# ubisoft/ubisoft-laforge-msmd

Hardware: NVIDIA B200
Metric: generated_animation_seconds_per_second (higher is better)
Workload: dtype bf16 tcgen05 (t > 16) + one-pass fp16 tcgen05 (2 < t <= 16) + fp32-grade fp16x3 (t <= 2): every sampling step <= 1e-3 rel-L2 of the fp32 reference

## Files before the change

### ubisoft-laforge-msmd_b200/csrc/denoiser.cu

```cuda
#include "denoiser_kernels.cuh"
#include "gemm_tc.cuh"
#include "profile.cuh"
#include <cuda_fp16.h>
#include <cstdlib>
#include <cstring>
#include <map>
#include <string>
#include <tuple>
#include <vector>

using namespace msmd;

namespace {

constexpr int kRow0FusedMaxS = 1 << 30;

struct LayerW {
  bf16 *Wqkv = nullptr, *Wo = nullptr, *Wq0 = nullptr, *Wkv = nullptr, *Wco = nullptr, *W1 = nullptr, *W2 = nullptr;
  float *bqkv = nullptr, *bo = nullptr, *bq0 = nullptr, *bkv = nullptr, *bco = nullptr, *b1 = nullptr, *b2 = nullptr;
  float *g1 = nullptr, *be1 = nullptr, *g2 = nullptr, *be2 = nullptr, *g3 = nullptr, *be3 = nullptr;
  bf16 *kv = nullptr, *ca = nullptr;
  bf16 *kvh = nullptr, *cah = nullptr;
  __half *Wqkv_h = nullptr, *Wqkv_l = nullptr, *Wo_h = nullptr, *Wo_l = nullptr, *Wq0_h = nullptr, *Wq0_l = nullptr,
         *Wkv_h = nullptr, *Wkv_l = nullptr, *Wco_h = nullptr, *Wco_l = nullptr, *W1_h = nullptr, *W1_l = nullptr,
         *W2_h = nullptr, *W2_l = nullptr;
  float *kv32 = nullptr, *ca32 = nullptr;
};

uint16_t f2bf(float f) {
  uint32_t u;
  memcpy(&u, &f, 4);
  if ((u & 0x7fffffffu) > 0x7f800000u) return (uint16_t)((u >> 16) | 0x40);
  u += 0x7fffu + ((u >> 16) & 1u);
  return (uint16_t)(u >> 16);
}

}

struct msmd_model {
  msmd_config c{};
  int device = 0;
  bool loaded = false, window = false;
  int T = 0, dp = 0, ldd = 80;
  std::vector<LayerW> L;
  std::vector<void*> owned;
  std::vector<void*> wowned;
  bool packing = false;
  float *PE = nullptr, *temb = nullptr, *Wp = nullptr, *bp = nullptr, *Wf = nullptr, *WfT = nullptr, *bf_ = nullptr;
  __half* Wf16 = nullptr;
  std::vector<float*> Ws0, bs0, Ws2, bs2;
  bf16 *Wd1 = nullptr, *Wd2 = nullptr;
  float *bd1 = nullptr, *bd2 = nullptr;
  float *alphas = nullptr, *alpha_bars = nullptr, *sig_flex = nullptr, *sig_inflex = nullptr;
  bf16 *x = nullptr, *qkv = nullptr, *ctx = nullptr, *h = nullptr, *dec1 = nullptr, *mem = nullptr, *x0c = nullptr,
       *q0 = nullptr, *ctx0 = nullptr;
  bf16 *y = nullptr, *y0 = nullptr, *memh = nullptr;
  float *dec2 = nullptr, *pp = nullptr, *pmproj = nullptr, *stat = nullptr,
        *hid = nullptr, *xbuf = nullptr, *mixed = nullptr, *thr = nullptr;
  int* steps = nullptr;
  __half *Wd1_h = nullptr, *Wd1_l = nullptr, *Wd2_h = nullptr, *Wd2_l = nullptr;
  float *fx = nullptr, *fqkv = nullptr, *fctx = nullptr, *fh = nullptr, *fy = nullptr, *fdec1 = nullptr, *fmem = nullptr,
        *fx0c = nullptr, *fq0 = nullptr, *fctx0 = nullptr, *fy0 = nullptr;
  __half *ws_hi = nullptr, *ws_lo = nullptr;
  int* overflow = nullptr;
  int *h_overflow = nullptr;
  cudaEvent_t ovf_event = nullptr;
  bool ovf_pending = false;
  bool window16[2] = {false, false}, window32 = false;
  float *w_audio = nullptr, *w_prev_audio = nullptr, *w_ind = nullptr;
  int S = 0, NX = 0, E = 0;
  const float* indicator = nullptr;
  UpdateParams* d_up = nullptr;
  unsigned int* d_done = nullptr;
  cudaStream_t cap_stream = nullptr;
  typedef std::tuple<int, int, int, int, int, float, float, float> GraphKey;
  std::map<GraphKey, cudaGraphExec_t> graphs;
  void drop_graphs() {
    for (auto& g : graphs) cudaGraphExecDestroy(g.second);
    graphs.clear();
  }
};

namespace {

template <class Tp>
int dalloc(msmd_model* m, Tp** p, size_t n) {
  void* q = nullptr;
  MSMD_CHECK_CUDA(cudaMalloc(&q, n * sizeof(Tp)));
  (m->packing ? m->wowned : m->owned).push_back(q);
  *p = static_cast<Tp*>(q);
  return MSMD_OK;
}

int up_f32(msmd_model* m, float** dst, const std::vector<float>& h) {
  int rc = dalloc(m, dst, h.size());
  if (rc) return rc;
  MSMD_CHECK_CUDA(cudaMemcpy(*dst, h.data(), h.size() * 4, cudaMemcpyHostToDevice));
  return MSMD_OK;
}
int up_bf16(msmd_model* m, bf16** dst, const float* h, size_t n) {
  std::vector<uint16_t> t(n);
  for (size_t i = 0; i < n; ++i) t[i] = f2bf(h[i]);
  int rc = dalloc(m, dst, n);
  if (rc) return rc;
  MSMD_CHECK_CUDA(cudaMemcpy(*dst, t.data(), n * 2, cudaMemcpyHostToDevice));
  return MSMD_OK;
}

int gemm(int fmt, const bf16* A, int64_t lda, const void* W, int64_t ldw, const float* bias, const bf16* aux, int64_t ld_aux,
         void* out, int64_t ldo, int out_f32, int M, int N, int K, int act, cudaStream_t st) {
  GemmDesc d;
  d.mode = fmt ? 3 : 0; d.A = A; d.W = W; d.bias = bias; d.aux = aux; d.out = out;
  d.M = M; d.N = N; d.K = K; d.lda = lda; d.ldw = ldw; d.ldo = ldo; d.ld_aux = ld_aux;
  d.out_f32 = out_f32; d.aux_f32 = 0; d.act = act; d.gelu_heavy = act;
  return gemm_tc_launch(d, st);
}

int up_split(msmd_model* m, __half** hi, __half** lo, const float* h, size_t n, bool want_lo) {
  std::vector<__half> a(n), b(want_lo ? n : 0);
  for (size_t i = 0; i < n; ++i) {
    a[i] = __float2half_rn(h[i]);
    if (want_lo) b[i] = __float2half_rn((h[i] - __half2float(a[i])) * 2048.0f);
  }
  int rc;
  if ((rc = dalloc(m, hi, n))) return rc;
  MSMD_CHECK_CUDA(cudaMemcpy(*hi, a.data(), n * sizeof(__half), cudaMemcpyHostToDevice));
  if (want_lo) {
    if ((rc = dalloc(m, lo, n))) return rc;
    MSMD_CHECK_CUDA(cudaMemcpy(*lo, b.data(), n * sizeof(__half), cudaMemcpyHostToDevice));
  }
  return MSMD_OK;
}

int gemm32(msmd_model* m, const float* A, int64_t lda, const __half* Wh, const __half* Wl, int64_t ldw, const float* bias,
           float* out, int64_t ldo, int M, int N, int K, int act, cudaStream_t st) {
  int rc;
  if ((rc = split_f16(A, m->ws_hi, m->ws_lo, (int64_t)(M - 1) * lda + K, st, m->overflow))) return rc;
  GemmDesc d;
  d.mode = 2; d.A = m->ws_hi; d.A_lo = m->ws_lo; d.W = Wh; d.W_lo = Wl; d.bias = bias; d.out = out;
  d.M = M; d.N = N; d.K = K; d.lda = lda; d.ldw = ldw; d.ldo = ldo; d.out_f32 = 1; d.aux_f32 = 1; d.act = act;
  return gemm_tc_launch(d, st);
}

int window_begin_f32(msmd_model* m, cudaStream_t st);

int run_forward_f32(msmd_model* m, const float* xrows, cudaStream_t st) {
  const msmd_config& c = m->c;
  const int S = m->S, T = m->T, d = c.d_model, M = S * T;
  int rc;
  if (!m->window32 && (rc = window_begin_f32(m, st))) return rc;
  EmbedParams ep{};
  ep.pp = m->pp; ep.temb = m->temb; ep.pmproj = m->pmproj; ep.PE = m->PE; ep.steps = m->steps;
  ep.x = xrows; ep.indicator = c.use_indicator ? m->indicator : nullptr; ep.WfT = m->WfT; ep.bf = m->bf_;
  ep.out = nullptr; ep.S = S; ep.NX = m->NX; ep.E = m->E; ep.Lp = c.n_prev_motions; ep.L = c.n_motions; ep.d = d;
  ep.dm = c.motion_dim;
  if ((rc = embed_f32_launch(ep, m->fx, st))) return rc;
  for (int l = 0; l < c.n_layers; ++l) {
    LayerW& w = m->L[l];
    if ((rc = gemm32(m, m->fx, d, w.Wqkv_h, w.Wqkv_l, d, w.bqkv, m->fqkv, 3 * d, M, 3 * d, d, 0, st))) return rc;
    if ((rc = self_attn_f32_launch(m->fqkv, m->fctx, S, T, c.n_heads, st))) return rc;
    if ((rc = gemm32(m, m->fctx, d, w.Wo_h, w.Wo_l, d, w.bo, m->fy, d, M, d, d, 0, st))) return rc;
    if ((rc = ln_f32_launch(m->fy, m->fx, w.g1, w.be1, w.ca32, w.g2, w.be2, m->fx, m->fx0c, M, T, st))) return rc;
    if ((rc = gemm32(m, m->fx0c, d, w.Wq0_h, w.Wq0_l, d, w.bq0, m->fq0, d, S, d, d, 0, st))) return rc;
    if ((rc = cross_attn_row0_f32_launch(m->fq0, w.kv32, m->fctx0, S, T - 1, c.n_heads, st))) return rc;
    if ((rc = gemm32(m, m->fctx0, d, w.Wco_h, w.Wco_l, d, w.bco, m->fy0, d, S, d, d, 0, st))) return rc;
    if ((rc = ln_row0_f32_launch(m->fy0, m->fx0c, w.g2, w.be2, m->fx, S, T, st))) return rc;
    if ((rc = gemm32(m, m->fx, d, w.W1_h, w.W1_l, d, w.b1, m->fh, c.d_ff, M, c.d_ff, d, 1, st))) return rc;
    if ((rc = gemm32(m, m->fh, c.d_ff, w.W2_h, w.W2_l, c.d_ff, w.b2, m->fy, d, M, d, c.d_ff, 0, st))) return rc;
    if ((rc = ln_f32_launch(m->fy, m->fx, w.g3, w.be3, nullptr, nullptr, nullptr, m->fx, nullptr, M, T, st))) return rc;
  }
  if ((rc = gemm32(m, m->fx, d, m->Wd1_h, m->Wd1_l, d, m->bd1, m->fdec1, d / 2, M, d / 2, d, 1, st))) return rc;
  if ((rc = gemm32(m, m->fdec1, d / 2, m->Wd2_h, m->Wd2_l, d / 2, m->bd2, m->dec2, m->ldd, M, c.motion_dim + c.n_basis,
                   d / 2, 0, st)))
    return rc;
  return MSMD_OK;
}

int window_begin_f32(msmd_model* m, cudaStream_t st) {
  const msmd_config& c = m->c;
  const int S = m->S, d = c.d_model, Tk = m->T - 1;
  int rc;
  if ((rc = build_memory_f32(m->w_prev_audio, m->w_audio, m->fmem, S, c.n_prev_motions, c.n_motions, d, st))) return rc;
  for (auto& w : m->L) {
    if ((rc = gemm32(m, m->fmem, d, w.Wkv_h, w.Wkv_l, d, w.bkv, w.kv32, 2 * d, S * Tk, 2 * d, d, 0, st))) return rc;
    if ((rc = split_f16(w.kv32, m->ws_hi, m->ws_lo, (int64_t)S * Tk * 2 * d, st, m->overflow))) return rc;
    GemmDesc g;
    g.mode = 2; g.A = m->ws_hi + d; g.A_lo = m->ws_lo + d; g.W = w.Wco_h; g.W_lo = w.Wco_l; g.bias = w.bco; g.out = w.ca32;
    g.M = S * Tk; g.N = d; g.K = d; g.lda = 2 * d; g.ldw = d; g.ldo = d; g.out_f32 = 1; g.aux_f32 = 1;
    if ((rc = gemm_tc_launch(g, st))) return rc;
  }
  m->window32 = true;
  return MSMD_OK;
}

int run_forward(msmd_model* m, const float* xrows, cudaStream_t st, int fmt) {
  const msmd_config& c = m->c;
  const int S = m->S, T = m->T, d = c.d_model, M = S * T;
  int rc;
  EmbedParams ep{};
  ep.pp = m->pp; ep.temb = m->temb; ep.pmproj = m->pmproj; ep.PE = m->PE; ep.steps = m->steps;
  ep.x = xrows; ep.indicator = c.use_indicator ? m->indicator : nullptr; ep.WfT = m->WfT; ep.bf = m->bf_;
  ep.out = m->x; ep.S = S; ep.NX = m->NX; ep.E = m->E; ep.Lp = c.n_prev_motions; ep.L = c.n_motions; ep.d = d;
  ep.dm = c.motion_dim; ep.fp16 = fmt; ep.Wf16 = m->Wf16;
  if ((rc = embed_launch(ep, st))) return rc;
  for (int l = 0; l < c.n_layers; ++l) {
    LayerW& w = m->L[l];
    const void *Wqkv = fmt ? (const void*)w.Wqkv_h : w.Wqkv, *Wo = fmt ? (const void*)w.Wo_h : w.Wo,
               *Wq0 = fmt ? (const void*)w.Wq0_h : w.Wq0, *Wco = fmt ? (const void*)w.Wco_h : w.Wco,
               *W1 = fmt ? (const void*)w.W1_h : w.W1, *W2 = fmt ? (const void*)w.W2_h : w.W2;
    const bf16 *kv = fmt ? w.kvh : w.kv, *ca = fmt ? w.cah : w.ca;
    if ((rc = gemm(fmt, m->x, d, Wqkv, d, w.bqkv, nullptr, 0, m->qkv, 3 * d, 0, M, 3 * d, d, 0, st))) return rc;
    if ((rc = self_attn_tc_launch(m->qkv, m->ctx, S, T, c.n_heads, fmt, st))) return rc;
    if ((rc = gemm(fmt, m->ctx, d, Wo, d, w.bo, nullptr, 0, m->y, d, 0, M, d, d, 0, st))) return rc;
    LnParams lp{};
    lp.resid = m->x;
    lp.y = m->y; lp.g1 = w.g1; lp.b1 = w.be1; lp.add = ca; lp.g2 = w.g2; lp.b2 = w.be2; lp.out = m->x;
    lp.x0 = m->x0c; lp.skip_tok0 = 0; lp.M = M; lp.T = T; lp.d = d; lp.fp16 = fmt;
    if ((rc = ln_launch(lp, st))) return rc;
    static const int row0_max_s = [] { const char* e = getenv("MSMD_ROW0_FUSED_MAX_S"); return e ? atoi(e) : kRow0FusedMaxS; }();
    if (S <= row0_max_s) {
      if ((rc = row0_fused_launch(m->x0c, static_cast<const bf16*>(Wq0), w.bq0, kv, static_cast<const bf16*>(Wco), w.bco, w.g2,
                                  w.be2, m->x, S, T, T - 1, c.n_heads, d, fmt, st)))
        return rc;
    } else {
      if ((rc = gemm(fmt, m->x0c, d, Wq0, d, w.bq0, nullptr, 0, m->q0, d, 0, S, d, d, 0, st))) return rc;
      if ((rc = cross_attn_row0_launch(m->q0, kv, m->ctx0, S, T - 1, c.n_heads, fmt, st))) return rc;
      if ((rc = gemm(fmt, m->ctx0, d, Wco, d, w.bco, nullptr, 0, m->y0, d, 0, S, d, d, 0, st))) return rc;
      if ((rc = ln_row0_launch(m->y0, m->x0c, w.g2, w.be2, m->x, nullptr, S, T, d, fmt, st))) return rc;
    }
    if ((rc = gemm(fmt, m->x, d, W1, d, w.b1, nullptr, 0, m->h, c.d_ff, 0, M, c.d_ff, d, 1, st))) return rc;
    if ((rc = gemm(fmt, m->h, c.d_ff, W2, c.d_ff, w.b2, nullptr, 0, m->y, d, 0, M, d, c.d_ff, 0, st))) return rc;
    LnParams l3{};
    l3.resid = m->x;
    l3.y = m->y; l3.g1 = w.g3; l3.b1 = w.be3; l3.add = nullptr; l3.g2 = nullptr; l3.b2 = nullptr; l3.out = m->x;
    l3.x0 = nullptr; l3.skip_tok0 = 0; l3.M = M; l3.T = T; l3.d = d; l3.fp16 = fmt;
    if ((rc = ln_launch(l3, st))) return rc;
  }
  const void *Wd1 = fmt ? (const void*)m->Wd1_h : m->Wd1, *Wd2 = fmt ? (const void*)m->Wd2_h : m->Wd2;
  if ((rc = gemm(fmt, m->x, d, Wd1, d, m->bd1, nullptr, 0, m->dec1, d / 2, 0, M, d / 2, d, 1, st))) return rc;
  if ((rc = gemm(fmt, m->dec1, d / 2, Wd2, d / 2, m->bd2, nullptr, 0, m->dec2, m->ldd, 1, M, c.motion_dim + c.n_basis,
                 d / 2, 0, st)))
    return rc;
  return MSMD_OK;
}

int window_begin_16(msmd_model* m, int fmt, cudaStream_t st) {
  const msmd_config& c = m->c;
  const int S = m->S, d = c.d_model, Tk = m->T - 1;
  int rc;
  bf16* mem = fmt ? m->memh : m->mem;
  if ((rc = build_memory_h16(m->w_prev_audio, m->w_audio, mem, S, c.n_prev_motions, c.n_motions, d, fmt, st))) return rc;
  for (auto& w : m->L) {
    bf16 *kv = fmt ? w.kvh : w.kv, *ca = fmt ? w.cah : w.ca;
    const void *Wkv = fmt ? (const void*)w.Wkv_h : w.Wkv, *Wco = fmt ? (const void*)w.Wco_h : w.Wco;
    if ((rc = gemm(fmt, mem, d, Wkv, d, w.bkv, nullptr, 0, kv, 2 * d, 0, S * Tk, 2 * d, d, 0, st))) return rc;
    if ((rc = gemm(fmt, kv + d, 2 * d, Wco, d, w.bco, nullptr, 0, ca, d, 0, S * Tk, d, d, 0, st))) return rc;
  }
  m->window16[fmt] = true;
  return MSMD_OK;
}

bool has_bf16(const msmd_config& c) { return c.precision == 0 || c.precision == 2; }
bool has_fp16(const msmd_config& c) { return c.precision == 2 || c.precision == 3; }
bool has_f32(const msmd_config& c) { return c.precision == 1 || c.precision == 2; }

int poll_overflow(msmd_model* m, const char* who) {
  if (!m->ovf_pending || cudaEventQuery(m->ovf_event) != cudaSuccess) return MSMD_OK;
  m->ovf_pending = false;
  if (*m->h_overflow) {
    *m->h_overflow = 0;
    cudaMemset(m->overflow, 0, sizeof(int));
    set_error("%s: an earlier fp32-grade call left the fp16 range of its GEMM operand split (|activation| > 65504 or NaN); "
              "its output was poisoned with NaN", who);
    return MSMD_ERR_INVALID;
  }
  return MSMD_OK;
}
int post_overflow(msmd_model* m, cudaStream_t st) {
  MSMD_CHECK_CUDA(cudaMemcpyAsync(m->h_overflow, m->overflow, sizeof(int), cudaMemcpyDeviceToHost, st));
  MSMD_CHECK_CUDA(cudaEventRecord(m->ovf_event, st));
  m->ovf_pending = true;
  return MSMD_OK;
}

}

extern "C" int msmd_create(const msmd_config* cfg, int device, msmd_model** out) {
  MSMD_REQUIRE(cfg && out, "msmd_create: null argument");
  const msmd_config& c = *cfg;
  MSMD_REQUIRE(c.d_model == 512 && c.n_heads * 64 == c.d_model, "msmd_create: only d_model=512 / 8 heads x 64 is built (got %d / %d)",
               c.d_model, c.n_heads);
  MSMD_REQUIRE(c.n_motions > 0 && c.n_prev_motions >= 0 && 1 + c.n_prev_motions + c.n_motions <= 112,
               "msmd_create: sequence 1 + n_prev_motions + n_motions = %d exceeds the 112-token attention tile "
               "(the released configuration is 1 + 10 + 100)", 1 + c.n_prev_motions + c.n_motions);
  MSMD_REQUIRE(c.n_layers > 0 && c.d_ff > 0 && c.d_ff % 8 == 0 && c.max_seqs > 0 && c.n_diff_steps > 0, "msmd_create: bad sizes");
  MSMD_REQUIRE(c.motion_dim > 3 && c.n_basis >= 0 && c.motion_dim + c.n_basis <= 80, "msmd_create: motion_dim + n_basis > 80");
  if (c.align_mask_width != 1) {
    set_error("msmd_create: align_mask_width=%d: only width 1 (step-invariant cross attention) is implemented", c.align_mask_width);
    return MSMD_ERR_UNSUPPORTED;
  }
  MSMD_REQUIRE(c.precision >= 0 && c.precision <= 3,
               "msmd_create: precision %d (0 bf16, 1 fp32-grade, 2 hybrid: bf16 + fp16 + fp32-grade, 3 fp16)", c.precision);
  MSMD_CHECK_CUDA(cudaSetDevice(device));
  msmd_model* m = new msmd_model();
  m->c = c;
  m->device = device;
  m->T = 1 + c.n_prev_motions + c.n_motions;
  m->dp = c.d_shape + c.d_style;
  m->L.resize(c.n_layers);
  const size_t S = c.max_seqs, T = m->T, M = S * T, d = c.d_model;
  int rc = MSMD_OK;
  auto A = [&](auto** p, size_t n) { if (!rc) rc = dalloc(m, p, n); };
  A(&m->dec2, M * m->ldd); A(&m->pp, S * d);
  A(&m->pmproj, S * c.n_prev_motions * d); A(&m->stat, S * c.n_basis * c.motion_dim); A(&m->hid, S * d);
  A(&m->thr, S);
  A(&m->xbuf, S * c.n_motions * c.motion_dim); A(&m->mixed, S * (T - 1) * c.motion_dim); A(&m->steps, S);
  A(&m->w_audio, S * c.n_motions * d); A(&m->w_prev_audio, S * c.n_prev_motions * d); A(&m->w_ind, S * c.n_motions);
  A(&m->d_up, 1); A(&m->d_done, 1);
  if (has_bf16(c) || has_fp16(c)) {
    A(&m->x, M * d); A(&m->qkv, M * 3 * d); A(&m->ctx, M * d); A(&m->h, M * c.d_ff); A(&m->dec1, M * d / 2);
    A(&m->x0c, S * d); A(&m->q0, S * d); A(&m->ctx0, S * d); A(&m->y, M * d); A(&m->y0, S * d);
  }
  if (has_bf16(c)) {
    A(&m->mem, S * (T - 1) * d);
    for (auto& w : m->L) { A(&w.kv, S * (T - 1) * 2 * d); A(&w.ca, S * (T - 1) * d); }
  }
  if (has_fp16(c)) {
    A(&m->memh, S * (T - 1) * d);
    for (auto& w : m->L) { A(&w.kvh, S * (T - 1) * 2 * d); A(&w.cah, S * (T - 1) * d); }
  }
  if (has_f32(c)) {
    A(&m->fx, M * d); A(&m->fqkv, M * 3 * d); A(&m->fctx, M * d); A(&m->fh, M * c.d_ff); A(&m->fy, M * d);
    A(&m->fdec1, M * d / 2); A(&m->fmem, S * (T - 1) * d); A(&m->fx0c, S * d); A(&m->fq0, S * d); A(&m->fctx0, S * d);
    A(&m->fy0, S * d);
    const size_t ws = std::max(M * (size_t)c.d_ff, S * (T - 1) * 2 * d);
    A(&m->ws_hi, ws); A(&m->ws_lo, ws); A(&m->overflow, 1);
    for (auto& w : m->L) { A(&w.kv32, S * (T - 1) * 2 * d); A(&w.ca32, S * (T - 1) * d); }
  }
  if (!rc && cudaStreamCreateWithFlags(&m->cap_stream, cudaStreamNonBlocking) != cudaSuccess) rc = MSMD_ERR_CUDA;
  if (!rc && m->overflow) {
    if (cudaMallocHost(&m->h_overflow, sizeof(int)) != cudaSuccess ||
        cudaEventCreateWithFlags(&m->ovf_event, cudaEventDisableTiming) != cudaSuccess)
      rc = MSMD_ERR_CUDA;
    else
      *m->h_overflow = 0;
  }
  if (rc) { msmd_destroy(m); return rc; }
  cudaMemset(m->dec2, 0, M * m->ldd * sizeof(float));
  cudaMemset(m->d_done, 0, sizeof(unsigned int));
  if (m->overflow) cudaMemset(m->overflow, 0, sizeof(int));
  *out = m;
  return MSMD_OK;
}

extern "C" void msmd_destroy(msmd_model* m) {
  if (!m) return;
  cudaSetDevice(m->device);
  cudaDeviceSynchronize();
  m->drop_graphs();
  if (m->cap_stream) cudaStreamDestroy(m->cap_stream);
  if (m->ovf_event) cudaEventDestroy(m->ovf_event);
  if (m->h_overflow) cudaFreeHost(m->h_overflow);
  for (void* p : m->owned) cudaFree(p);
  for (void* p : m->wowned) cudaFree(p);
  delete m;
}

extern "C" int msmd_load_weights(msmd_model* m, const char* const* names, const void* const* data,
                                 const int64_t* numel, int n) {
  MSMD_REQUIRE(m && names && data && numel, "msmd_load_weights: null argument");
  const msmd_config& c = m->c;
  MSMD_CHECK_CUDA(cudaSetDevice(m->device));
  MSMD_CHECK_CUDA(cudaDeviceSynchronize());
  m->drop_graphs();
  for (void* p : m->wowned) cudaFree(p);
  m->wowned.clear();
  m->loaded = false;
  m->window = false;
  struct PackScope { msmd_model* m; PackScope(msmd_model* mm) : m(mm) { m->packing = true; } ~PackScope() { m->packing = false; } } scope(m);
  std::map<std::string, int> idx;
  for (int i = 0; i < n; ++i) idx[names[i]] = i;
  std::string missing;
  int rc = MSMD_OK;
  auto fetch = [&](const std::string& key, size_t expect, std::vector<float>& h) -> bool {
    auto it = idx.find(key);
    if (it == idx.end()) { missing += key + " "; return false; }
    if ((size_t)numel[it->second] != expect) {
      set_error("msmd_load_weights: %s has %lld elements, expected %zu", key.c_str(), (long long)numel[it->second], expect);
      rc = MSMD_ERR_INVALID;
      return false;
    }
    h.resize(expect);
    if (cudaMemcpy(h.data(), data[it->second], expect * 4, cudaMemcpyDefault) != cudaSuccess) {
      set_error("msmd_load_weights: copy of %s failed", key.c_str());
      rc = MSMD_ERR_CUDA;
      return false;
    }
    return true;
  };
  const size_t d = c.d_model, ff = c.d_ff, dm = c.motion_dim, fin = dm + (c.use_indicator ? 1 : 0);
  const std::string P = "denoising_net.";
  std::vector<float> h, h2;
  auto F32 = [&](const std::string& key, size_t n_, float** dst) { if (!rc && fetch(key, n_, h)) rc = up_f32(m, dst, h); };
  const bool want_bf = has_bf16(c), want_hi = has_fp16(c) || has_f32(c), want_lo = has_f32(c);
  auto put_w = [&](const float* src, size_t n_, bf16** dst, __half** hi, __half** lo) {
    if (!rc && want_bf) rc = up_bf16(m, dst, src, n_);
    if (!rc && want_hi) rc = up_split(m, hi, lo, src, n_, want_lo);
  };
  auto BF = [&](const std::string& key, size_t n_, bf16** dst, __half** hi, __half** lo) {
    if (!rc && fetch(key, n_, h)) put_w(h.data(), n_, dst, hi, lo);
  };

  for (int l = 0; l < c.n_layers && !rc; ++l) {
    LayerW& w = m->L[l];
    const std::string q = P + "transformer.layers." + std::to_string(l) + ".";
    BF(q + "self_attn.in_proj_weight", 3 * d * d, &w.Wqkv, &w.Wqkv_h, &w.Wqkv_l);
    F32(q + "self_attn.in_proj_bias", 3 * d, &w.bqkv);
    BF(q + "self_attn.out_proj.weight", d * d, &w.Wo, &w.Wo_h, &w.Wo_l);
    F32(q + "self_attn.out_proj.bias", d, &w.bo);
    if (!rc && fetch(q + "multihead_attn.in_proj_weight", 3 * d * d, h)) {
      put_w(h.data(), d * d, &w.Wq0, &w.Wq0_h, &w.Wq0_l);
      put_w(h.data() + d * d, 2 * d * d, &w.Wkv, &w.Wkv_h, &w.Wkv_l);
    }
    if (!rc && fetch(q + "multihead_attn.in_proj_bias", 3 * d, h)) {
      rc = up_f32(m, &w.bq0, std::vector<float>(h.begin(), h.begin() + d));
      if (!rc) rc = up_f32(m, &w.bkv, std::vector<float>(h.begin() + d, h.end()));
    }
    BF(q + "multihead_attn.out_proj.weight", d * d, &w.Wco, &w.Wco_h, &w.Wco_l);
    F32(q + "multihead_attn.out_proj.bias", d, &w.bco);
    BF(q + "linear1.weight", ff * d, &w.W1, &w.W1_h, &w.W1_l);
    F32(q + "linear1.bias", ff, &w.b1);
    BF(q + "linear2.weight", d * ff, &w.W2, &w.W2_h, &w.W2_l);
    F32(q + "linear2.bias", d, &w.b2);
    F32(q + "norm1.weight", d, &w.g1); F32(q + "norm1.bias", d, &w.be1);
    F32(q + "norm2.weight", d, &w.g2); F32(q + "norm2.bias", d, &w.be2);
    F32(q + "norm3.weight", d, &w.g3); F32(q + "norm3.bias", d, &w.be3);
  }
  F32(P + "PE", (size_t)m->T * d, &m->PE);
  F32(P + "person_proj.weight", d * m->dp, &m->Wp);
  F32(P + "person_proj.bias", d, &m->bp);
  if (!rc && fetch(P + "feature_proj.weight", d * fin, h)) {
    rc = up_f32(m, &m->Wf, h);
    std::vector<float> t((dm + 1) * d, 0.f);
    for (size_t cc = 0; cc < d; ++cc)
      for (size_t k = 0; k < fin; ++k) t[k * d + cc] = h[cc * fin + k];
    if (!rc) rc = up_f32(m, &m->WfT, t);
    if (!rc && dm <= 80) {
      std::vector<__half> w16(2 * d * 80, __float2half_rn(0.f));
      for (size_t cc = 0; cc < d; ++cc)
        for (size_t k = 0; k < dm; ++k) {
          const float v = h[cc * fin + k];
          const __half hi = __float2half_rn(v);
          w16[cc * 80 + k] = hi;
          w16[d * 80 + cc * 80 + k] = __float2half_rn(v - __half2float(hi));
        }
      rc = dalloc(m, &m->Wf16, w16.size());
      if (!rc) MSMD_CHECK_CUDA(cudaMemcpy(m->Wf16, w16.data(), w16.size() * sizeof(__half), cudaMemcpyHostToDevice));
    }
  }
  F32(P + "feature_proj.bias", d, &m->bf_);
  m->Ws0.assign(c.n_basis, nullptr); m->bs0 = m->Ws2 = m->bs2 = m->Ws0;
  for (int b = 0; b < c.n_basis && !rc; ++b) {
    const std::string q = P + "static_feature_mapping." + std::to_string(b) + ".";
    F32(q + "0.weight", d * c.d_style, &m->Ws0[b]); F32(q + "0.bias", d, &m->bs0[b]);
    F32(q + "2.weight", dm * d, &m->Ws2[b]); F32(q + "2.bias", dm, &m->bs2[b]);
  }
  BF(P + "motion_dec.0.weight", (d / 2) * d, &m->Wd1, &m->Wd1_h, &m->Wd1_l);
  F32(P + "motion_dec.0.bias", d / 2, &m->bd1);
  BF(P + "motion_dec.2.weight", (dm + c.n_basis) * (d / 2), &m->Wd2, &m->Wd2_h, &m->Wd2_l);
  if (!rc && fetch(P + "motion_dec.2.bias", dm + c.n_basis, h)) {
    h.resize(m->ldd, 0.f);
    rc = up_f32(m, &m->bd2, h);
  }
  const size_t nt = c.n_diff_steps + 1;
  float *te = nullptr, *w0 = nullptr, *b0 = nullptr, *w2 = nullptr, *b2 = nullptr, *hid = nullptr;
  F32(P + "TE.pe", nt * d, &te);
  F32(P + "diff_step_map.0.weight", d * d, &w0); F32(P + "diff_step_map.0.bias", d, &b0);
  F32(P + "diff_step_map.2.weight", d * d, &w2); F32(P + "diff_step_map.2.bias", d, &b2);
  F32("diffusion_sched.alphas", nt, &m->alphas);
  F32("diffusion_sched.alpha_bars", nt, &m->alpha_bars);
  F32("diffusion_sched.sigmas_flex", nt, &m->sig_flex);
  F32("diffusion_sched.sigmas_inflex", nt, &m->sig_inflex);
  if (rc) return rc;
  if (!missing.empty()) {
    set_error("msmd_load_weights: missing state_dict keys: %s", missing.c_str());
    return MSMD_ERR_INVALID;
  }
  if ((rc = dalloc(m, &hid, nt * d)) || (rc = dalloc(m, &m->temb, nt * d))) return rc;
  if ((rc = linear_simt(te, d, w0, d, b0, hid, d, (int)nt, (int)d, (int)d, 1, 0))) return rc;
  if ((rc = linear_simt(hid, d, w2, d, b2, m->temb, d, (int)nt, (int)d, (int)d, 0, 0))) return rc;
  MSMD_CHECK_CUDA(cudaDeviceSynchronize());
  m->loaded = true;
  return MSMD_OK;
}

extern "C" int msmd_window_begin(msmd_model* m, const float* audio, const float* person, const float* style,
                                 const float* prev_motion, const float* prev_audio, const float* indicator, int S,
                                 int NX, int E, void* stream) {
  MSMD_REQUIRE(m, "msmd_window_begin: null model");
  if (!m->loaded) { set_error("msmd_window_begin: weights not loaded"); return MSMD_ERR_STATE; }
  const msmd_config& c = m->c;
  MSMD_REQUIRE(S > 0 && NX > 0 && E > 0 && S == NX * E, "msmd_window_begin: S=%d must equal NX*E=%d*%d", S, NX, E);
  MSMD_REQUIRE(S <= c.max_seqs, "msmd_window_begin: %d sequences exceed the capacity %d given at create", S, c.max_seqs);
  MSMD_REQUIRE(E <= 3, "msmd_window_begin: at most 2 guidance conditions (3 entries)");
  MSMD_REQUIRE(audio && person && style && prev_motion && prev_audio, "msmd_window_begin: null conditioning tensor");
  MSMD_REQUIRE(!c.use_indicator || indicator, "Missing indicator: the model was built with use_indicator");
  int rc;
  if ((rc = poll_overflow(m, "msmd_window_begin"))) return rc;
  cudaStream_t st = static_cast<cudaStream_t>(stream);
  const int d = c.d_model, Lp = c.n_prev_motions, dm = c.motion_dim;
  m->S = S; m->NX = NX; m->E = E;
  MSMD_CHECK_CUDA(cudaMemcpyAsync(m->w_audio, audio, (size_t)S * c.n_motions * d * 4, cudaMemcpyDeviceToDevice, st));
  MSMD_CHECK_CUDA(cudaMemcpyAsync(m->w_prev_audio, prev_audio, (size_t)S * Lp * d * 4, cudaMemcpyDeviceToDevice, st));
  if (c.use_indicator)
    MSMD_CHECK_CUDA(cudaMemcpyAsync(m->w_ind, indicator, (size_t)S * c.n_motions * 4, cudaMemcpyDeviceToDevice, st));
  m->indicator = c.use_indicator ? m->w_ind : nullptr;
  m->window16[0] = m->window16[1] = m->window32 = false;
  if ((rc = linear_simt(person, m->dp, m->Wp, m->dp, m->bp, m->pp, d, S, d, m->dp, 0, st))) return rc;
  const int fin = dm + (c.use_indicator ? 1 : 0);
  if ((rc = linear_simt(prev_motion, dm, m->Wf, fin, m->bf_, m->pmproj, d, S * Lp, d, dm, 0, st))) return rc;
  for (int b = 0; b < c.n_basis; ++b) {
    if ((rc = linear_simt(style, c.d_style, m->Ws0[b], c.d_style, m->bs0[b], m->hid, d, S, d, c.d_style, 1, st))) return rc;
    if ((rc = linear_simt(m->hid, d, m->Ws2[b], d, m->bs2[b], m->stat + b * dm, (int64_t)c.n_basis * dm, S, dm, d, 0, st)))
      return rc;
  }
  if (c.precision == 1) { if ((rc = window_begin_f32(m, st))) return rc; }
  else if ((rc = window_begin_16(m, c.precision == 3 ? 1 : 0, st))) return rc;
  m->window = true;
  return MSMD_OK;
}

__global__ void steps_from_i64_kernel(const int64_t* in, int* out, int S, int t_max) {
  const int i = blockIdx.x * blockDim.x + threadIdx.x;
  if (i < S) out[i] = (int)min((int64_t)t_max, max((int64_t)0, in[i]));
}

namespace {
int check_path(const msmd_model* m, int path, const char* who) {
  const bool ok = path == 0 ? has_bf16(m->c) : (path == 1 ? has_f32(m->c) : (path == 2 ? has_fp16(m->c) : false));
  if (!ok) {
    set_error("%s: arithmetic %d (0 bf16, 1 fp32-grade, 2 fp16) is not resident in a model created with precision %d", who,
              path, m->c.precision);
    return MSMD_ERR_STATE;
  }
  return MSMD_OK;
}
int forward_path(msmd_model* m, const float* xrows, int path, cudaStream_t st) {
  int rc;
  if (path == 1) return run_forward_f32(m, xrows, st);
  const int fmt = path == 2 ? 1 : 0;
  if (!m->window16[fmt] && (rc = window_begin_16(m, fmt, st))) return rc;
  return run_forward(m, xrows, st, fmt);
}
}

extern "C" int msmd_denoise(msmd_model* m, const float* motion, const int64_t* steps, float* out, void* stream) {
  MSMD_REQUIRE(m, "msmd_denoise: null argument");
  return msmd_denoise_ex(m, motion, steps, out, m->c.precision == 1 ? 1 : (m->c.precision == 3 ? 2 : 0), stream);
}

extern "C" int msmd_denoise_ex(msmd_model* m, const float* motion, const int64_t* steps, float* out, int precise,
                               void* stream) {
  MSMD_REQUIRE(m && motion && steps && out, "msmd_denoise: null argument");
  if (!m->window) { set_error("msmd_denoise: call msmd_window_begin first"); return MSMD_ERR_STATE; }
  MSMD_REQUIRE(m->E == 1 && m->NX == m->S, "msmd_denoise: window must be opened with NX == S, E == 1");
  int rc = check_path(m, precise, "msmd_denoise");
  if (rc) return rc;
  cudaStream_t st = static_cast<cudaStream_t>(stream);
  steps_from_i64_kernel<<<cdiv(m->S, 256), 256, 0, st>>>(steps, m->steps, m->S, m->c.n_diff_steps);
  MSMD_CHECK_LAUNCH();
  if ((rc = forward_path(m, motion, precise, st))) return rc;
  if ((rc = mix_static_launch(m->dec2, m->stat, out, m->S, m->T, m->c.motion_dim, m->c.n_basis, m->ldd, st))) return rc;
  if (precise == 1) {
    int flag = 0;
    MSMD_CHECK_CUDA(cudaMemcpyAsync(&flag, m->overflow, sizeof(int), cudaMemcpyDeviceToHost, st));
    MSMD_CHECK_CUDA(cudaStreamSynchronize(st));
    if (flag) {
      cudaMemsetAsync(m->overflow, 0, sizeof(int), st);
      set_error("msmd_denoise: an activation left the fp16 range of the fp32-grade GEMM operand split (|x| > 65504 or NaN)");
      return MSMD_ERR_INVALID;
    }
  }
  return MSMD_OK;
}

extern "C" int msmd_denoise_parts(msmd_model* m, const float* motion, const int64_t* steps, float* dyn, float* stat,
                                  float* alphas, int precise, void* stream) {
  MSMD_REQUIRE(m && motion && steps && dyn && stat && alphas, "msmd_denoise_parts: null argument");
  if (!m->window) { set_error("msmd_denoise_parts: call msmd_window_begin first"); return MSMD_ERR_STATE; }
  MSMD_REQUIRE(m->E == 1 && m->NX == m->S, "msmd_denoise_parts: window must be opened with NX == S, E == 1");
  int rc = check_path(m, precise, "msmd_denoise_parts");
  if (rc) return rc;
  cudaStream_t st = static_cast<cudaStream_t>(stream);
  steps_from_i64_kernel<<<cdiv(m->S, 256), 256, 0, st>>>(steps, m->steps, m->S, m->c.n_diff_steps);
  MSMD_CHECK_LAUNCH();
  if ((rc = forward_path(m, motion, precise, st))) return rc;
  return split_parts_launch(m->dec2, m->stat, dyn, stat, alphas, m->S, m->T, m->c.motion_dim, m->c.n_basis, m->ldd, st);
}

extern "C" int msmd_sample_window(msmd_model* m, const float* x_T, const float* z, uint64_t seed, int cfg_independent,
                                  float scale0, float scale1, float flexibility, int t_start, int n_steps,
                                  float* x_out, float* traj, void* stream) {
  return msmd_sample_window_ex(m, x_T, z, seed, cfg_independent, scale0, scale1, flexibility, t_start, n_steps, x_out,
                               traj, nullptr, stream);
}

extern "C" int msmd_sample_window_ex(msmd_model* m, const float* x_T, const float* z, uint64_t seed, int cfg_independent,
                                     float scale0, float scale1, float flexibility, int t_start, int n_steps,
                                     float* x_out, float* traj, const msmd_sample_extras* ex, void* stream) {
  MSMD_REQUIRE(m && x_T && x_out, "msmd_sample_window: null argument");
  if (!m->window) { set_error("msmd_sample_window: call msmd_window_begin first"); return MSMD_ERR_STATE; }
  const msmd_config& c = m->c;
  MSMD_REQUIRE(t_start >= 1 && t_start <= c.n_diff_steps && n_steps >= 1 && n_steps <= t_start,
               "msmd_sample_window: steps %d..%d outside 1..%d", t_start, t_start - n_steps + 1, c.n_diff_steps);
  MSMD_REQUIRE(flexibility >= 0.f && flexibility <= 1.f, "msmd_sample_window: flexibility outside [0,1]");
  int rc;
  if ((rc = poll_overflow(m, "msmd_sample_window"))) return rc;
  cudaStream_t st = static_cast<cudaStream_t>(stream);
  const size_t n_el = (size_t)m->NX * c.n_motions * c.motion_dim;
  MSMD_CHECK_CUDA(cudaMemcpyAsync(m->xbuf, x_T, n_el * 4, cudaMemcpyDeviceToDevice, st));
  if ((rc = steps_set(m->steps, m->S, t_start, st))) return rc;

  int k32 = c.precision == 1 ? c.n_diff_steps : 0;
  int k16 = c.precision == 3 ? c.n_diff_steps : 0;
  if (ex && c.precision != 1) {
    k32 = ex->precise_last_steps < 0 ? c.n_diff_steps : ex->precise_last_steps;
    MSMD_REQUIRE(k32 == 0 || has_f32(c), "msmd_sample_window: precise_last_steps needs a model created with precision 2");
  }
  if (ex && c.precision != 3 && c.precision != 1) {
    k16 = ex->fp16_last_steps < 0 ? c.n_diff_steps : ex->fp16_last_steps;
    MSMD_REQUIRE(k16 == 0 || has_fp16(c), "msmd_sample_window: fp16_last_steps needs a model created with precision 2");
  }
  if (k16 < k32) k16 = k32;

  UpdateParams up{};
  up.dec = m->dec2; up.stat = m->stat; up.x = m->xbuf; up.z = z; up.traj = traj; up.steps = m->steps;
  up.alphas = m->alphas; up.alpha_bars = m->alpha_bars; up.sig_flex = m->sig_flex; up.sig_inflex = m->sig_inflex;
  up.scale0 = scale0; up.scale1 = scale1; up.flexibility = flexibility; up.seed = seed;
  up.NX = m->NX; up.E = m->E; up.T = m->T; up.L = c.n_motions; up.Lp = c.n_prev_motions; up.dm = c.motion_dim;
  up.nb = c.n_basis; up.ldd = m->ldd; up.cfg_independent = cfg_independent; up.target_noise = c.target_noise;
  up.thr = nullptr; up.tgt_dyn = nullptr; up.cum_static = nullptr; up.alpha_traj = nullptr; up.t_start = t_start;
  up.overflow = k32 > 0 ? m->overflow : nullptr;
  up.done = m->d_done; up.steps_rw = m->steps; up.S = m->S;
  bool use_dt = false;
  float dt_ratio = 0.f, dt_min = 0.f, dt_max = 0.f;
  if (ex) {
    use_dt = ex->use_dynamic_threshold != 0;
    dt_ratio = ex->dt_ratio; dt_min = ex->dt_min; dt_max = ex->dt_max;
    MSMD_REQUIRE(!use_dt || (dt_ratio >= 0.f && dt_ratio <= 1.f), "quantile() q values must be in the range [0, 1]");
    if (use_dt) up.thr = m->thr;
    up.tgt_dyn = ex->target_dynamic; up.cum_static = ex->cumulative_static; up.alpha_traj = ex->alpha_traj;
    up.noise_offset = (long long)ex->noise_clip_offset * c.n_motions * c.motion_dim;
    if (up.cum_static) MSMD_CHECK_CUDA(cudaMemsetAsync(up.cum_static, 0, n_el * 4, st));
  }
  if ((rc = update_params_set(m->d_up, up, st))) return rc;

  auto one_step = [&](cudaStream_t s, int path) -> int {
    int r;
    if ((r = forward_path(m, m->xbuf, path, s))) return r;
    if (use_dt && (r = threshold_launch(m->dec2, m->stat, m->thr, m->S, m->T, c.n_motions, c.n_prev_motions, c.motion_dim,
                                        c.n_basis, m->ldd, dt_ratio, dt_min, dt_max, s)))
      return r;
    return update_launch(m->d_up, m->NX, c.n_motions, c.motion_dim, s);
  };

  auto run_16 = [&](int path, int n) -> int {
    if (n <= 0) return MSMD_OK;
    int r;
    const int fmt = path == 2 ? 1 : 0;
    if ((r = check_path(m, path, "msmd_sample_window"))) return r;
    if (!m->window16[fmt] && (r = window_begin_16(m, fmt, st))) return r;
    if (profiling_on() || n < 3) {
      for (int i = 0; i < n; ++i)
        if ((r = one_step(st, path))) return r;
      return MSMD_OK;
    }
    const msmd_model::GraphKey key(fmt, m->S, m->NX, m->E, use_dt ? 1 : 0, dt_ratio, dt_min, dt_max);
    auto it = m->graphs.find(key);
    if (it == m->graphs.end()) {
      if ((r = one_step(st, path))) return r;
      n -= 1;
      cudaGraph_t graph = nullptr;
      cudaGraphExec_t exec = nullptr;
      MSMD_CHECK_CUDA(cudaStreamBeginCapture(m->cap_stream, cudaStreamCaptureModeThreadLocal));
      r = one_step(m->cap_stream, path);
      cudaError_t ce = cudaStreamEndCapture(m->cap_stream, &graph);
      if (r || ce != cudaSuccess) {
        if (graph) cudaGraphDestroy(graph);
        if (!r) { set_error("msmd_sample_window: graph capture failed: %s", cudaGetErrorString(ce)); r = MSMD_ERR_CUDA; }
        return r;
      }
      ce = cudaGraphInstantiate(&exec, graph, 0);
      cudaGraphDestroy(graph);
      if (ce != cudaSuccess) {
        set_error("msmd_sample_window: cudaGraphInstantiate failed: %s", cudaGetErrorString(ce));
        return MSMD_ERR_CUDA;
      }
      it = m->graphs.emplace(key, exec).first;
    }
    for (int i = 0; i < n; ++i) MSMD_CHECK_CUDA(cudaGraphLaunch(it->second, st));
    return MSMD_OK;
  };

  const int t_end = t_start - n_steps + 1;
  auto count = [&](int hi, int lo) { hi = std::min(hi, t_start); lo = std::max(lo, t_end); return hi >= lo ? hi - lo + 1 : 0; };
  const int n_main = count(c.n_diff_steps, k16 + 1), n_f16 = count(k16, k32 + 1), n_hi = count(k32, 1);
  if ((rc = run_16(has_bf16(c) ? 0 : 2, n_main))) return rc;
  if ((rc = run_16(2, n_f16))) return rc;
  if (n_hi > 0 && (rc = check_path(m, 1, "msmd_sample_window"))) return rc;
  for (int i = 0; i < n_hi; ++i)
    if ((rc = one_step(st, 1))) return rc;
  if (n_hi > 0 && (rc = post_overflow(m, st))) return rc;
  MSMD_CHECK_CUDA(cudaMemcpyAsync(x_out, m->xbuf, n_el * 4, cudaMemcpyDeviceToDevice, st));
  return MSMD_OK;
}

extern "C" int msmd_check(msmd_model* m, void* stream) {
  MSMD_REQUIRE(m, "msmd_check: null model");
  MSMD_CHECK_CUDA(cudaStreamSynchronize(static_cast<cudaStream_t>(stream)));
  return poll_overflow(m, "msmd_check");
}
```

### ubisoft-laforge-msmd_b200/csrc/denoiser_kernels.cu

```cuda
#include "denoiser_kernels.cuh"
#include "profile.cuh"
#include <cuda_fp16.h>
#include <cstdlib>

namespace msmd {

__device__ __forceinline__ float warp_sum(float v) {
#pragma unroll
  for (int o = 16; o > 0; o >>= 1) v += __shfl_xor_sync(0xffffffffu, v, o);
  return v;
}
__device__ __forceinline__ float warp_max(float v) {
#pragma unroll
  for (int o = 16; o > 0; o >>= 1) v = fmaxf(v, __shfl_xor_sync(0xffffffffu, v, o));
  return v;
}
__device__ __forceinline__ uint32_t pack_bf16(float lo, float hi) {
  __nv_bfloat162 h = __floats2bfloat162_rn(lo, hi);
  return *reinterpret_cast<uint32_t*>(&h);
}
template <bool F16>
__device__ __forceinline__ uint32_t pack_h(float lo, float hi) {
  if constexpr (F16) {
    __half2 h = __floats2half2_rn(lo, hi);
    return *reinterpret_cast<uint32_t*>(&h);
  } else {
    return pack_bf16(lo, hi);
  }
}
template <bool F16>
__device__ __forceinline__ float2 unpack_h(uint32_t w) {
  if constexpr (F16) return __half22float2(*reinterpret_cast<const __half2*>(&w));
  else return make_float2(__uint_as_float(w << 16), __uint_as_float(w & 0xffff0000u));
}
template <bool F16>
__device__ __forceinline__ void store_h1(bf16* dst, float v) {
  if constexpr (F16) *reinterpret_cast<__half*>(dst) = __float2half_rn(v);
  else *dst = __float2bfloat16_rn(v);
}
__device__ __forceinline__ float gelu_exact(float x) { return 0.5f * x * (1.0f + erff(x * 0.70710678118654752f)); }

__global__ void __launch_bounds__(256) linear_simt_kernel(const float* __restrict__ x, int64_t ldx,
                                                          const float* __restrict__ W, int64_t ldw,
                                                          const float* __restrict__ b, float* __restrict__ out,
                                                          int64_t ldo, int R, int C, int K, int act) {
  const int lane = threadIdx.x & 31;
  const int64_t w = ((int64_t)blockIdx.x * blockDim.x + threadIdx.x) >> 5;
  if (w >= (int64_t)R * C) return;
  const int r = (int)(w / C), c = (int)(w % C);
  const float* xr = x + r * ldx;
  const float* wr = W + (int64_t)c * ldw;
  float s = 0.f;
  for (int k = lane; k < K; k += 32) s = fmaf(xr[k], wr[k], s);
  s = warp_sum(s);
  if (lane == 0) {
    s += b ? b[c] : 0.f;
    if (act == 1) s = gelu_exact(s);
    out[r * ldo + c] = s;
  }
}
int linear_simt(const float* x, int64_t ldx, const float* W, int64_t ldw, const float* b, float* out, int64_t ldo, int R,
                int C, int K, int act, cudaStream_t st) {
  if (R <= 0 || C <= 0) return MSMD_OK;
  const int64_t warps = (int64_t)R * C;
  linear_simt_kernel<<<cdiv(warps * 32, 256), 256, 0, st>>>(x, ldx, W, ldw, b, out, ldo, R, C, K, act);
  MSMD_CHECK_LAUNCH();
  return MSMD_OK;
}

__global__ void cast_rows_bf16_kernel(const float* __restrict__ src, int64_t lds, bf16* __restrict__ dst, int64_t ldd,
                                      int64_t rows, int cols) {
  const int64_t n = rows * cols;
  for (int64_t i = (int64_t)blockIdx.x * blockDim.x + threadIdx.x; i < n; i += (int64_t)gridDim.x * blockDim.x) {
    const int64_t r = i / cols;
    const int c = (int)(i % cols);
    dst[r * ldd + c] = __float2bfloat16_rn(src[r * lds + c]);
  }
}
int cast_rows_bf16(const float* src, int64_t lds, bf16* dst, int64_t ldd, int64_t rows, int cols, cudaStream_t st) {
  if (rows * cols == 0) return MSMD_OK;
  cast_rows_bf16_kernel<<<(int)std::min<int64_t>(cdiv(rows * cols, 256), kNumSMs * 16), 256, 0, st>>>(src, lds, dst, ldd,
                                                                                                   rows, cols);
  MSMD_CHECK_LAUNCH();
  return MSMD_OK;
}

template <bool F16>
__global__ void build_memory_kernel(const float* __restrict__ prev_audio, const float* __restrict__ audio,
                                    bf16* __restrict__ mem, int S, int Lp, int L, int d) {
  const int64_t n = (int64_t)S * (Lp + L) * d;
  for (int64_t i = (int64_t)blockIdx.x * blockDim.x + threadIdx.x; i < n; i += (int64_t)gridDim.x * blockDim.x) {
    const int c = (int)(i % d);
    const int64_t row = i / d;
    const int tok = (int)(row % (Lp + L));
    const int64_t s = row / (Lp + L);
    const float v = tok < Lp ? prev_audio[(s * Lp + tok) * d + c] : audio[(s * L + tok - Lp) * d + c];
    store_h1<F16>(mem + i, v);
  }
}
int build_memory_h16(const float* prev_audio, const float* audio, bf16* mem, int S, int Lp, int L, int d, int fp16,
                     cudaStream_t st) {
  const int64_t n = (int64_t)S * (Lp + L) * d;
  const int grid = (int)std::min<int64_t>(cdiv(n, 256), kNumSMs * 16);
  if (fp16) build_memory_kernel<true><<<grid, 256, 0, st>>>(prev_audio, audio, mem, S, Lp, L, d);
  else build_memory_kernel<false><<<grid, 256, 0, st>>>(prev_audio, audio, mem, S, Lp, L, d);
  MSMD_CHECK_LAUNCH();
  return MSMD_OK;
}

template <bool F16>
__device__ __forceinline__ void embed_ctx_rows(const EmbedParams& p, int row) {
  const int T = 1 + p.Lp + p.L;
  const int s = row / (p.Lp + 1), i = row % (p.Lp + 1);
  const int t = p.steps[s];
  for (int c = threadIdx.x; c < p.d; c += blockDim.x) {
    float v = p.PE[i * p.d + c];
    v += (i == 0) ? (p.pp[(int64_t)s * p.d + c] + p.temb[(int64_t)t * p.d + c])
                  : p.pmproj[((int64_t)s * p.Lp + (i - 1)) * p.d + c];
    store_h1<F16>(p.out + ((int64_t)s * T + i) * p.d + c, v);
  }
}
constexpr int kEmbedRows = 25, kEmbedPitch = 28;
template <bool F16>
__global__ void __launch_bounds__(256, 2) embed_x_kernel(EmbedParams p) {
  griddep_launch();
  griddep_wait();
  extern __shared__ __align__(16) float xs[];
  const int T = 1 + p.Lp + p.L;
  const int blocks_per_x = (p.L + kEmbedRows - 1) / kEmbedRows;
  if ((int)blockIdx.x >= p.NX * blocks_per_x) {
    embed_ctx_rows<F16>(p, (int)blockIdx.x - p.NX * blocks_per_x);
    return;
  }
  const int n = blockIdx.x / blocks_per_x;
  const int l0 = (blockIdx.x % blocks_per_x) * kEmbedRows;
  const int nr = min(kEmbedRows, p.L - l0);
  float* inds = xs + p.dm * kEmbedPitch;
  for (int i = threadIdx.x; i < kEmbedPitch * p.dm; i += blockDim.x) {
    const int r = i / p.dm, k = i % p.dm;
    xs[k * kEmbedPitch + r] = r < nr ? p.x[((int64_t)n * p.L + l0 + r) * p.dm + k] : 0.f;
  }
  for (int i = threadIdx.x; i < p.E * kEmbedPitch; i += blockDim.x) {
    const int e = i / kEmbedPitch, r = i % kEmbedPitch;
    inds[i] = (p.indicator && r < nr) ? p.indicator[(int64_t)(e * p.NX + n) * p.L + l0 + r] : 0.f;
  }
  __syncthreads();
  for (int c = 2 * threadIdx.x; c < p.d; c += 2 * blockDim.x) {
    float a0[kEmbedPitch], a1[kEmbedPitch];
    const float2 bc = *reinterpret_cast<const float2*>(p.bf + c);
#pragma unroll
    for (int r = 0; r < kEmbedPitch; ++r) {
      float2 pe = make_float2(0.f, 0.f);
      if (r < nr) pe = __ldg(reinterpret_cast<const float2*>(p.PE + (int64_t)(1 + p.Lp + l0 + r) * p.d + c));
      a0[r] = bc.x + pe.x;
      a1[r] = bc.y + pe.y;
    }
    const float* wcol = p.WfT + c;
    for (int k0 = 0; k0 < p.dm; k0 += 4) {
      float2 w[4];
#pragma unroll
      for (int u = 0; u < 4; ++u)
        w[u] = k0 + u < p.dm ? __ldg(reinterpret_cast<const float2*>(wcol + (int64_t)(k0 + u) * p.d)) : make_float2(0.f, 0.f);
#pragma unroll
      for (int u = 0; u < 4; ++u) {
        if (k0 + u < p.dm) {
          const float4* xr = reinterpret_cast<const float4*>(xs + (k0 + u) * kEmbedPitch);
#pragma unroll
          for (int q = 0; q < kEmbedPitch / 4; ++q) {
            const float4 xv = xr[q];
            a0[4 * q + 0] = fmaf(xv.x, w[u].x, a0[4 * q + 0]); a1[4 * q + 0] = fmaf(xv.x, w[u].y, a1[4 * q + 0]);
            a0[4 * q + 1] = fmaf(xv.y, w[u].x, a0[4 * q + 1]); a1[4 * q + 1] = fmaf(xv.y, w[u].y, a1[4 * q + 1]);
            a0[4 * q + 2] = fmaf(xv.z, w[u].x, a0[4 * q + 2]); a1[4 * q + 2] = fmaf(xv.z, w[u].y, a1[4 * q + 2]);
            a0[4 * q + 3] = fmaf(xv.w, w[u].x, a0[4 * q + 3]); a1[4 * q + 3] = fmaf(xv.w, w[u].y, a1[4 * q + 3]);
          }
        }
      }
    }
    const float2 wi = *reinterpret_cast<const float2*>(p.WfT + (int64_t)p.dm * p.d + c);
#pragma unroll
    for (int r = 0; r < kEmbedRows; ++r) {
      if (r < nr) {
        const int l = l0 + r;
        for (int e = 0; e < p.E; ++e) {
          const float ind = inds[e * kEmbedPitch + r];
          const int s = e * p.NX + n;
          *reinterpret_cast<uint32_t*>(p.out + ((int64_t)s * T + 1 + p.Lp + l) * p.d + c) =
              pack_h<F16>(fmaf(ind, wi.x, a0[r]), fmaf(ind, wi.y, a1[r]));
        }
      }
    }
  }
}

constexpr int kEmRows = 32, kEmK = 80, kEmAPitch = 88, kEmSPitch = 72;
constexpr int kEmSmem = 2 * kEmRows * kEmAPitch * 2 + 3 * kEmRows * 4 + 8 * kEmRows * kEmSPitch * 4;
__device__ __forceinline__ void em_ldmatrix_x4(uint32_t (&r)[4], const void* smem_row) {
  asm volatile("ldmatrix.sync.aligned.m8n8.x4.shared.b16 {%0, %1, %2, %3}, [%4];"
               : "=r"(r[0]), "=r"(r[1]), "=r"(r[2]), "=r"(r[3])
               : "r"((uint32_t)__cvta_generic_to_shared(smem_row)));
}
__device__ __forceinline__ void em_mma(float (&d)[4], const uint32_t (&a)[4], uint32_t b0, uint32_t b1) {
  asm("mma.sync.aligned.m16n8k16.row.col.f32.f16.f16.f32 {%0, %1, %2, %3}, {%4, %5, %6, %7}, {%8, %9}, {%0, %1, %2, %3};"
               : "+f"(d[0]), "+f"(d[1]), "+f"(d[2]), "+f"(d[3]) : "r"(a[0]), "r"(a[1]), "r"(a[2]), "r"(a[3]), "r"(b0), "r"(b1));
}
template <bool F16>
__global__ void __launch_bounds__(256, 2) embed_x_mma_kernel(EmbedParams p) {
  griddep_launch();
  griddep_wait();
  extern __shared__ __align__(16) uint8_t esm[];
  const int T = 1 + p.Lp + p.L;
  const int rows_total = p.NX * p.L;
  const int n_tiles = (rows_total + kEmRows - 1) / kEmRows;
  if ((int)blockIdx.x >= n_tiles) {
    embed_ctx_rows<F16>(p, (int)blockIdx.x - n_tiles);
    return;
  }
  __half* a_hi = reinterpret_cast<__half*>(esm);
  __half* a_lo = a_hi + kEmRows * kEmAPitch;
  float* inds = reinterpret_cast<float*>(a_lo + kEmRows * kEmAPitch);
  float* stage = inds + 3 * kEmRows;
  const int tid = threadIdx.x, warp = tid >> 5, lane = tid & 31, gid = lane >> 2, tig = lane & 3;
  const int g0 = blockIdx.x * kEmRows;
  for (int i = tid; i < kEmRows * kEmK; i += 256) {
    const int r = i / kEmK, k = i - r * kEmK;
    float v = 0.f;
    if (k < p.dm && g0 + r < rows_total) v = p.x[(int64_t)(g0 + r) * p.dm + k];
    const __half hi = __float2half_rn(v);
    a_hi[r * kEmAPitch + k] = hi;
    a_lo[r * kEmAPitch + k] = __float2half_rn(v - __half2float(hi));
  }
  for (int i = tid; i < 3 * kEmRows; i += 256) {
    const int e = i / kEmRows, r = i - e * kEmRows, g = g0 + r;
    float v = 0.f;
    if (p.indicator != nullptr && e < p.E && g < rows_total) {
      const int n = g / p.L, l = g - n * p.L;
      v = p.indicator[(int64_t)(e * p.NX + n) * p.L + l];
    }
    inds[i] = v;
  }
  __syncthreads();

  const int n0 = warp * 64;
  float acc[2][8][4];
#pragma unroll
  for (int mt = 0; mt < 2; ++mt)
#pragma unroll
    for (int nt = 0; nt < 8; ++nt)
#pragma unroll
      for (int j = 0; j < 4; ++j) acc[mt][nt][j] = 0.f;
  const __half* Wh = static_cast<const __half*>(p.Wf16);
  const __half* Wl = Wh + (int64_t)p.d * kEmK;
  const int a_off = ((lane & 7) + ((lane >> 3) & 1) * 8) * kEmAPitch + (lane >> 4) * 8;
#pragma unroll
  for (int ks = 0; ks < kEmK / 16; ++ks) {
    uint32_t ah[2][4], al[2][4];
#pragma unroll
    for (int mt = 0; mt < 2; ++mt) {
      em_ldmatrix_x4(ah[mt], a_hi + 16 * mt * kEmAPitch + a_off + 16 * ks);
      em_ldmatrix_x4(al[mt], a_lo + 16 * mt * kEmAPitch + a_off + 16 * ks);
    }
#pragma unroll
    for (int nt = 0; nt < 8; ++nt) {
      const int64_t wo = (int64_t)(n0 + 8 * nt + gid) * kEmK + 16 * ks + 2 * tig;
      const uint32_t bh0 = __ldg(reinterpret_cast<const uint32_t*>(Wh + wo)), bh1 = __ldg(reinterpret_cast<const uint32_t*>(Wh + wo + 8));
      const uint32_t bl0 = __ldg(reinterpret_cast<const uint32_t*>(Wl + wo)), bl1 = __ldg(reinterpret_cast<const uint32_t*>(Wl + wo + 8));
#pragma unroll
      for (int mt = 0; mt < 2; ++mt) {
        em_mma(acc[mt][nt], al[mt], bh0, bh1);
        em_mma(acc[mt][nt], ah[mt], bl0, bl1);
        em_mma(acc[mt][nt], ah[mt], bh0, bh1);
      }
    }
  }
  float* sw = stage + warp * (kEmRows * kEmSPitch);
#pragma unroll
  for (int mt = 0; mt < 2; ++mt)
#pragma unroll
    for (int nt = 0; nt < 8; ++nt) {
      *reinterpret_cast<float2*>(sw + (16 * mt + gid) * kEmSPitch + 8 * nt + 2 * tig) = make_float2(acc[mt][nt][0], acc[mt][nt][1]);
      *reinterpret_cast<float2*>(sw + (16 * mt + gid + 8) * kEmSPitch + 8 * nt + 2 * tig) = make_float2(acc[mt][nt][2], acc[mt][nt][3]);
    }
  __syncwarp();
  const int c8 = (lane & 7) * 8, col = n0 + c8;
  float bias[8], wi[8];
  {
    const float4 b0 = __ldg(reinterpret_cast<const float4*>(p.bf + col)), b1 = __ldg(reinterpret_cast<const float4*>(p.bf + col + 4));
    const float4 w0 = __ldg(reinterpret_cast<const float4*>(p.WfT + (int64_t)p.dm * p.d + col));
    const float4 w1 = __ldg(reinterpret_cast<const float4*>(p.WfT + (int64_t)p.dm * p.d + col + 4));
    bias[0] = b0.x; bias[1] = b0.y; bias[2] = b0.z; bias[3] = b0.w; bias[4] = b1.x; bias[5] = b1.y; bias[6] = b1.z; bias[7] = b1.w;
    wi[0] = w0.x; wi[1] = w0.y; wi[2] = w0.z; wi[3] = w0.w; wi[4] = w1.x; wi[5] = w1.y; wi[6] = w1.z; wi[7] = w1.w;
  }
  float4 pe0[kEmRows / 4], pe1[kEmRows / 4];
#pragma unroll
  for (int it = 0; it < kEmRows / 4; ++it) {
    const int g = g0 + it * 4 + (lane >> 3);
    pe0[it] = pe1[it] = make_float4(0.f, 0.f, 0.f, 0.f);
    if (g < rows_total) {
      const int l = g - (g / p.L) * p.L;
      const float* pe = p.PE + (int64_t)(1 + p.Lp + l) * p.d + col;
      pe0[it] = __ldg(reinterpret_cast<const float4*>(pe));
      pe1[it] = __ldg(reinterpret_cast<const float4*>(pe + 4));
    }
  }
#pragma unroll
  for (int it = 0; it < kEmRows / 4; ++it) {
    const int r = it * 4 + (lane >> 3), g = g0 + r;
    if (g < rows_total) {
      const int n = g / p.L, l = g - n * p.L;
      const float4 s0 = *reinterpret_cast<const float4*>(sw + r * kEmSPitch + c8), s1 = *reinterpret_cast<const float4*>(sw + r * kEmSPitch + c8 + 4);
      const float4 p0 = pe0[it], p1 = pe1[it];
      float v[8] = {s0.x + (bias[0] + p0.x), s0.y + (bias[1] + p0.y), s0.z + (bias[2] + p0.z), s0.w + (bias[3] + p0.w),
                    s1.x + (bias[4] + p1.x), s1.y + (bias[5] + p1.y), s1.z + (bias[6] + p1.z), s1.w + (bias[7] + p1.w)};
      for (int e = 0; e < p.E; ++e) {
        const float ind = inds[e * kEmRows + r];
        uint4 o;
        o.x = pack_h<F16>(fmaf(ind, wi[0], v[0]), fmaf(ind, wi[1], v[1]));
        o.y = pack_h<F16>(fmaf(ind, wi[2], v[2]), fmaf(ind, wi[3], v[3]));
        o.z = pack_h<F16>(fmaf(ind, wi[4], v[4]), fmaf(ind, wi[5], v[5]));
        o.w = pack_h<F16>(fmaf(ind, wi[6], v[6]), fmaf(ind, wi[7], v[7]));
        *reinterpret_cast<uint4*>(p.out + ((int64_t)(e * p.NX + n) * T + 1 + p.Lp + l) * p.d + col) = o;
      }
    }
  }
}
int embed_launch(const EmbedParams& p, cudaStream_t st) {
  ProfileScope prof("embed", st);
  static const bool use_mma = [] { const char* e = getenv("MSMD_EMBED_MMA"); return e ? atoi(e) != 0 : true; }();
  if (use_mma && p.Wf16 != nullptr && p.d == 512 && p.dm <= kEmK && p.E <= 3) {
    static bool attr = false;
    if (!attr) {
      MSMD_CHECK_CUDA(cudaFuncSetAttribute(embed_x_mma_kernel<true>, cudaFuncAttributeMaxDynamicSharedMemorySize, kEmSmem));
      MSMD_CHECK_CUDA(cudaFuncSetAttribute(embed_x_mma_kernel<false>, cudaFuncAttributeMaxDynamicSharedMemorySize, kEmSmem));
      attr = true;
    }
    const int blocks = cdiv(p.NX * p.L, kEmRows) + p.S * (p.Lp + 1);
    MSMD_CHECK_CUDA(launch_pdl(p.fp16 ? embed_x_mma_kernel<true> : embed_x_mma_kernel<false>, dim3(blocks), dim3(256), kEmSmem, st, p));
    MSMD_CHECK_LAUNCH();
    return MSMD_OK;
  }
  const int blocks = p.NX * ((p.L + kEmbedRows - 1) / kEmbedRows) + p.S * (p.Lp + 1);
  MSMD_CHECK_CUDA(launch_pdl(p.fp16 ? embed_x_kernel<true> : embed_x_kernel<false>, dim3(blocks), dim3(256),
                             (p.dm + 3) * kEmbedPitch * sizeof(float), st, p));
  MSMD_CHECK_LAUNCH();
  return MSMD_OK;
}

template <int D>
__device__ __forceinline__ void ln_row(float (&v)[D / 32], const float* __restrict__ g, const float* __restrict__ b,
                                       int lane) {
  constexpr int NV = D / 32;
  float s = 0.f;
#pragma unroll
  for (int i = 0; i < NV; ++i) s += v[i];
  const float mean = warp_sum(s) * (1.0f / D);
  float q = 0.f;
#pragma unroll
  for (int i = 0; i < NV; ++i) { const float dlt = v[i] - mean; q = fmaf(dlt, dlt, q); }
  const float rstd = rsqrtf(warp_sum(q) * (1.0f / D) + 1e-5f);
#pragma unroll
  for (int i = 0; i < NV / 4; ++i) {
    const float4 gg = *reinterpret_cast<const float4*>(g + i * 128 + lane * 4);
    const float4 bb = *reinterpret_cast<const float4*>(b + i * 128 + lane * 4);
    v[4 * i + 0] = (v[4 * i + 0] - mean) * rstd * gg.x + bb.x;
    v[4 * i + 1] = (v[4 * i + 1] - mean) * rstd * gg.y + bb.y;
    v[4 * i + 2] = (v[4 * i + 2] - mean) * rstd * gg.z + bb.z;
    v[4 * i + 3] = (v[4 * i + 3] - mean) * rstd * gg.w + bb.w;
  }
}
template <bool F16>
__device__ __forceinline__ void store_h4(bf16* dst, float a, float b, float c, float d) {
  uint2 u;
  u.x = pack_h<F16>(a, b);
  u.y = pack_h<F16>(c, d);
  *reinterpret_cast<uint2*>(dst) = u;
}
template <bool F16, bool ADD>
__device__ __forceinline__ void load_h4(const bf16* src, float* v) {
  const uint2 u = *reinterpret_cast<const uint2*>(src);
  const float2 a = unpack_h<F16>(u.x), b = unpack_h<F16>(u.y);
  if (ADD) { v[0] += a.x; v[1] += a.y; v[2] += b.x; v[3] += b.y; }
  else { v[0] = a.x; v[1] = a.y; v[2] = b.x; v[3] = b.y; }
}

template <bool F16>
__device__ __forceinline__ void ln_unpack8(const uint4& u, float* v, bool add) {
  const float2 a = unpack_h<F16>(u.x), b = unpack_h<F16>(u.y), c = unpack_h<F16>(u.z), d = unpack_h<F16>(u.w);
  if (add) { v[0] += a.x; v[1] += a.y; v[2] += b.x; v[3] += b.y; v[4] += c.x; v[5] += c.y; v[6] += d.x; v[7] += d.y; }
  else { v[0] = a.x; v[1] = a.y; v[2] = b.x; v[3] = b.y; v[4] = c.x; v[5] = c.y; v[6] = d.x; v[7] = d.y; }
}
template <bool F16>
__device__ __forceinline__ uint4 ln_pack8(const float* v) {
  return make_uint4(pack_h<F16>(v[0], v[1]), pack_h<F16>(v[2], v[3]), pack_h<F16>(v[4], v[5]), pack_h<F16>(v[6], v[7]));
}
__device__ __forceinline__ void ln16(float (&v)[16], const float* __restrict__ sg, const float* __restrict__ sb, int lane) {
  float s = 0.f;
#pragma unroll
  for (int i = 0; i < 16; ++i) s += v[i];
  const float mean = warp_sum(s) * (1.0f / 512.0f);
  float q = 0.f;
#pragma unroll
  for (int i = 0; i < 16; ++i) { v[i] -= mean; q = fmaf(v[i], v[i], q); }
  const float rstd = rsqrtf(warp_sum(q) * (1.0f / 512.0f) + 1e-5f);
#pragma unroll
  for (int h = 0; h < 2; ++h) {
    const float4 g0 = *reinterpret_cast<const float4*>(sg + h * 256 + lane * 8), g1 = *reinterpret_cast<const float4*>(sg + h * 256 + lane * 8 + 4);
    const float4 b0 = *reinterpret_cast<const float4*>(sb + h * 256 + lane * 8), b1 = *reinterpret_cast<const float4*>(sb + h * 256 + lane * 8 + 4);
    float* w = v + 8 * h;
    w[0] = fmaf(w[0] * rstd, g0.x, b0.x); w[1] = fmaf(w[1] * rstd, g0.y, b0.y); w[2] = fmaf(w[2] * rstd, g0.z, b0.z); w[3] = fmaf(w[3] * rstd, g0.w, b0.w);
    w[4] = fmaf(w[4] * rstd, g1.x, b1.x); w[5] = fmaf(w[5] * rstd, g1.y, b1.y); w[6] = fmaf(w[6] * rstd, g1.z, b1.z); w[7] = fmaf(w[7] * rstd, g1.w, b1.w);
  }
}

template <int D, bool F16, int kLnRows>
__global__ void __launch_bounds__(256) ln_kernel(LnParams p) {
  static_assert(D == 512, "lane layout: two 8-element chunks per lane");
  griddep_launch();
  __shared__ __align__(16) float sgb[4][D];
  for (int i = threadIdx.x; i < D; i += blockDim.x) {
    sgb[0][i] = p.g1[i]; sgb[1][i] = p.b1[i];
    sgb[2][i] = p.g2 ? p.g2[i] : 0.f; sgb[3][i] = p.b2 ? p.b2[i] : 0.f;
  }
  griddep_wait();
  __syncthreads();
  const int lane = threadIdx.x & 31;
  const int row0 = (blockIdx.x * (blockDim.x >> 5) + (threadIdx.x >> 5)) * kLnRows;
  const int c0 = lane * 8, c1 = 256 + lane * 8;
  struct Raw { uint4 y0, y1, r0, r1, a0, a1; };
  auto load = [&](int row, Raw& w) {
    if (row >= p.M) return;
    const bf16* y = p.y + (int64_t)row * D;
    w.y0 = *reinterpret_cast<const uint4*>(y + c0); w.y1 = *reinterpret_cast<const uint4*>(y + c1);
    if (p.resid != nullptr) {
      const bf16* r = p.resid + (int64_t)row * D;
      w.r0 = *reinterpret_cast<const uint4*>(r + c0); w.r1 = *reinterpret_cast<const uint4*>(r + c1);
    }
    const int s = row / p.T, tok = row - s * p.T;
    if (p.add != nullptr && tok > 0) {
      const bf16* a = p.add + ((int64_t)s * (p.T - 1) + (tok - 1)) * D;
      w.a0 = __ldg(reinterpret_cast<const uint4*>(a + c0)); w.a1 = __ldg(reinterpret_cast<const uint4*>(a + c1));
    }
  };
  Raw cur, nxt;
  load(row0, cur);
#pragma unroll
  for (int i = 0; i < kLnRows; ++i) {
    const int row = row0 + i;
    if (i + 1 < kLnRows) load(row + 1, nxt);
    if (row < p.M) {
      const int s = row / p.T, tok = row - s * p.T;
      float v[16];
      ln_unpack8<F16>(cur.y0, v, false); ln_unpack8<F16>(cur.y1, v + 8, false);
      if (p.resid != nullptr) {
        ln_unpack8<F16>(cur.r0, v, true); ln_unpack8<F16>(cur.r1, v + 8, true);
      }
      if (!(tok == 0 && p.skip_tok0)) {
        ln16(v, sgb[0], sgb[1], lane);
        if (tok == 0 && p.x0 != nullptr) {
          bf16* o = p.x0 + (int64_t)s * D;
          *reinterpret_cast<uint4*>(o + c0) = ln_pack8<F16>(v); *reinterpret_cast<uint4*>(o + c1) = ln_pack8<F16>(v + 8);
        } else {
          if (p.add != nullptr && tok > 0) {
            ln_unpack8<F16>(cur.a0, v, true); ln_unpack8<F16>(cur.a1, v + 8, true);
            ln16(v, sgb[2], sgb[3], lane);
          }
          bf16* o = p.out + (int64_t)row * D;
          *reinterpret_cast<uint4*>(o + c0) = ln_pack8<F16>(v); *reinterpret_cast<uint4*>(o + c1) = ln_pack8<F16>(v + 8);
        }
      }
    }
    cur = nxt;
  }
}
template <int D, bool F16>
__global__ void __launch_bounds__(256) ln_kernel_v1(LnParams p) {
  griddep_launch();
  griddep_wait();
  constexpr int NV = D / 32;
  const int lane = threadIdx.x & 31;
  const int row = blockIdx.x * (blockDim.x >> 5) + (threadIdx.x >> 5);
  if (row >= p.M) return;
  const int s = row / p.T, tok = row % p.T;
  float v[NV];
  const bf16* y = p.y + (int64_t)row * D;
#pragma unroll
  for (int i = 0; i < NV / 4; ++i) load_h4<F16, false>(y + i * 128 + lane * 4, v + 4 * i);
  if (p.resid != nullptr) {
    const bf16* r = p.resid + (int64_t)row * D;
#pragma unroll
    for (int i = 0; i < NV / 4; ++i) load_h4<F16, true>(r + i * 128 + lane * 4, v + 4 * i);
  }
  if (tok == 0 && p.skip_tok0) return;
  ln_row<D>(v, p.g1, p.b1, lane);
  if (tok == 0 && p.x0 != nullptr) {
#pragma unroll
    for (int i = 0; i < NV / 4; ++i)
      store_h4<F16>(p.x0 + (int64_t)s * D + i * 128 + lane * 4, v[4 * i], v[4 * i + 1], v[4 * i + 2], v[4 * i + 3]);
    return;
  }
  if (p.add != nullptr && tok > 0) {
    const bf16* a = p.add + ((int64_t)s * (p.T - 1) + (tok - 1)) * D;
#pragma unroll
    for (int i = 0; i < NV / 4; ++i) load_h4<F16, true>(a + i * 128 + lane * 4, v + 4 * i);
    ln_row<D>(v, p.g2, p.b2, lane);
  }
  bf16* o = p.out + (int64_t)row * D;
#pragma unroll
  for (int i = 0; i < NV / 4; ++i) store_h4<F16>(o + i * 128 + lane * 4, v[4 * i], v[4 * i + 1], v[4 * i + 2], v[4 * i + 3]);
}
int ln_launch(const LnParams& p, cudaStream_t st) {
  MSMD_REQUIRE(p.d == 512, "ln: only d_model = 512 is instantiated (got %d)", p.d);
  ProfileScope prof(p.add ? "ln1_ln2" : "ln3", st);
  static const int rows = [] { const char* e = getenv("MSMD_LN_ROWS"); return e ? atoi(e) : 0; }();
  if (rows == 0) {
    MSMD_CHECK_CUDA(launch_pdl(p.fp16 ? ln_kernel_v1<512, true> : ln_kernel_v1<512, false>, dim3(cdiv(p.M, 8)), dim3(256), 0, st, p));
  } else if (rows == 1 || p.M <= 148 * 3 * 8) {
    MSMD_CHECK_CUDA(launch_pdl(p.fp16 ? ln_kernel<512, true, 1> : ln_kernel<512, false, 1>, dim3(cdiv(p.M, 8)), dim3(256), 0, st, p));
  } else if (rows == 4 || p.M < 148 * 3 * 8 * 4) {
    MSMD_CHECK_CUDA(launch_pdl(p.fp16 ? ln_kernel<512, true, 4> : ln_kernel<512, false, 4>, dim3(cdiv(p.M, 8 * 4)), dim3(256), 0, st, p));
  } else {
    MSMD_CHECK_CUDA(launch_pdl(p.fp16 ? ln_kernel<512, true, 6> : ln_kernel<512, false, 6>, dim3(cdiv(p.M, 8 * 6)), dim3(256), 0, st, p));
  }
  MSMD_CHECK_LAUNCH();
  return MSMD_OK;
}

template <int D, bool F16>
__global__ void __launch_bounds__(256) ln_row0_kernel(const bf16* __restrict__ y0, const bf16* __restrict__ resid0,
                                                      const float* __restrict__ g, const float* __restrict__ b,
                                                      bf16* __restrict__ out, bf16* __restrict__ out_c, int S, int T) {
  griddep_launch();
  griddep_wait();
  constexpr int NV = D / 32;
  const int lane = threadIdx.x & 31;
  const int s = blockIdx.x * (blockDim.x >> 5) + (threadIdx.x >> 5);
  if (s >= S) return;
  float v[NV];
#pragma unroll
  for (int i = 0; i < NV / 4; ++i) {
    load_h4<F16, false>(y0 + (int64_t)s * D + i * 128 + lane * 4, v + 4 * i);
    if (resid0 != nullptr) load_h4<F16, true>(resid0 + (int64_t)s * D + i * 128 + lane * 4, v + 4 * i);
  }
  ln_row<D>(v, g, b, lane);
#pragma unroll
  for (int i = 0; i < NV / 4; ++i) {
    if (out) store_h4<F16>(out + (int64_t)s * T * D + i * 128 + lane * 4, v[4 * i], v[4 * i + 1], v[4 * i + 2], v[4 * i + 3]);
    if (out_c) store_h4<F16>(out_c + (int64_t)s * D + i * 128 + lane * 4, v[4 * i], v[4 * i + 1], v[4 * i + 2], v[4 * i + 3]);
  }
}
int ln_row0_launch(const bf16* y0, const bf16* resid0, const float* g, const float* b, bf16* out, bf16* out_c, int S,
                   int T, int d, int fp16, cudaStream_t st) {
  MSMD_REQUIRE(d == 512, "ln_row0: only d_model = 512 is instantiated");
  ProfileScope prof("ln_row0", st);
  MSMD_CHECK_CUDA(launch_pdl(fp16 ? ln_row0_kernel<512, true> : ln_row0_kernel<512, false>, dim3(cdiv(S, 8)), dim3(256), 0, st,
                             y0, resid0, g, b, out, out_c, S, T));
  MSMD_CHECK_LAUNCH();
  return MSMD_OK;
}

constexpr int kCaBatch = 28;
template <bool F16>
__global__ void __launch_bounds__(128, 3) cross_attn_row0_kernel(const bf16* __restrict__ q0, const bf16* __restrict__ kv,
                                                                 bf16* __restrict__ ctx0, int Tk, int H) {
  griddep_launch();
  griddep_wait();
  constexpr int d = 512;
  const int w = blockIdx.x * 4 + (threadIdx.x >> 5), lane = threadIdx.x & 31;
  const int s = w / H, h = w % H;
  const bf16* kbase = kv + (int64_t)s * Tk * 2 * d + h * 64;
  const uint32_t* vbase = reinterpret_cast<const uint32_t*>(kbase + d) + lane;
  const int64_t vstride = d;

  uint32_t vb[2][kCaBatch];
  auto load_v = [&](int b, uint32_t (&dst)[kCaBatch]) {
#pragma unroll
    for (int u = 0; u < kCaBatch; ++u) {
      const int j = b * kCaBatch + u;
      dst[u] = j < Tk ? __ldg(vbase + (int64_t)j * vstride) : 0u;
    }
  };
  load_v(0, vb[0]);

  float q[64];
  {
    const uint4* qp = reinterpret_cast<const uint4*>(q0 + (int64_t)s * d + h * 64);
#pragma unroll
    for (int i = 0; i < 8; ++i) {
      const uint4 u = __ldg(qp + i);
      const uint32_t ww[4] = {u.x, u.y, u.z, u.w};
#pragma unroll
      for (int k = 0; k < 4; ++k) {
        const float2 f = unpack_h<F16>(ww[k]);
        q[i * 8 + 2 * k] = f.x;
        q[i * 8 + 2 * k + 1] = f.y;
      }
    }
  }
  float sc[4];
#pragma unroll
  for (int grp = 0; grp < 4; ++grp) {
    const int j = grp * 32 + lane;
    float dot = -INFINITY;
    if (j < Tk) {
      const uint4* kp = reinterpret_cast<const uint4*>(kbase + (int64_t)j * 2 * d);
      uint4 kr[8];
#pragma unroll
      for (int i = 0; i < 8; ++i) kr[i] = __ldg(kp + i);
      float acc = 0.f;
#pragma unroll
      for (int i = 0; i < 8; ++i) {
        const uint32_t ww[4] = {kr[i].x, kr[i].y, kr[i].z, kr[i].w};
#pragma unroll
        for (int k = 0; k < 4; ++k) {
          const float2 f = unpack_h<F16>(ww[k]);
          acc = fmaf(q[i * 8 + 2 * k], f.x, acc);
          acc = fmaf(q[i * 8 + 2 * k + 1], f.y, acc);
        }
      }
      dot = acc * 0.125f;
    }
    sc[grp] = dot;
  }
  const float m = warp_max(fmaxf(fmaxf(sc[0], sc[1]), fmaxf(sc[2], sc[3])));
  float l = 0.f;
#pragma unroll
  for (int i = 0; i < 4; ++i) { sc[i] = (sc[i] == -INFINITY) ? 0.f : __expf(sc[i] - m); l += sc[i]; }
  l = warp_sum(l);
  float oa = 0.f, ob = 0.f;
  auto consume = [&](int b, const uint32_t (&src)[kCaBatch]) {
#pragma unroll
    for (int u = 0; u < kCaBatch; ++u) {
      const int j = b * kCaBatch + u;
      const float p = __shfl_sync(0xffffffffu, sc[j >> 5], j & 31);
      const float2 f = unpack_h<F16>(src[u]);
      oa = fmaf(p, f.x, oa);
      ob = fmaf(p, f.y, ob);
    }
  };
  load_v(1, vb[1]); consume(0, vb[0]);
  load_v(2, vb[0]); consume(1, vb[1]);
  load_v(3, vb[1]); consume(2, vb[0]);
  consume(3, vb[1]);
  const float inv = 1.0f / l;
  *reinterpret_cast<uint32_t*>(ctx0 + (int64_t)s * d + h * 64 + 2 * lane) = pack_h<F16>(oa * inv, ob * inv);
}
int cross_attn_row0_launch(const bf16* q0, const bf16* kv, bf16* ctx0, int S, int Tk, int H, int fp16, cudaStream_t st) {
  MSMD_REQUIRE(Tk <= 4 * kCaBatch && H == 8, "cross_attn_row0: built for 8 heads x 64 and <= %d memory tokens (got %d, %d)",
               4 * kCaBatch, H, Tk);
  ProfileScope prof("cross_attn_row0", st);
  MSMD_CHECK_CUDA(launch_pdl(fp16 ? cross_attn_row0_kernel<true> : cross_attn_row0_kernel<false>, dim3(S * H / 4), dim3(128), 0, st,
                             q0, kv, ctx0, Tk, H));
  MSMD_CHECK_LAUNCH();
  return MSMD_OK;
}

__device__ __forceinline__ float philox_normal(unsigned long long seed, uint32_t t, uint32_t idx) {
  uint32_t c0 = idx, c1 = t, c2 = 0x9E3779B9u, c3 = 0xBB67AE85u;
  uint32_t k0 = (uint32_t)seed, k1 = (uint32_t)(seed >> 32);
#pragma unroll
  for (int r = 0; r < 10; ++r) {
    const uint32_t hi0 = __umulhi(0xD2511F53u, c0), lo0 = 0xD2511F53u * c0;
    const uint32_t hi1 = __umulhi(0xCD9E8D57u, c2), lo1 = 0xCD9E8D57u * c2;
    c0 = hi1 ^ c1 ^ k0; c1 = lo1; c2 = hi0 ^ c3 ^ k1; c3 = lo0;
    k0 += 0x9E3779B9u; k1 += 0xBB67AE85u;
  }
  const float u1 = ((c0 >> 8) + 1) * (1.0f / 16777216.0f);
  const float u2 = (c1 >> 8) * (1.0f / 16777216.0f);
  return sqrtf(-2.0f * __logf(u1)) * __cosf(6.283185307179586f * u2);
}

__device__ __forceinline__ void split_target(const float* dec, const float* stat, int T, int Lp, int dm, int nb, int ldd,
                                             int s, int l, int c, float& dyn, float& sta) {
  const float* row = dec + ((int64_t)s * T + 1 + Lp + l) * ldd;
  const float* st = stat + (int64_t)s * nb * dm;
  dyn = row[c];
  const bool face = c < dm - 3;
  float v = 0.f;
  for (int b = 0; b < nb; ++b) v += (face ? row[dm + b] : 1.0f) * st[b * dm + c];
  sta = v;
}

__global__ void __launch_bounds__(256) update_kernel(const UpdateParams* __restrict__ pp) {
  griddep_launch();
  griddep_wait();
  __shared__ __align__(16) unsigned char p_raw[sizeof(UpdateParams)];
  static_assert(sizeof(UpdateParams) % 4 == 0, "UpdateParams is copied in 32-bit words");
  for (int i = threadIdx.x; i < (int)(sizeof(UpdateParams) / 4); i += blockDim.x)
    reinterpret_cast<uint32_t*>(p_raw)[i] = reinterpret_cast<const uint32_t*>(pp)[i];
  __syncthreads();
  const UpdateParams& p = *reinterpret_cast<const UpdateParams*>(p_raw);
  const int64_t n_el = (int64_t)p.NX * p.L * p.dm;
  const int t = p.steps[0];
  const float alpha = p.alphas[t], ab = p.alpha_bars[t], abp = p.alpha_bars[t - 1];
  const float sigma = p.sig_flex[t] * p.flexibility + p.sig_inflex[t] * (1.0f - p.flexibility);
  float c0, c1;
  if (p.target_noise) {
    c0 = 1.0f / sqrtf(alpha);
    c1 = (1.0f - alpha) / sqrtf(1.0f - ab);
  } else {
    c0 = (1.0f - abp) * sqrtf(alpha) / (1.0f - ab);
    c1 = (1.0f - alpha) * sqrtf(abp) / (1.0f - ab);
  }
  struct Loc {
    const float *dec, *stat, *z, *thr; float *x, *traj, *tgt_dyn, *cum_static, *alpha_traj; const int* overflow;
    float scale0, scale1; unsigned long long seed; long long noise_offset;
    int NX, E, T, L, Lp, dm, nb, ldd, cfg_independent, target_noise, t_start;
  };
  const Loc q = {p.dec, p.stat, p.z, p.thr, p.x, p.traj, p.tgt_dyn, p.cum_static, p.alpha_traj, p.overflow,
                 p.scale0, p.scale1, p.seed, p.noise_offset,
                 p.NX, p.E, p.T, p.L, p.Lp, p.dm, p.nb, p.ldd, p.cfg_independent, p.target_noise, p.t_start};
  const bool sep = q.tgt_dyn != nullptr || q.cum_static != nullptr;
  const int lane = threadIdx.x & 31;
  const int rows = q.NX * q.L;
  for (int row = blockIdx.x * (blockDim.x >> 5) + (threadIdx.x >> 5); row < rows; row += gridDim.x * (blockDim.x >> 5)) {
    const int n = row / q.L, l = row - n * q.L;
    const float* rowp[3];
    const float* stp[3];
    float thv[3], al[3][4];
#pragma unroll
    for (int e = 0; e < 3; ++e) {
      const int sq = (e < q.E ? e : 0) * q.NX + n;
      rowp[e] = q.dec + ((int64_t)sq * q.T + 1 + q.Lp + l) * q.ldd;
      stp[e] = q.stat + (int64_t)sq * q.nb * q.dm;
      thv[e] = q.thr ? q.thr[sq] : 0.f;
#pragma unroll
      for (int b = 0; b < 4; ++b) al[e][b] = b < q.nb ? rowp[e][q.dm + b] : 0.f;
    }
   for (int c = lane; c < q.dm; c += 32) {
    const int64_t i = (int64_t)row * q.dm + c;
    const bool face = c < q.dm - 3;
    float tgt = 0.f, prev = 0.f, td = 0.f, pd = 0.f, ts = 0.f, psv = 0.f;
#pragma unroll
    for (int e = 0; e < 3; ++e) {
      if (e >= q.E) break;
      const float dyn = rowp[e][c];
      float sta = 0.f;
      if (q.nb <= 4) {
#pragma unroll
        for (int b = 0; b < 4; ++b)
          if (b < q.nb) sta += (face ? al[e][b] : 1.0f) * stp[e][b * q.dm + c];
      } else {
        for (int b = 0; b < q.nb; ++b) sta += (face ? rowp[e][q.dm + b] : 1.0f) * stp[e][b * q.dm + c];
      }
      float r = dyn + sta;
      if (q.thr) { const float th = thv[e]; r = fminf(fmaxf(r, -th), th); }
      if (e == 0) {
        tgt = r; td = dyn; ts = sta;
      } else {
        const float sc = (e == 1) ? q.scale0 : q.scale1;
        const bool run = q.cfg_independent || e == 1;
        tgt = tgt + sc * (r - (run ? tgt : prev));
        if (sep) { td = td + sc * (dyn - (run ? td : pd)); ts = ts + sc * (sta - (run ? ts : psv)); }
      }
      prev = r; pd = dyn; psv = sta;
    }
    float zt = 0.f;
    if (t > 1) zt = q.z ? q.z[(int64_t)t * n_el + i] : philox_normal(q.seed, (uint32_t)t, (uint32_t)(i + q.noise_offset));
    const float xo = q.x[i];
    float xn = q.target_noise ? (c0 * (xo - c1 * tgt) + sigma * zt) : (c0 * xo + c1 * tgt + sigma * zt);
    if (q.overflow != nullptr && *q.overflow != 0) xn = __int_as_float(0x7fc00000);
    q.x[i] = xn;
    if (q.traj) q.traj[(int64_t)(t - 1) * n_el + i] = xn;
    if (q.tgt_dyn) q.tgt_dyn[i] = td;
    if (q.cum_static) q.cum_static[i] += c1 * ts;
    if (q.alpha_traj && c < q.nb) {
      float ta = 0.f, pa = 0.f;
      for (int e = 0; e < q.E; ++e) {
        const float a = q.dec[((int64_t)(e * q.NX + n) * q.T + 1 + q.Lp + l) * q.ldd + q.dm + c];
        if (e == 0) ta = a;
        else ta = ta + ((e == 1) ? q.scale0 : q.scale1) * (a - ((q.cfg_independent || e == 1) ? ta : pa));
        pa = a;
      }
      q.alpha_traj[(((int64_t)(q.t_start - t) * q.NX + n) * q.L + l) * q.nb + c] = ta;
    }
   }
  }
  if (p.done != nullptr) {
    __shared__ bool last;
    __syncthreads();
    if (threadIdx.x == 0) {
      __threadfence();
      last = atomicAdd(p.done, 1u) == gridDim.x - 1;
    }
    __syncthreads();
    if (last) {
      for (int i = threadIdx.x; i < p.S; i += blockDim.x) p.steps_rw[i] = t - 1;
      if (threadIdx.x == 0) *p.done = 0u;
    }
  }
}

__global__ void __launch_bounds__(1024) threshold_kernel(const float* __restrict__ dec, const float* __restrict__ stat,
                                                         float* __restrict__ thr, int T, int L, int Lp, int dm, int nb,
                                                         int ldd, float ratio, float lo, float hi) {
  extern __shared__ uint32_t keys[];
  const int n = L * dm;
  uint32_t* hist = keys + n;
  uint32_t* sel = hist + 256;
  const int s = blockIdx.x, tid = threadIdx.x;
  for (int i = tid; i < n; i += blockDim.x) {
    float dyn, sta;
    split_target(dec, stat, T, Lp, dm, nb, ldd, s, i / dm, i % dm, dyn, sta);
    keys[i] = __float_as_uint(fabsf(dyn + sta));
  }
  const float pos = ratio * (float)(n - 1);
  const int k_lo = (int)floorf(pos), k_hi = (int)ceilf(pos);
  float v[2];
  for (int which = 0; which < 2; ++which) {
    int k = which == 0 ? k_lo : k_hi;
    uint32_t prefix = 0, mask = 0;
    for (int pass = 3; pass >= 0; --pass) {
      for (int i = tid; i < 256; i += blockDim.x) hist[i] = 0;
      __syncthreads();
      for (int i = tid; i < n; i += blockDim.x) {
        const uint32_t key = keys[i];
        if ((key & mask) == prefix) atomicAdd(&hist[(key >> (8 * pass)) & 255u], 1u);
      }
      __syncthreads();
      if (tid == 0) {
        uint32_t cum = 0, b = 0;
        for (; b < 256; ++b) {
          if (cum + hist[b] > (uint32_t)k) break;
          cum += hist[b];
        }
        sel[0] = b; sel[1] = cum;
      }
      __syncthreads();
      prefix |= sel[0] << (8 * pass);
      mask |= 255u << (8 * pass);
      k -= (int)sel[1];
      __syncthreads();
    }
    v[which] = __uint_as_float(prefix);
  }
  if (tid == 0) {
    const float w = pos - (float)k_lo;
    const float q = v[0] + w * (v[1] - v[0]);
    thr[s] = fminf(fmaxf(q, lo), hi);
  }
}
int threshold_launch(const float* dec, const float* stat, float* thr, int S, int T, int L, int Lp, int dm, int nb, int ldd,
                     float ratio, float lo, float hi, cudaStream_t st) {
  MSMD_REQUIRE(ratio >= 0.f && ratio <= 1.f, "quantile() q values must be in the range [0, 1] (got %f)", ratio);
  const size_t smem = ((size_t)L * dm + 256 + 4) * sizeof(uint32_t);
  MSMD_REQUIRE(smem <= 48 * 1024, "threshold: %d values per sequence exceed the shared-memory tile", L * dm);
  threshold_kernel<<<S, 1024, smem, st>>>(dec, stat, thr, T, L, Lp, dm, nb, ldd, ratio, lo, hi);
  MSMD_CHECK_LAUNCH();
  return MSMD_OK;
}

__global__ void update_params_set_kernel(UpdateParams* dst, const UpdateParams src) { *dst = src; }
int update_params_set(UpdateParams* d_dst, const UpdateParams& p, cudaStream_t st) {
  update_params_set_kernel<<<1, 1, 0, st>>>(d_dst, p);
  MSMD_CHECK_LAUNCH();
  return MSMD_OK;
}
int update_launch(const UpdateParams* d_p, int NX, int L, int dm, cudaStream_t st) {
  (void)dm;
  ProfileScope prof("update", st);
  MSMD_CHECK_CUDA(launch_pdl(update_kernel, dim3(std::min(cdiv(NX * L, 8), kNumSMs * 2)), dim3(256), 0, st, d_p));
  MSMD_CHECK_LAUNCH();
  return MSMD_OK;
}

__global__ void steps_set_kernel(int* steps, int S, int v) {
  const int i = blockIdx.x * blockDim.x + threadIdx.x;
  if (i < S) steps[i] = v;
}
int steps_set(int* steps, int S, int value, cudaStream_t st) {
  steps_set_kernel<<<cdiv(S, 256), 256, 0, st>>>(steps, S, value);
  MSMD_CHECK_LAUNCH();
  return MSMD_OK;
}
__global__ void mix_static_kernel(const float* __restrict__ dec, const float* __restrict__ stat, float* __restrict__ out,
                                  int S, int T, int dm, int nb, int ldd) {
  const int64_t n_el = (int64_t)S * (T - 1) * dm;
  for (int64_t i = (int64_t)blockIdx.x * blockDim.x + threadIdx.x; i < n_el; i += (int64_t)gridDim.x * blockDim.x) {
    const int c = (int)(i % dm);
    const int tok = (int)((i / dm) % (T - 1));
    const int s = (int)(i / ((int64_t)dm * (T - 1)));
    const float* row = dec + ((int64_t)s * T + 1 + tok) * ldd;
    float v = row[c];
    const bool face = c < dm - 3;
    for (int b = 0; b < nb; ++b) v += (face ? row[dm + b] : 1.0f) * stat[((int64_t)s * nb + b) * dm + c];
    out[i] = v;
  }
}
int mix_static_launch(const float* dec, const float* stat, float* out, int S, int T, int dm, int nb, int ldd,
                      cudaStream_t st) {
  const int64_t n = (int64_t)S * (T - 1) * dm;
  mix_static_kernel<<<(int)std::min<int64_t>(cdiv(n, 256), kNumSMs * 8), 256, 0, st>>>(dec, stat, out, S, T, dm, nb, ldd);
  MSMD_CHECK_LAUNCH();
  return MSMD_OK;
}


__global__ void split_parts_kernel(const float* __restrict__ dec, const float* __restrict__ stat, float* __restrict__ dyn,
                                   float* __restrict__ sta, float* __restrict__ alphas, int S, int T, int dm, int nb, int ldd) {
  const int64_t rows = (int64_t)S * (T - 1);
  const int per_row = dm + nb * dm + nb;
  const int64_t n = rows * per_row;
  for (int64_t i = (int64_t)blockIdx.x * blockDim.x + threadIdx.x; i < n; i += (int64_t)gridDim.x * blockDim.x) {
    const int64_t r = i / per_row;
    const int k = (int)(i % per_row);
    const int s = (int)(r / (T - 1)), tok = (int)(r % (T - 1));
    const float* row = dec + ((int64_t)s * T + 1 + tok) * ldd;
    if (k < dm) dyn[r * dm + k] = row[k];
    else if (k < dm + nb * dm) sta[r * nb * dm + (k - dm)] = stat[(int64_t)s * nb * dm + (k - dm)];
    else alphas[r * nb + (k - dm - nb * dm)] = row[dm + (k - dm - nb * dm)];
  }
}
int split_parts_launch(const float* dec, const float* stat, float* dyn, float* sta, float* alphas, int S, int T, int dm,
                       int nb, int ldd, cudaStream_t st) {
  const int64_t n = (int64_t)S * (T - 1) * (dm + nb * dm + nb);
  split_parts_kernel<<<(int)std::min<int64_t>(cdiv(n, 256), kNumSMs * 8), 256, 0, st>>>(dec, stat, dyn, sta, alphas, S, T, dm,
                                                                                        nb, ldd);
  MSMD_CHECK_LAUNCH();
  return MSMD_OK;
}

}
```

### ubisoft-laforge-msmd_b200/csrc/gemm_tc.cu

```cuda
#include "gemm_tc.cuh"
#include "profile.cuh"
#include <cuda_fp16.h>
#include <algorithm>
#include <cudaTypedefs.h>
#include <mutex>
#include <cstdlib>
#include <cstring>
#include <vector>

namespace msmd {

static PFN_cuTensorMapEncodeTiled_v12000 get_encode() {
  static PFN_cuTensorMapEncodeTiled_v12000 fn = nullptr;
  static std::once_flag once;
  std::call_once(once, [] {
    void* p = nullptr;
    cudaDriverEntryPointQueryResult q;
    if (cudaGetDriverEntryPoint("cuTensorMapEncodeTiled", &p, cudaEnableDefault, &q) == cudaSuccess &&
        q == cudaDriverEntryPointSuccess)
      fn = reinterpret_cast<PFN_cuTensorMapEncodeTiled_v12000>(p);
  });
  return fn;
}

int make_tmap(CUtensorMap* out, const void* base, CUtensorMapDataType dt, int rank, const uint64_t* dims,
              const uint64_t* strides_bytes, const uint32_t* box, CUtensorMapSwizzle swz) {
  auto enc = get_encode();
  if (!enc) {
    set_error("cuTensorMapEncodeTiled entry point unavailable (driver too old?)");
    return MSMD_ERR_CUDA;
  }
  cuuint64_t gdim[5], gstr[4];
  cuuint32_t bx[5], es[5];
  for (int i = 0; i < rank; ++i) { gdim[i] = dims[i]; bx[i] = box[i]; es[i] = 1; }
  for (int i = 0; i + 1 < rank; ++i) gstr[i] = strides_bytes[i];
  if ((reinterpret_cast<uintptr_t>(base) & 15) != 0) {
    set_error("tensor map: base address %p is not 16-byte aligned", base);
    return MSMD_ERR_INVALID;
  }
  for (int i = 0; i + 1 < rank; ++i)
    if (gstr[i] % 16 != 0) {
      set_error("tensor map: stride %llu bytes is not a multiple of 16", (unsigned long long)gstr[i]);
      return MSMD_ERR_INVALID;
    }
  CUresult r = enc(out, dt, rank, const_cast<void*>(base), gdim, gstr, bx, es, CU_TENSOR_MAP_INTERLEAVE_NONE, swz,
                   CU_TENSOR_MAP_L2_PROMOTION_L2_256B, CU_TENSOR_MAP_FLOAT_OOB_FILL_NONE);
  if (r != CUDA_SUCCESS) {
    set_error("cuTensorMapEncodeTiled failed with CUresult %d (rank %d dims %llu,%llu box %u,%u)", (int)r, rank,
              (unsigned long long)gdim[0], (unsigned long long)(rank > 1 ? gdim[1] : 0), bx[0], rank > 1 ? bx[1] : 0);
    return MSMD_ERR_CUDA;
  }
  return MSMD_OK;
}

int make_tmap_2d(CUtensorMap* out, const void* base, CUtensorMapDataType dt, uint64_t inner, uint64_t outer,
                 uint64_t row_stride_bytes, uint32_t box_inner, uint32_t box_outer, CUtensorMapSwizzle swz) {
  uint64_t dims[2] = {inner, outer};
  uint64_t str[1] = {row_stride_bytes};
  uint32_t box[2] = {box_inner, box_outer};
  return make_tmap(out, base, dt, 2, dims, str, box, swz);
}

static int make_tmap_23(CUtensorMap* out, const void* base, CUtensorMapDataType dt, int esz, uint64_t inner,
                        uint64_t outer, int64_t row_stride, int batch, int64_t batch_stride, uint32_t box_inner,
                        uint32_t box_outer) {
  if (batch <= 1)
    return make_tmap_2d(out, base, dt, inner, outer, (uint64_t)row_stride * esz, box_inner, box_outer,
                        CU_TENSOR_MAP_SWIZZLE_128B);
  uint64_t dims[3] = {inner, outer, (uint64_t)batch};
  uint64_t str[2] = {(uint64_t)row_stride * esz, (uint64_t)batch_stride * esz};
  uint32_t box[3] = {box_inner, box_outer, 1};
  return make_tmap(out, base, dt, 3, dims, str, box, CU_TENSOR_MAP_SWIZZLE_128B);
}

template <class Cfg, int MODE, bool GELU>
static int launch_cfg2(const GemmDesc& d, cudaStream_t st) {
  GemmParams p;
  memset(&p, 0, sizeof(p));
  const auto in_dt = MODE == 0 ? CU_TENSOR_MAP_DATA_TYPE_BFLOAT16
                               : (MODE == 1 ? CU_TENSOR_MAP_DATA_TYPE_FLOAT32 : CU_TENSOR_MAP_DATA_TYPE_FLOAT16);
  const int esz = Cfg::ELT;
  int rc;
  if ((rc = make_tmap_23(&p.a_map, d.A, in_dt, esz, d.K, d.M, d.lda, d.batch, d.sA, Cfg::BK, Cfg::BM))) return rc;
  {
    const int wb = (d.batch > 1 && d.wz_mod != 0) ? (d.wz_mod > 0 ? d.wz_mod : d.batch) : 1;
    if ((rc = make_tmap_23(&p.b_map, d.W, in_dt, esz, d.K, d.N, d.ldw, wb, d.sW, Cfg::BK, Cfg::B_ROWS))) return rc;
  }
  if (Cfg::NSPLIT == 2) {
    MSMD_REQUIRE(d.A_lo && d.W_lo, "gemm: the three-pass modes need the lo operands");
    MSMD_REQUIRE(d.batch <= 1, "gemm: batched three-pass GEMMs are not implemented");
    if ((rc = make_tmap_23(&p.a_lo_map, d.A_lo, in_dt, esz, d.K, d.M, d.lda, 1, 0, Cfg::BK, Cfg::BM))) return rc;
    if ((rc = make_tmap_23(&p.b_lo_map, d.W_lo, in_dt, esz, d.K, d.N, d.ldw, 1, 0, Cfg::BK, Cfg::B_ROWS))) return rc;
  }
  using OutT = typename Cfg::OutT;
  using AuxT = typename Cfg::AuxT;
  const auto dt16 = MODE == 3 ? CU_TENSOR_MAP_DATA_TYPE_FLOAT16 : CU_TENSOR_MAP_DATA_TYPE_BFLOAT16;
  const auto out_dt = sizeof(OutT) == 2 ? dt16 : CU_TENSOR_MAP_DATA_TYPE_FLOAT32;
  if ((rc = make_tmap_23(&p.out_map, d.out, out_dt, sizeof(OutT), d.N, d.M, d.ldo, d.batch, d.sO, Cfg::OUT_COLS, 32)))
    return rc;
  if (Cfg::HAS_AUX) {
    const auto aux_dt = sizeof(AuxT) == 2 ? dt16 : CU_TENSOR_MAP_DATA_TYPE_FLOAT32;
    if ((rc = make_tmap_23(&p.aux_map, d.aux, aux_dt, sizeof(AuxT), d.N, d.M, d.ld_aux, d.batch, d.sAux,
                           Cfg::AUX_COLS, 32)))
      return rc;
  }
  p.bias = d.bias;
  p.M = d.M; p.N = d.N; p.K = d.K;
  p.act = d.act;
  p.batch = d.batch < 1 ? 1 : d.batch;
  p.wz_mod = d.wz_mod;
  p.bias_zstride = d.bias_zstride;
#ifdef MSMD_GEMM_TRACE
  static const bool env_trace = getenv("MSMD_GEMM_TRACE") != nullptr;
#else
  constexpr bool env_trace = false;
#endif
  static unsigned long long* trace_buf = nullptr;
  constexpr size_t kTraceN = (size_t)kNumSMs * 3 * 16 * 4;
  if (env_trace) {
    if (!trace_buf) MSMD_CHECK_CUDA(cudaMalloc(&trace_buf, kTraceN * 8));
    MSMD_CHECK_CUDA(cudaMemsetAsync(trace_buf, 0, kTraceN * 8, st));
    p.trace = trace_buf;
  }
  p.tiles_m = cdiv(d.M, Cfg::CTA2 ? 2 * Cfg::BM : Cfg::BM);
  p.tiles_n = cdiv(d.N, Cfg::BN);
  const int tiles = p.tiles_m * p.tiles_n * p.batch;
  auto kern = gemm_tc_kernel<Cfg, MODE, GELU>;
  static bool attr_set = false;
  if (!attr_set) {
    MSMD_CHECK_CUDA(cudaFuncSetAttribute(kern, cudaFuncAttributeMaxDynamicSharedMemorySize, Cfg::SMEM_BYTES));
    attr_set = true;
  }
  ProfileScope prof(MODE == 0 ? "gemm_bf16" : (MODE == 1 ? "gemm_tf32x3" : (MODE == 2 ? "gemm_fp16x3" : "gemm_fp16")), st);
  char shape_name[64];
  snprintf(shape_name, sizeof(shape_name), "gemm_%dx%dx%d%s", d.M, d.N, d.K, Cfg::CTA2 ? "_pair" : "");
  ProfileScope prof2(profiling_on() ? strdup(shape_name) : "", st);
  if constexpr (Cfg::CTA2) {
    const int sms = (d.max_ctas > 0 && d.max_ctas < kNumSMs) ? d.max_ctas : kNumSMs;
    int pairs = tiles < sms / 2 ? tiles : sms / 2;
    cudaLaunchConfig_t cfg = {};
    cfg.blockDim = dim3(Cfg::THREADS);
    cfg.dynamicSmemBytes = Cfg::SMEM_BYTES;
    cfg.stream = st;
    cudaLaunchAttribute attr[2];
    attr[0].id = cudaLaunchAttributeClusterDimension;
    attr[0].val.clusterDim.x = 2; attr[0].val.clusterDim.y = 1; attr[0].val.clusterDim.z = 1;
    static const int cl4_env = [] { const char* e = getenv("MSMD_GEMM_CL4"); return e ? atoi(e) : 1; }();
    if (cl4_env && Cfg::NSPLIT == 1 && p.tiles_n % 2 == 0 && d.max_ctas <= 0 && tiles >= 4) {
      static int max_cl4 = -1;
      if (max_cl4 < 0) {
        cfg.gridDim = dim3(kNumSMs / 4 * 4);
        attr[0].val.clusterDim.x = 4;
        cfg.attrs = attr;
        cfg.numAttrs = 1;
        int nc = 0;
        if (cudaOccupancyMaxActiveClusters(&nc, kern, &cfg) != cudaSuccess) { (void)cudaGetLastError(); nc = 0; }
        max_cl4 = nc < kNumSMs / 4 ? nc : kNumSMs / 4;
        attr[0].val.clusterDim.x = 2;
      }
      const int want = pairs / 2;
      const int cl = want < max_cl4 ? want : max_cl4;
      if (cl >= 1 && cdiv(tiles, 2 * cl) <= cdiv(tiles, pairs)) {
        if (make_tmap_23(&p.a_half_map, d.A, in_dt, esz, d.K, d.M, d.lda, 1, 0, Cfg::BK, Cfg::BM / 2)) return MSMD_ERR_CUDA;
        p.cl4 = 1;
        pairs = 2 * cl;
        attr[0].val.clusterDim.x = 4;
      }
    }
    cfg.gridDim = dim3(2 * pairs);
    attr[1].id = cudaLaunchAttributeProgrammaticStreamSerialization;
    attr[1].val.programmaticStreamSerializationAllowed = 1;
    cfg.attrs = attr;
    cfg.numAttrs = pdl_enabled() ? 2 : 1;
    MSMD_CHECK_CUDA(cudaLaunchKernelEx(&cfg, kern, p));
  } else {
    const int sms = (d.max_ctas > 0 && d.max_ctas < kNumSMs) ? d.max_ctas : kNumSMs;
    const int grid = tiles < sms ? tiles : sms;
    MSMD_CHECK_CUDA(launch_pdl(kern, dim3(grid), dim3(Cfg::THREADS), Cfg::SMEM_BYTES, st, p));
  }
  MSMD_CHECK_LAUNCH();
  if (env_trace) {
    static int dumps = 0;
    std::vector<unsigned long long> h(kTraceN);
    MSMD_CHECK_CUDA(cudaStreamSynchronize(st));
    MSMD_CHECK_CUDA(cudaMemcpy(h.data(), trace_buf, kTraceN * 8, cudaMemcpyDeviceToHost));
    if (dumps++ % 23 == 22) {
      for (int cta : {0, 1, 77}) {
        const unsigned long long t0 = h[((size_t)cta * 3 + 0) * 64 + 0];
        fprintf(stderr, "[trace] %s cta %d (cycles since the producer's first stamp)\n", shape_name, cta);
        const char* names[3] = {"tma  [start, slot0 free, last kb issued, -]", "mma  [start, acc free, first full, last issued]",
                                "epi0 [start, acc full, tmem drained, done]"};
        for (int role = 0; role < 3; ++role) {
          fprintf(stderr, "  %s\n", names[role]);
          for (int it = 0; it < 12; ++it) {
            const unsigned long long* e = &h[(((size_t)cta * 3 + role) * 16 + it) * 4];
            if (!e[0] && !e[1]) break;
            fprintf(stderr, "    tile %2d: %7lld %7lld %7lld %7lld\n", it, (long long)(e[0] - t0), (long long)(e[1] - t0),
                    (long long)(e[2] ? e[2] - t0 : 0), (long long)(e[3] ? e[3] - t0 : 0));
          }
        }
      }
    }
  }
  return MSMD_OK;
}

template <class Cfg, int MODE>
static int launch_cfg(const GemmDesc& d, cudaStream_t st) {
  return d.act ? launch_cfg2<Cfg, MODE, true>(d, st) : launch_cfg2<Cfg, MODE, false>(d, st);
}

template <int MODE, class H>
static int dispatch16(const GemmDesc& d, cudaStream_t st) {
  const bool aux = d.aux != nullptr;
  const bool narrow = d.N <= 128;
  static const int cta2_mode = [] { const char* e = getenv("MSMD_GEMM_CTA2"); return e ? atoi(e) : 1; }();
  const bool cta2_env = cta2_mode != 0;
  const bool pair = d.cta2 == 1 || (d.cta2 < 0 && cta2_env && !aux && !d.out_f32 && d.batch <= 1 && d.N >= 256 &&
                                    d.M >= 2048);
  const bool epi8 = d.gelu_heavy != 0;
  if (pair) {
    if (epi8) return launch_cfg<GemmCfg<MODE, 256, 8, false, H, H, true>, MODE>(d, st);
    return launch_cfg<GemmCfg<MODE, 256, 4, false, H, H, true>, MODE>(d, st);
  }
  if (!aux && !d.out_f32 && d.batch <= 1 && d.M <= 512 && d.N >= 256)
    return launch_cfg<GemmCfg<MODE, 64, 4, false, H, H>, MODE>(d, st);
  if (!aux) {
    if (d.out_f32) {
      return narrow ? launch_cfg<GemmCfg<MODE, 128, 4, false, float, float>, MODE>(d, st)
                    : launch_cfg<GemmCfg<MODE, 256, 4, false, float, float>, MODE>(d, st);
    }
    if (epi8 && !narrow) return launch_cfg<GemmCfg<MODE, 256, 8, false, H, H>, MODE>(d, st);
    return narrow ? launch_cfg<GemmCfg<MODE, 128, 4, false, H, H>, MODE>(d, st)
                  : launch_cfg<GemmCfg<MODE, 256, 4, false, H, H>, MODE>(d, st);
  }
  if constexpr (MODE == 0) {
    if (d.out_f32 && !d.aux_f32) return launch_cfg<GemmCfg<0, 256, 4, true, float, H>, 0>(d, st);
    if (d.out_f32 && d.aux_f32) return launch_cfg<GemmCfg<0, 256, 4, true, float, float>, 0>(d, st);
    if (!d.out_f32 && !d.aux_f32) return launch_cfg<GemmCfg<0, 256, 4, true, H, H>, 0>(d, st);
    set_error("gemm: bf16 output with fp32 aux is not instantiated");
    return MSMD_ERR_UNSUPPORTED;
  } else {
    set_error("gemm: the one-pass fp16 mode has no residual (aux) epilogue");
    return MSMD_ERR_UNSUPPORTED;
  }
}

int gemm_tc_launch(const GemmDesc& d, cudaStream_t st) {
  MSMD_REQUIRE(d.M > 0 && d.N > 0 && d.K > 0, "gemm: empty problem %dx%dx%d", d.M, d.N, d.K);
  MSMD_REQUIRE(d.A && d.W && d.out, "gemm: null operand");
  const bool aux = d.aux != nullptr;
  if (d.mode == 0) return dispatch16<0, __nv_bfloat16>(d, st);
  if (d.mode == 3) return dispatch16<3, __half>(d, st);
  MSMD_REQUIRE(d.mode == 1 || d.mode == 2, "gemm: unknown mode %d", d.mode);
  MSMD_REQUIRE(d.out_f32 && (!aux || d.aux_f32), "gemm: the three-pass modes are fp32 out");
  if (d.mode == 2) {
    static const bool cta2_env2 = [] { const char* e = getenv("MSMD_GEMM_CTA2"); return !e || atoi(e) != 0; }();
    if (aux) return launch_cfg<GemmCfg<2, 128, 4, true, float, float>, 2>(d, st);
    if (d.cta2 != 0 && cta2_env2 && d.batch <= 1 && d.N >= 256 && d.M >= 2048)
      return launch_cfg<GemmCfg<2, 128, 4, false, float, float, true>, 2>(d, st);
    return launch_cfg<GemmCfg<2, 128, 4, false, float, float>, 2>(d, st);
  }
  if (aux) return launch_cfg<GemmCfg<1, 128, 4, true, float, float>, 1>(d, st);
  return launch_cfg<GemmCfg<1, 128, 4, false, float, float>, 1>(d, st);
}

__global__ void split_tf32_kernel(const float* __restrict__ x, float* __restrict__ hi, float* __restrict__ lo, int64_t n) {
  for (int64_t i = (int64_t)blockIdx.x * blockDim.x + threadIdx.x; i < n; i += (int64_t)gridDim.x * blockDim.x) {
    const float v = x[i];
    const float h = __uint_as_float(__float_as_uint(v) & 0xffffe000u);
    hi[i] = h;
    lo[i] = v - h;
  }
}

__global__ void split_f16_kernel(const float* __restrict__ x, __half* __restrict__ hi, __half* __restrict__ lo, int64_t n,
                                 int* __restrict__ overflow) {
  bool bad = false;
  for (int64_t i = (int64_t)blockIdx.x * blockDim.x + threadIdx.x; i < n; i += (int64_t)gridDim.x * blockDim.x) {
    const float v = x[i];
    const __half h = __float2half_rn(v);
    hi[i] = h;
    lo[i] = __float2half_rn((v - __half2float(h)) * 2048.0f);
    bad |= !(fabsf(v) <= 65504.0f);
  }
  if (bad && overflow) *overflow = 1;
}
int split_f16(const float* x, __half* hi, __half* lo, int64_t n, cudaStream_t st, int* overflow) {
  if (n == 0) return MSMD_OK;
  ProfileScope prof("split_f16", st);
  const int blocks = (int)std::min<int64_t>(cdiv(n, 256), kNumSMs * 16);
  split_f16_kernel<<<blocks, 256, 0, st>>>(x, hi, lo, n, overflow);
  MSMD_CHECK_LAUNCH();
  return MSMD_OK;
}

int split_tf32(const float* x, float* hi, float* lo, int64_t n, cudaStream_t st) {
  if (n == 0) return MSMD_OK;
  const int blocks = (int)std::min<int64_t>((n + 255) / 256, (int64_t)kNumSMs * 8);
  split_tf32_kernel<<<blocks, 256, 0, st>>>(x, hi, lo, n);
  MSMD_CHECK_LAUNCH();
  return MSMD_OK;
}

}

using namespace msmd;

extern "C" int msmd_linear(int mode, const void* x, const void* x_lo, const void* w, const void* w_lo,
                           const float* bias, const void* aux, void* out, int M, int N, int K, int64_t ldx,
                           int64_t ldw, int64_t ldo, int64_t ld_aux, int out_f32, int aux_f32, int act, void* stream) {
  GemmDesc d;
  d.mode = mode; d.A = x; d.A_lo = x_lo; d.W = w; d.W_lo = w_lo; d.bias = bias; d.aux = aux; d.out = out;
  d.M = M; d.N = N; d.K = K; d.lda = ldx; d.ldw = ldw; d.ldo = ldo; d.ld_aux = ld_aux;
  d.out_f32 = out_f32; d.aux_f32 = aux_f32; d.act = act & 1; d.gelu_heavy = (act & 1);
  return gemm_tc_launch(d, static_cast<cudaStream_t>(stream));
}

extern "C" int msmd_split_f16(const float* x, void* hi, void* lo, int64_t n, void* stream) {
  MSMD_REQUIRE(n >= 0, "msmd_split_f16: negative count");
  MSMD_REQUIRE(n == 0 || (x && hi && lo), "msmd_split_f16: null pointer");
  return split_f16(x, static_cast<__half*>(hi), static_cast<__half*>(lo), n, static_cast<cudaStream_t>(stream), nullptr);
}

extern "C" int msmd_split_tf32(const float* x, float* hi, float* lo, int64_t n, void* stream) {
  MSMD_REQUIRE(n >= 0, "msmd_split_tf32: negative count");
  MSMD_REQUIRE(n == 0 || (x && hi && lo), "msmd_split_tf32: null pointer");
  return split_tf32(x, hi, lo, n, static_cast<cudaStream_t>(stream));
}
```

### ubisoft-laforge-msmd_b200/csrc/gemm_tc.cuh

```cuda
#pragma once
#include "common.cuh"
#include "tc_common.cuh"
#include <cuda_bf16.h>
#include <cuda_fp16.h>

namespace msmd {

struct GemmParams {
  CUtensorMap a_map, b_map;
  CUtensorMap a_lo_map, b_lo_map;
  CUtensorMap out_map;
  CUtensorMap aux_map;
  CUtensorMap a_half_map;
  int cl4;
  const float* bias;
  int M, N, K;
  int act;
  int batch;
  int wz_mod;
  int bias_zstride;
  int tiles_m, tiles_n;
  unsigned long long* trace;
};

template <int MODE, int BN_, int EPI_WARPS_, bool HAS_AUX_, typename OutT_, typename AuxT_, bool CTA2_ = false, int OUT_BUFS_ = 2>
struct GemmCfg {
  static constexpr int OUT_BUFS = OUT_BUFS_;
  static constexpr bool CTA2 = CTA2_;
  using OutT = OutT_;
  using AuxT = AuxT_;
  static constexpr int BN = BN_, EPI_WARPS = EPI_WARPS_;
  static constexpr bool HAS_AUX = HAS_AUX_;
  static constexpr int BM = 128;
  static constexpr int ELT = MODE == 1 ? 4 : 2;
  static constexpr int BK = 128 / ELT;
  static constexpr int UK = 32 / ELT;
  static constexpr int B_ROWS = CTA2 ? BN / 2 : BN;
  static constexpr int A_BYTES = BM * 128, B_BYTES = B_ROWS * 128;
  static constexpr int UMMA_M = CTA2 ? 256 : 128;
  static constexpr int NSPLIT = (MODE == 0 || MODE == 3) ? 1 : 2;
  static constexpr int STAGE_BYTES = NSPLIT * (A_BYTES + B_BYTES);
  static constexpr int OUT_COLS = 128 / (int)sizeof(OutT);
  static constexpr int AUX_COLS = 128 / (int)sizeof(AuxT);
  static constexpr int EPI_WARP_BYTES = OUT_BUFS * 4096 + (HAS_AUX ? 8192 : 0);
  static constexpr int EPI_BYTES = EPI_WARPS * EPI_WARP_BYTES;
  static constexpr int BAR_BYTES = 256 + 2 * 256 * 4;
  static constexpr int ALIGN_SLACK = 512;
  static constexpr int BUDGET = 227 * 1024 - ALIGN_SLACK - BAR_BYTES;
  static constexpr int STAGES_RAW = (BUDGET - EPI_BYTES) / STAGE_BYTES;
  static constexpr int STAGES = STAGES_RAW > 6 ? 6 : STAGES_RAW;
  static constexpr int SMEM_BYTES = ALIGN_SLACK + STAGES * STAGE_BYTES + EPI_BYTES + BAR_BYTES;
  static constexpr int THREADS = 64 + 32 * EPI_WARPS;
  static constexpr int ACC_COLS = NSPLIT * BN;
  static constexpr int TMEM_NEED = 2 * ACC_COLS;
  static constexpr int TMEM_COLS = (TMEM_NEED <= 32) ? 32 : (TMEM_NEED <= 64) ? 64 : (TMEM_NEED <= 128) ? 128 : (TMEM_NEED <= 256) ? 256 : 512;
  static constexpr int COL_SPLIT = EPI_WARPS / 4;
  static constexpr int COLS_PER_WARP = BN / COL_SPLIT;
  static_assert(EPI_WARPS == 4 || EPI_WARPS == 8, "epilogue warps must cover the 4 TMEM lane quarters");
  static_assert(BN % 32 == 0 && BN <= 256 && TMEM_NEED <= 512, "BN");
  static_assert(COLS_PER_WARP % 64 == 0, "the epilogue processes 32-column chunks in pairs");
  static_assert(SMEM_BYTES <= 227 * 1024, "shared memory budget");
  static_assert(STAGES >= 2, "not enough shared memory for a pipeline");
  static_assert(!CTA2 || (MODE != 1 && !HAS_AUX && BN % 32 == 0), "CTA-pair variant: 16-bit operands, no aux");
};

__device__ __forceinline__ float erf_fast(float x) {
  const float ax = fabsf(x);
  const float t = __fdividef(1.0f, fmaf(0.3275911f, ax, 1.0f));
  float p = fmaf(1.061405429f, t, -1.453152027f);
  p = fmaf(p, t, 1.421413741f);
  p = fmaf(p, t, -0.284496736f);
  p = fmaf(p, t, 0.254829592f);
  const float r = 1.0f - p * t * __expf(-ax * ax);
  return copysignf(r, x);
}
__device__ __forceinline__ float gelu_tanh3(float x) {
  const float x2 = fminf(x * x, 64.0f);
  const float u = x * fmaf(x2, fmaf(x2, -0.000351516788570472f, 0.037005646019657945f), 0.7975078842869763f);
  float th;
  asm("tanh.approx.f32 %0, %1;" : "=f"(th) : "f"(u));
  const float hx = 0.5f * x;
  return fmaf(hx, th, hx);
}
template <int MODE>
__device__ __forceinline__ float gelu_erf(float x) {
  if constexpr (MODE == 0) return gelu_tanh3(x);
  else if constexpr (MODE == 3) return 0.5f * x * (1.0f + erf_fast(x * 0.70710678118654752f));
  else return 0.5f * x * (1.0f + erff(x * 0.70710678118654752f));
}
template <class T> struct is_half_t { static constexpr bool value = false; };
template <> struct is_half_t<__half> { static constexpr bool value = true; };
template <class T>
__device__ __forceinline__ uint32_t pack16x2(float a, float b) {
  if constexpr (is_half_t<T>::value) {
    __half2 h = __floats2half2_rn(a, b);
    return *reinterpret_cast<uint32_t*>(&h);
  } else {
    __nv_bfloat162 h = __floats2bfloat162_rn(a, b);
    return *reinterpret_cast<uint32_t*>(&h);
  }
}
template <class T>
__device__ __forceinline__ float2 unpack16x2(uint32_t w) {
  if constexpr (is_half_t<T>::value) return __half22float2(*reinterpret_cast<const __half2*>(&w));
  else return make_float2(__uint_as_float(w << 16), __uint_as_float(w & 0xffff0000u));
}

__device__ __forceinline__ void trace_stamp(unsigned long long* tr, int role, int it, int ev) {
#ifdef MSMD_GEMM_TRACE
  if (tr != nullptr && it < 16) tr[((blockIdx.x * 3 + role) * 16 + it) * 4 + ev] = clock64();
#endif
}

template <class Cfg, int MODE, bool GELU>
__global__ void __launch_bounds__(Cfg::THREADS, 1) gemm_tc_kernel(const __grid_constant__ GemmParams p) {
  using namespace tc;
  using OutT = typename Cfg::OutT;
  using AuxT = typename Cfg::AuxT;
  constexpr int BM = Cfg::BM, BN = Cfg::BN, BK = Cfg::BK, STAGES = Cfg::STAGES;
  extern __shared__ uint8_t smem_raw[];
  uint8_t* smem = reinterpret_cast<uint8_t*>((reinterpret_cast<uintptr_t>(smem_raw) + 1023) & ~uintptr_t(1023));
  uint8_t* stage_base = smem;
  uint8_t* epi_base = smem + STAGES * Cfg::STAGE_BYTES;
  uint64_t* bars = reinterpret_cast<uint64_t*>(epi_base + Cfg::EPI_BYTES);
  uint64_t* full_bar = bars;
  uint64_t* empty_bar = bars + STAGES;
  uint64_t* tfull_bar = bars + 2 * STAGES;
  uint64_t* tempty_bar = bars + 2 * STAGES + 2;
  uint64_t* aux_bar = bars + 2 * STAGES + 4;
  uint32_t* tmem_slot = reinterpret_cast<uint32_t*>(bars + 2 * STAGES + 4 + 2 * Cfg::EPI_WARPS);
  float* bias_tile = reinterpret_cast<float*>(reinterpret_cast<uint8_t*>(bars) + 256);
  static_assert((2 * Cfg::STAGES + 4 + 2 * Cfg::EPI_WARPS) * 8 + 4 <= 256, "barrier block overflows its 256 bytes");
  if (threadIdx.x == 0 && reinterpret_cast<uint8_t*>(bias_tile) + 2 * 256 * 4 > smem_raw + Cfg::SMEM_BYTES) __trap();

  griddep_launch();
  const int warp = threadIdx.x >> 5, lane = threadIdx.x & 31;
  const int crank = Cfg::CTA2 ? (int)cluster_ctarank() : 0;
  const int cta_rank = crank & 1;
  const bool cl4 = Cfg::CTA2 && p.cl4 != 0;
  const uint16_t pair_mask = (uint16_t)(3u << (crank & ~1));
  const int tile0 = Cfg::CTA2 ? (int)blockIdx.x / 2 : (int)blockIdx.x;
  const int tstride = Cfg::CTA2 ? (int)gridDim.x / 2 : (int)gridDim.x;
  const int num_tiles = p.tiles_m * p.tiles_n * p.batch;
  const int num_kb = (p.K + BK - 1) / BK;

  if (warp == 0 && lane == 0) {
    prefetch_tmap(&p.a_map);
    prefetch_tmap(&p.b_map);
    prefetch_tmap(&p.out_map);
    if (Cfg::NSPLIT == 2) { prefetch_tmap(&p.a_lo_map); prefetch_tmap(&p.b_lo_map); }
    if (cl4) prefetch_tmap(&p.a_half_map);
    if (Cfg::HAS_AUX) prefetch_tmap(&p.aux_map);
    for (int s = 0; s < STAGES; ++s) { mbar_init(&full_bar[s], 1); mbar_init(&empty_bar[s], cl4 ? 2 : 1); }
    for (int a = 0; a < 2; ++a) { mbar_init(&tfull_bar[a], 1); mbar_init(&tempty_bar[a], Cfg::EPI_WARPS * (Cfg::CTA2 ? 2 : 1)); }
    for (int i = 0; i < 2 * Cfg::EPI_WARPS; ++i) mbar_init(&aux_bar[i], 1);
    fence_barrier_init();
  }
  if (warp == 1) {
    if constexpr (Cfg::CTA2) tmem_alloc_2sm(tmem_slot, Cfg::TMEM_COLS);
    else tmem_alloc(tmem_slot, Cfg::TMEM_COLS);
  }
  tc_fence_before();
  if constexpr (Cfg::CTA2) cluster_sync();
  else __syncthreads();
  tc_fence_after();
  const uint32_t tmem_base = *tmem_slot;
  griddep_wait();

  auto tile_coords = [&](int t, int& m0, int& n0, int& z) {
    const int per_z = p.tiles_m * p.tiles_n;
    z = t / per_z;
    const int r = t - z * per_z;
    m0 = (r / p.tiles_n) * (Cfg::CTA2 ? 2 * BM : BM) + cta_rank * BM;
    n0 = (r % p.tiles_n) * BN;
  };

  if (warp == 0) {
    int s = 0;
    uint32_t ph = 0;
    int pit = 0;
    for (int t = tile0; t < num_tiles; t += tstride, ++pit) {
      int m0, n0, z;
      tile_coords(t, m0, n0, z);
      for (int kb = 0; kb < num_kb; ++kb) {
        if (lane == 0) {
          if (kb == 0) trace_stamp(p.trace, 0, pit, 0);
          mbar_wait(&empty_bar[s], ph ^ 1);
          if (kb == 0) trace_stamp(p.trace, 0, pit, 1);
          if (kb == num_kb - 1) trace_stamp(p.trace, 0, pit, 2);
          uint8_t* sa = stage_base + s * Cfg::STAGE_BYTES;
          uint8_t* sb = sa + Cfg::NSPLIT * Cfg::A_BYTES;
          if constexpr (Cfg::CTA2) {
            if (cta_rank == 0) mbar_expect_tx(&full_bar[s], 2 * Cfg::STAGE_BYTES);
            if (cl4) {
              const int j = crank >> 1;
              tma_load_2d_2sm_mc(sa + j * (Cfg::A_BYTES / 2), &p.a_half_map, &full_bar[s], kb * BK, m0 + j * (BM / 2),
                                 (uint16_t)(5u << cta_rank));
            } else {
              tma_load_2d_2sm(sa, &p.a_map, &full_bar[s], kb * BK, m0);
            }
            tma_load_2d_2sm(sb, &p.b_map, &full_bar[s], kb * BK, n0 + cta_rank * Cfg::B_ROWS);
            if (Cfg::NSPLIT == 2) {
              tma_load_2d_2sm(sa + Cfg::A_BYTES, &p.a_lo_map, &full_bar[s], kb * BK, m0);
              tma_load_2d_2sm(sb + Cfg::B_BYTES, &p.b_lo_map, &full_bar[s], kb * BK, n0 + cta_rank * Cfg::B_ROWS);
            }
          } else if (p.batch > 1) {
            mbar_expect_tx(&full_bar[s], Cfg::STAGE_BYTES);
            tma_load_3d(sa, &p.a_map, &full_bar[s], kb * BK, m0, z);
            if (p.wz_mod == 0) tma_load_2d(sb, &p.b_map, &full_bar[s], kb * BK, n0);
            else tma_load_3d(sb, &p.b_map, &full_bar[s], kb * BK, n0, p.wz_mod > 0 ? z % p.wz_mod : z);
          } else {
            mbar_expect_tx(&full_bar[s], Cfg::STAGE_BYTES);
            tma_load_2d(sa, &p.a_map, &full_bar[s], kb * BK, m0);
            tma_load_2d(sb, &p.b_map, &full_bar[s], kb * BK, n0);
            if (Cfg::NSPLIT == 2) {
              tma_load_2d(sa + Cfg::A_BYTES, &p.a_lo_map, &full_bar[s], kb * BK, m0);
              tma_load_2d(sb + Cfg::B_BYTES, &p.b_lo_map, &full_bar[s], kb * BK, n0);
            }
          }
        }
        __syncwarp();
        if (++s == STAGES) { s = 0; ph ^= 1; }
      }
    }
  } else if (warp == 1) {
    constexpr uint32_t idesc = make_idesc(MODE == 0 ? 1 : (MODE == 1 ? 2 : 0), Cfg::UMMA_M, BN);
    int s = 0;
    uint32_t ph = 0;
    int it = 0;
    for (int t = (Cfg::CTA2 && cta_rank != 0) ? num_tiles : tile0; t < num_tiles; t += tstride, ++it) {
      const int a = it & 1;
      const uint32_t aph = (it >> 1) & 1;
      const uint32_t d_tmem = tmem_base + a * Cfg::ACC_COLS;
      if (lane == 0) {
        trace_stamp(p.trace, 1, it, 0);
        mbar_wait(&tempty_bar[a], aph ^ 1);
        tc_fence_after();
        trace_stamp(p.trace, 1, it, 1);
      }
      __syncwarp();
      for (int kb = 0; kb < num_kb; ++kb) {
        if (lane == 0) {
          mbar_wait(&full_bar[s], ph);
          tc_fence_after();
          if (kb == 0) trace_stamp(p.trace, 1, it, 2);
          const uint32_t sa = smem_u32(stage_base + s * Cfg::STAGE_BYTES);
          const uint32_t sb = sa + Cfg::NSPLIT * Cfg::A_BYTES;
          const uint64_t da = make_smem_desc_sw128(sa), db = make_smem_desc_sw128(sb);
#pragma unroll
          for (int k = 0; k < BK / Cfg::UK; ++k) {
            const uint32_t acc = (kb | k) != 0;
            if constexpr (Cfg::NSPLIT == 1) {
              if constexpr (Cfg::CTA2) umma_2sm(d_tmem, desc_advance(da, k * 32), desc_advance(db, k * 32), idesc, acc);
              else umma<0>(d_tmem, desc_advance(da, k * 32), desc_advance(db, k * 32), idesc, acc);
            } else {
              const uint64_t dal = make_smem_desc_sw128(sa + Cfg::A_BYTES), dbl = make_smem_desc_sw128(sb + Cfg::B_BYTES);
              constexpr int KIND = MODE == 1 ? 1 : 0;
              if constexpr (Cfg::CTA2) {
                umma_2sm(d_tmem + BN, desc_advance(dal, k * 32), desc_advance(db, k * 32), idesc, acc);
                umma_2sm(d_tmem + BN, desc_advance(da, k * 32), desc_advance(dbl, k * 32), idesc, 1u);
                umma_2sm(d_tmem, desc_advance(da, k * 32), desc_advance(db, k * 32), idesc, acc);
              } else {
                umma<KIND>(d_tmem + BN, desc_advance(dal, k * 32), desc_advance(db, k * 32), idesc, acc);
                umma<KIND>(d_tmem + BN, desc_advance(da, k * 32), desc_advance(dbl, k * 32), idesc, 1u);
                umma<KIND>(d_tmem, desc_advance(da, k * 32), desc_advance(db, k * 32), idesc, acc);
              }
            }
          }
          if constexpr (Cfg::CTA2) umma_commit_2sm(&empty_bar[s], cl4 ? (uint16_t)0xF : pair_mask);
          else umma_commit(&empty_bar[s]);
        }
        __syncwarp();
        if (++s == STAGES) { s = 0; ph ^= 1; }
      }
      if (lane == 0) trace_stamp(p.trace, 1, it, 3);
      if (lane == 0) {
        if constexpr (Cfg::CTA2) umma_commit_2sm(&tfull_bar[a], pair_mask);
        else umma_commit(&tfull_bar[a]);
      }
      __syncwarp();
    }
  } else {
    const int e = warp - 2;
    const int q = warp & 3;
    const int csplit = e / 4;
    uint8_t* my = epi_base + e * Cfg::EPI_WARP_BYTES;
    uint8_t* out_stage = my;
    uint8_t* aux_stage = my + Cfg::OUT_BUFS * 4096;
    uint64_t* my_aux_bar = aux_bar + 2 * e;
    constexpr int CPW = Cfg::COLS_PER_WARP;
    constexpr int AUX_PER_TILE = Cfg::HAS_AUX ? CPW / Cfg::AUX_COLS : 1;
    constexpr int EPI_THREADS = 32 * Cfg::EPI_WARPS;
    const int swz = lane & 7;
    const int etid = threadIdx.x - 64;

    auto issue_aux = [&](int f) {
      if constexpr (Cfg::HAS_AUX) {
        const int lt = f / AUX_PER_TILE, ck = f % AUX_PER_TILE;
        const int t = tile0 + lt * tstride;
        if (t < num_tiles && lane == 0) {
          int m0, n0, z;
          tile_coords(t, m0, n0, z);
          const int b = f & 1;
          mbar_expect_tx(&my_aux_bar[b], 4096);
          const int c0 = n0 + csplit * CPW + ck * Cfg::AUX_COLS;
          if (p.batch > 1) tma_load_3d(aux_stage + b * 4096, &p.aux_map, &my_aux_bar[b], c0, m0 + q * 32, z);
          else tma_load_2d(aux_stage + b * 4096, &p.aux_map, &my_aux_bar[b], c0, m0 + q * 32);
        }
      }
    };
    int af = 0;
    int so = 0;
    issue_aux(0);

    constexpr int BPT = (BN + EPI_THREADS - 1) / EPI_THREADS;
    float bnext[BPT];
    auto fetch_bias = [&](int t) {
      if (t < num_tiles) {
        int m0, n0, z;
        tile_coords(t, m0, n0, z);
        const float* bias_z = p.bias + (p.wz_mod > 0 ? (z % p.wz_mod) * p.bias_zstride : 0);
#pragma unroll
        for (int i = 0; i < BPT; ++i) {
          const int col = etid + i * EPI_THREADS;
          bnext[i] = (p.bias != nullptr && col < BN && n0 + col < p.N) ? __ldg(bias_z + n0 + col) : 0.f;
        }
      }
    };
    fetch_bias(tile0);

    int it = 0;
    for (int t = tile0; t < num_tiles; t += tstride, ++it) {
      int m0, n0, z;
      tile_coords(t, m0, n0, z);
      const int a = it & 1;
      const uint32_t aph = (it >> 1) & 1;
      float* sb = bias_tile + a * BN;
#pragma unroll
      for (int i = 0; i < BPT; ++i) {
        const int col = etid + i * EPI_THREADS;
        if (col < BN) sb[col] = bnext[i];
      }
      asm volatile("bar.sync 1, %0;" ::"n"(EPI_THREADS) : "memory");
      fetch_bias(t + tstride);
      if (e == 0 && lane == 0) trace_stamp(p.trace, 2, it, 0);
      mbar_wait(&tfull_bar[a], aph);
      tc_fence_after();
      if (e == 0 && lane == 0) trace_stamp(p.trace, 2, it, 1);
      const uint32_t t_addr = tmem_base + ((uint32_t)(q * 32) << 16) + a * Cfg::ACC_COLS + csplit * CPW;
      const float* sbw = sb + csplit * CPW;

      auto process = [&](uint32_t (&raw)[32], uint32_t (&raw2)[Cfg::NSPLIT == 2 ? 32 : 1], int c) {
        const uint8_t* aux_buf = nullptr;
        int aux_off = 0;
        if constexpr (Cfg::HAS_AUX) {
          if (c % Cfg::AUX_COLS == 0) {
            __syncwarp();
            issue_aux(af + 1);
            mbar_wait(&my_aux_bar[af & 1], (af >> 1) & 1);
          }
          aux_buf = aux_stage + (af & 1) * 4096 + lane * 128;
          aux_off = (c % Cfg::AUX_COLS) * (int)sizeof(AuxT) / 16;
        }
        float v[32];
#pragma unroll
        for (int j = 0; j < 8; ++j) {
          const float4 b4 = *reinterpret_cast<const float4*>(sbw + c + 4 * j);
          v[4 * j + 0] = __uint_as_float(raw[4 * j + 0]) + b4.x;
          v[4 * j + 1] = __uint_as_float(raw[4 * j + 1]) + b4.y;
          v[4 * j + 2] = __uint_as_float(raw[4 * j + 2]) + b4.z;
          v[4 * j + 3] = __uint_as_float(raw[4 * j + 3]) + b4.w;
        }
        if constexpr (MODE == 1) {
#pragma unroll
          for (int j = 0; j < 32; ++j) v[j] += __uint_as_float(raw2[j]);
        }
        if constexpr (MODE == 2) {
#pragma unroll
          for (int j = 0; j < 32; ++j) v[j] = fmaf(__uint_as_float(raw2[j]), 1.0f / 2048.0f, v[j]);
        }
        if constexpr (GELU) {
#pragma unroll
          for (int j = 0; j < 32; ++j) v[j] = gelu_erf<MODE>(v[j]);
        }
        if constexpr (Cfg::HAS_AUX) {
          if constexpr (sizeof(AuxT) == 4) {
#pragma unroll
            for (int j = 0; j < 8; ++j) {
              const float4 r4 = *reinterpret_cast<const float4*>(aux_buf + (((aux_off + j) ^ swz) << 4));
              v[4 * j + 0] += r4.x; v[4 * j + 1] += r4.y; v[4 * j + 2] += r4.z; v[4 * j + 3] += r4.w;
            }
          } else {
#pragma unroll
            for (int j = 0; j < 4; ++j) {
              const uint4 r4 = *reinterpret_cast<const uint4*>(aux_buf + (((aux_off + j) ^ swz) << 4));
              const uint32_t w[4] = {r4.x, r4.y, r4.z, r4.w};
#pragma unroll
              for (int u = 0; u < 4; ++u) {
                const float2 f2 = unpack16x2<AuxT>(w[u]);
                v[8 * j + 2 * u + 0] += f2.x;
                v[8 * j + 2 * u + 1] += f2.y;
              }
            }
          }
          if ((c + 32) % Cfg::AUX_COLS == 0) ++af;
        }
        const int o_off = (c % Cfg::OUT_COLS) * (int)sizeof(OutT) / 16;
        if (c % Cfg::OUT_COLS == 0) {
          if (lane == 0) tma_store_wait_read<Cfg::OUT_BUFS - 1>();
          __syncwarp();
        }
        uint8_t* obuf = out_stage + (so % Cfg::OUT_BUFS) * 4096;
        uint8_t* orow = obuf + lane * 128;
        if constexpr (sizeof(OutT) == 4) {
#pragma unroll
          for (int j = 0; j < 8; ++j)
            *reinterpret_cast<float4*>(orow + (((o_off + j) ^ swz) << 4)) =
                make_float4(v[4 * j], v[4 * j + 1], v[4 * j + 2], v[4 * j + 3]);
        } else {
#pragma unroll
          for (int j = 0; j < 4; ++j) {
            uint32_t w[4];
#pragma unroll
            for (int u = 0; u < 4; ++u) w[u] = pack16x2<OutT>(v[8 * j + 2 * u], v[8 * j + 2 * u + 1]);
            *reinterpret_cast<uint4*>(orow + (((o_off + j) ^ swz) << 4)) = make_uint4(w[0], w[1], w[2], w[3]);
          }
        }
        if ((c + 32) % Cfg::OUT_COLS == 0) {
          fence_proxy_async_smem();
          __syncwarp();
          if (lane == 0) {
            const int c0 = n0 + csplit * CPW + (c / Cfg::OUT_COLS) * Cfg::OUT_COLS;
            if (p.batch > 1) tma_store_3d(&p.out_map, obuf, c0, m0 + q * 32, z);
            else tma_store_2d(&p.out_map, obuf, c0, m0 + q * 32);
            tma_store_commit();
          }
          ++so;
        }
      };

      auto release_acc = [&]() {
        if (e == 0 && lane == 0) trace_stamp(p.trace, 2, it, 2);
        tc_fence_before();
        __syncwarp();
        if (lane == 0) {
          if (Cfg::CTA2 && cta_rank != 0) mbar_arrive_cluster(&tempty_bar[a], crank & ~1);
          else mbar_arrive(&tempty_bar[a]);
        }
      };
      if constexpr (Cfg::NSPLIT == 2) {
        uint32_t rA[32], rB[32], rA2[32], rB2[32];
        tmem_ld32(t_addr, rA);
        tmem_ld32(t_addr + BN, rA2);
#pragma unroll 1
        for (int c = 0; c < CPW; c += 64) {
          tmem_ld_wait();
          tmem_ld32(t_addr + c + 32, rB);
          tmem_ld32(t_addr + BN + c + 32, rB2);
          process(rA, rA2, c);
          tmem_ld_wait();
          if (c + 64 < CPW) {
            tmem_ld32(t_addr + c + 64, rA);
            tmem_ld32(t_addr + BN + c + 64, rA2);
          } else {
            release_acc();
          }
          process(rB, rB2, c + 32);
        }
      } else {
        uint32_t r0[32], r1[32], r2[32], r3[32];
        uint32_t none[1];
        tmem_ld32(t_addr, r0);
        tmem_ld32(t_addr + 32, r1);
#pragma unroll 1
        for (int c = 0; c < CPW; c += 128) {
          tmem_ld_wait();
          const bool more = c + 64 < CPW;
          if (more) {
            tmem_ld32(t_addr + c + 64, r2);
            tmem_ld32(t_addr + c + 96, r3);
          } else {
            release_acc();
          }
          process(r0, none, c);
          process(r1, none, c + 32);
          if (more) {
            tmem_ld_wait();
            if (c + 128 < CPW) {
              tmem_ld32(t_addr + c + 128, r0);
              tmem_ld32(t_addr + c + 160, r1);
            } else {
              release_acc();
            }
            process(r2, none, c + 64);
            process(r3, none, c + 96);
          }
        }
      }
      if (e == 0 && lane == 0) trace_stamp(p.trace, 2, it, 3);
    }
    if (lane == 0) tma_store_wait<0>();
  }

  tc_fence_before();
  if constexpr (Cfg::CTA2) cluster_sync();
  else __syncthreads();
  if (warp == 1) {
    tc_fence_after();
    if constexpr (Cfg::CTA2) tmem_dealloc_2sm(tmem_base, Cfg::TMEM_COLS);
    else tmem_dealloc(tmem_base, Cfg::TMEM_COLS);
  }
}

struct GemmDesc {
  int mode = 0;
  const void* A = nullptr;
  const void* A_lo = nullptr;
  const void* W = nullptr;
  const void* W_lo = nullptr;
  const float* bias = nullptr;
  const void* aux = nullptr;
  void* out = nullptr;
  int M = 0, N = 0, K = 0;
  int64_t lda = 0, ldw = 0, ldo = 0, ld_aux = 0;
  int out_f32 = 0, aux_f32 = 0;
  int act = 0;
  int batch = 1;
  int64_t sA = 0, sW = 0, sO = 0, sAux = 0;
  int wz_mod = -1;
  int bias_zstride = 0;
  int gelu_heavy = 0;
  int cta2 = -1;
  int max_ctas = 0;
};

int gemm_tc_launch(const GemmDesc& d, cudaStream_t st);
int split_f16(const float* x, __half* hi, __half* lo, int64_t n, cudaStream_t st, int* overflow = nullptr);

}
```

### ubisoft-laforge-msmd_b200/csrc/tc_common.cuh

```cuda
#pragma once
#include <cuda.h>
#include <cuda_runtime.h>
#include <cstdint>

namespace msmd {
namespace tc {

__device__ __forceinline__ uint32_t smem_u32(const void* p) { return (uint32_t)__cvta_generic_to_shared(p); }

__device__ __forceinline__ bool elect_one() {
  uint32_t pred;
  asm volatile(
      "{\n\t.reg .pred p;\n\telect.sync _|p, 0xffffffff;\n\tselp.u32 %0, 1, 0, p;\n\t}"
      : "=r"(pred));
  return pred != 0;
}

__device__ __forceinline__ void mbar_init(uint64_t* bar, uint32_t count) {
  asm volatile("mbarrier.init.shared::cta.b64 [%0], %1;" ::"r"(smem_u32(bar)), "r"(count) : "memory");
}
__device__ __forceinline__ void fence_barrier_init() {
  asm volatile("fence.mbarrier_init.release.cluster;" ::: "memory");
}
__device__ __forceinline__ void mbar_expect_tx(uint64_t* bar, uint32_t bytes) {
  asm volatile("mbarrier.arrive.expect_tx.shared::cta.b64 _, [%0], %1;" ::"r"(smem_u32(bar)), "r"(bytes) : "memory");
}
__device__ __forceinline__ void mbar_arrive(uint64_t* bar) {
  asm volatile("mbarrier.arrive.shared::cta.b64 _, [%0];" ::"r"(smem_u32(bar)) : "memory");
}
__device__ __forceinline__ bool mbar_try_wait(uint64_t* bar, uint32_t parity) {
  uint32_t ok;
  asm volatile(
      "{\n\t.reg .pred p;\n\t"
      "mbarrier.try_wait.parity.shared::cta.b64 p, [%1], %2;\n\t"
      "selp.u32 %0, 1, 0, p;\n\t}"
      : "=r"(ok)
      : "r"(smem_u32(bar)), "r"(parity)
      : "memory");
  return ok != 0;
}
__device__ __forceinline__ void mbar_wait(uint64_t* bar, uint32_t parity) {
  while (!mbar_try_wait(bar, parity)) {
  }
}

__device__ __forceinline__ void prefetch_tmap(const CUtensorMap* m) {
  asm volatile("prefetch.tensormap [%0];" ::"l"(reinterpret_cast<uint64_t>(m)) : "memory");
}
__device__ __forceinline__ void tma_load_2d(void* smem_dst, const CUtensorMap* map, uint64_t* bar, int c0, int c1) {
  asm volatile(
      "cp.async.bulk.tensor.2d.shared::cluster.global.mbarrier::complete_tx::bytes [%0], [%1, {%3, %4}], [%2];"
      ::"r"(smem_u32(smem_dst)), "l"(reinterpret_cast<uint64_t>(map)), "r"(smem_u32(bar)), "r"(c0), "r"(c1)
      : "memory");
}
__device__ __forceinline__ void tma_load_3d(void* smem_dst, const CUtensorMap* map, uint64_t* bar, int c0, int c1,
                                            int c2) {
  asm volatile(
      "cp.async.bulk.tensor.3d.shared::cluster.global.mbarrier::complete_tx::bytes [%0], [%1, {%3, %4, %5}], [%2];"
      ::"r"(smem_u32(smem_dst)), "l"(reinterpret_cast<uint64_t>(map)), "r"(smem_u32(bar)), "r"(c0), "r"(c1), "r"(c2)
      : "memory");
}
__device__ __forceinline__ void tma_store_2d(const CUtensorMap* map, const void* smem_src, int c0, int c1) {
  asm volatile("cp.async.bulk.tensor.2d.global.shared::cta.bulk_group [%0, {%2, %3}], [%1];"
               ::"l"(reinterpret_cast<uint64_t>(map)), "r"(smem_u32(smem_src)), "r"(c0), "r"(c1)
               : "memory");
}
__device__ __forceinline__ void tma_store_3d(const CUtensorMap* map, const void* smem_src, int c0, int c1, int c2) {
  asm volatile("cp.async.bulk.tensor.3d.global.shared::cta.bulk_group [%0, {%2, %3, %4}], [%1];"
               ::"l"(reinterpret_cast<uint64_t>(map)), "r"(smem_u32(smem_src)), "r"(c0), "r"(c1), "r"(c2)
               : "memory");
}
__device__ __forceinline__ void tma_store_commit() { asm volatile("cp.async.bulk.commit_group;" ::: "memory"); }
template <int N>
__device__ __forceinline__ void tma_store_wait_read() {
  asm volatile("cp.async.bulk.wait_group.read %0;" ::"n"(N) : "memory");
}
template <int N>
__device__ __forceinline__ void tma_store_wait() {
  asm volatile("cp.async.bulk.wait_group %0;" ::"n"(N) : "memory");
}
__device__ __forceinline__ void fence_proxy_async_smem() { asm volatile("fence.proxy.async.shared::cta;" ::: "memory"); }

__device__ __forceinline__ void tmem_alloc(uint32_t* smem_dst, uint32_t ncols) {
  asm volatile("tcgen05.alloc.cta_group::1.sync.aligned.shared::cta.b32 [%0], %1;" ::"r"(smem_u32(smem_dst)), "r"(ncols)
               : "memory");
  asm volatile("tcgen05.relinquish_alloc_permit.cta_group::1.sync.aligned;" ::: "memory");
}
__device__ __forceinline__ void tmem_dealloc(uint32_t taddr, uint32_t ncols) {
  asm volatile("tcgen05.dealloc.cta_group::1.sync.aligned.b32 %0, %1;" ::"r"(taddr), "r"(ncols) : "memory");
}
__device__ __forceinline__ void tc_fence_before() { asm volatile("tcgen05.fence::before_thread_sync;" ::: "memory"); }
__device__ __forceinline__ void tc_fence_after() { asm volatile("tcgen05.fence::after_thread_sync;" ::: "memory"); }

template <int KIND>
__device__ __forceinline__ void umma(uint32_t tmem_d, uint64_t desc_a, uint64_t desc_b, uint32_t idesc, uint32_t accum) {
  if constexpr (KIND == 0) {
    asm volatile(
        "{\n\t.reg .pred p;\n\tsetp.ne.b32 p, %4, 0;\n\t"
        "tcgen05.mma.cta_group::1.kind::f16 [%0], %1, %2, %3, p;\n\t}"
        ::"r"(tmem_d), "l"(desc_a), "l"(desc_b), "r"(idesc), "r"(accum)
        : "memory");
  } else {
    asm volatile(
        "{\n\t.reg .pred p;\n\tsetp.ne.b32 p, %4, 0;\n\t"
        "tcgen05.mma.cta_group::1.kind::tf32 [%0], %1, %2, %3, p;\n\t}"
        ::"r"(tmem_d), "l"(desc_a), "l"(desc_b), "r"(idesc), "r"(accum)
        : "memory");
  }
}
__device__ __forceinline__ void umma_commit(uint64_t* bar) {
  asm volatile("tcgen05.commit.cta_group::1.mbarrier::arrive::one.shared::cluster.b64 [%0];" ::"r"(smem_u32(bar))
               : "memory");
}

__device__ __forceinline__ void tmem_ld32(uint32_t taddr, uint32_t* v) {
  asm volatile(
      "tcgen05.ld.sync.aligned.32x32b.x32.b32 "
      "{%0, %1, %2, %3, %4, %5, %6, %7, %8, %9, %10, %11, %12, %13, %14, %15, "
      "%16, %17, %18, %19, %20, %21, %22, %23, %24, %25, %26, %27, %28, %29, %30, %31}, [%32];"
      : "=r"(v[0]), "=r"(v[1]), "=r"(v[2]), "=r"(v[3]), "=r"(v[4]), "=r"(v[5]), "=r"(v[6]), "=r"(v[7]), "=r"(v[8]),
        "=r"(v[9]), "=r"(v[10]), "=r"(v[11]), "=r"(v[12]), "=r"(v[13]), "=r"(v[14]), "=r"(v[15]), "=r"(v[16]),
        "=r"(v[17]), "=r"(v[18]), "=r"(v[19]), "=r"(v[20]), "=r"(v[21]), "=r"(v[22]), "=r"(v[23]), "=r"(v[24]),
        "=r"(v[25]), "=r"(v[26]), "=r"(v[27]), "=r"(v[28]), "=r"(v[29]), "=r"(v[30]), "=r"(v[31])
      : "r"(taddr)
      : "memory");
}
__device__ __forceinline__ void tmem_ld_wait() { asm volatile("tcgen05.wait::ld.sync.aligned;" ::: "memory"); }

__device__ __forceinline__ uint32_t cluster_ctarank() {
  uint32_t r;
  asm volatile("mov.u32 %0, %%cluster_ctarank;" : "=r"(r));
  return r;
}
__device__ __forceinline__ void cluster_sync() {
  asm volatile("barrier.cluster.arrive.release.aligned;" ::: "memory");
  asm volatile("barrier.cluster.wait.acquire.aligned;" ::: "memory");
}
__device__ __forceinline__ void tma_load_2d_2sm(void* smem_dst, const CUtensorMap* map, uint64_t* bar, int c0, int c1) {
  asm volatile(
      "cp.async.bulk.tensor.2d.cta_group::2.shared::cluster.global.mbarrier::complete_tx::bytes [%0], [%1, {%3, %4}], [%2];"
      ::"r"(smem_u32(smem_dst)), "l"(reinterpret_cast<uint64_t>(map)), "r"(smem_u32(bar) & 0xFEFFFFFFu), "r"(c0), "r"(c1)
      : "memory");
}
__device__ __forceinline__ void tma_load_2d_2sm_mc(void* smem_dst, const CUtensorMap* map, uint64_t* bar, int c0, int c1,
                                                   uint16_t cta_mask) {
  asm volatile(
      "cp.async.bulk.tensor.2d.cta_group::2.shared::cluster.global.mbarrier::complete_tx::bytes.multicast::cluster"
      " [%0], [%1, {%3, %4}], [%2], %5;"
      ::"r"(smem_u32(smem_dst)), "l"(reinterpret_cast<uint64_t>(map)), "r"(smem_u32(bar) & 0xFEFFFFFFu), "r"(c0), "r"(c1),
        "h"(cta_mask)
      : "memory");
}
__device__ __forceinline__ void tmem_alloc_2sm(uint32_t* smem_dst, uint32_t ncols) {
  asm volatile("tcgen05.alloc.cta_group::2.sync.aligned.shared::cta.b32 [%0], %1;" ::"r"(smem_u32(smem_dst)), "r"(ncols)
               : "memory");
  asm volatile("tcgen05.relinquish_alloc_permit.cta_group::2.sync.aligned;" ::: "memory");
}
__device__ __forceinline__ void tmem_dealloc_2sm(uint32_t taddr, uint32_t ncols) {
  asm volatile("tcgen05.dealloc.cta_group::2.sync.aligned.b32 %0, %1;" ::"r"(taddr), "r"(ncols) : "memory");
}
__device__ __forceinline__ void umma_2sm(uint32_t tmem_d, uint64_t desc_a, uint64_t desc_b, uint32_t idesc, uint32_t accum) {
  asm volatile(
      "{\n\t.reg .pred p;\n\tsetp.ne.b32 p, %4, 0;\n\t"
      "tcgen05.mma.cta_group::2.kind::f16 [%0], %1, %2, %3, p;\n\t}"
      ::"r"(tmem_d), "l"(desc_a), "l"(desc_b), "r"(idesc), "r"(accum)
      : "memory");
}
__device__ __forceinline__ void umma_2sm_tf32(uint32_t tmem_d, uint64_t desc_a, uint64_t desc_b, uint32_t idesc, uint32_t accum) {
  asm volatile(
      "{\n\t.reg .pred p;\n\tsetp.ne.b32 p, %4, 0;\n\t"
      "tcgen05.mma.cta_group::2.kind::tf32 [%0], %1, %2, %3, p;\n\t}"
      ::"r"(tmem_d), "l"(desc_a), "l"(desc_b), "r"(idesc), "r"(accum)
      : "memory");
}
__device__ __forceinline__ void umma_commit_2sm(uint64_t* bar, uint16_t cta_mask = 3) {
  asm volatile("tcgen05.commit.cta_group::2.mbarrier::arrive::one.shared::cluster.multicast::cluster.b64 [%0], %1;"
               ::"r"(smem_u32(bar)), "h"(cta_mask)
               : "memory");
}
__device__ __forceinline__ void mbar_arrive_cluster(uint64_t* bar, uint32_t rank) {
  asm volatile(
      "{\n\t.reg .b32 ra;\n\tmapa.shared::cluster.u32 ra, %0, %1;\n\t"
      "mbarrier.arrive.shared::cluster.b64 _, [ra];\n\t}"
      ::"r"(smem_u32(bar)), "r"(rank)
      : "memory");
}

__device__ __forceinline__ uint64_t make_smem_desc_sw128(uint32_t smem_addr) {
  uint64_t d = 0;
  d |= (uint64_t)((smem_addr & 0x3FFFF) >> 4);
  d |= (uint64_t)1 << 16;
  d |= (uint64_t)(1024 >> 4) << 32;
  d |= (uint64_t)1 << 46;
  d |= (uint64_t)2 << 61;
  return d;
}
__device__ __forceinline__ uint64_t make_smem_desc_sw64(uint32_t smem_addr) {
  uint64_t d = 0;
  d |= (uint64_t)((smem_addr & 0x3FFFF) >> 4);
  d |= (uint64_t)1 << 16;
  d |= (uint64_t)(512 >> 4) << 32;
  d |= (uint64_t)1 << 46;
  d |= (uint64_t)4 << 61;
  return d;
}
__device__ __forceinline__ uint64_t desc_advance(uint64_t d, uint32_t bytes) { return d + (uint64_t)(bytes >> 4); }

__host__ __device__ constexpr uint32_t make_idesc(int fmt, int M, int N) {
  return (1u << 4) | ((uint32_t)fmt << 7) | ((uint32_t)fmt << 10) | ((uint32_t)(N >> 3) << 17) |
         ((uint32_t)(M >> 4) << 24);
}

}

int make_tmap(CUtensorMap* out, const void* base, CUtensorMapDataType dt, int rank, const uint64_t* dims,
              const uint64_t* strides_bytes, const uint32_t* box, CUtensorMapSwizzle swz);
int make_tmap_2d(CUtensorMap* out, const void* base, CUtensorMapDataType dt, uint64_t inner, uint64_t outer,
                 uint64_t row_stride_bytes, uint32_t box_inner, uint32_t box_outer, CUtensorMapSwizzle swz);

}
```

Baseline: 230.7.

## Fuse residual-add LayerNorm into FFN down-projection GEMM epilogue via cluster exchange

Adds a LayerNorm epilogue to the CTA-pair tcgen05 GEMM used for the FFN second projection. Each CTA holds half of the 512 columns in TMEM, adds bias and the residual (loaded by TMA), and computes partial mean and M2. It swaps those partials with its peer CTA through st.async to cluster shared memory, then normalizes and writes the result back into x. This removes the separate LN3 kernel launch and the round trip of y through global memory. In exchange it adds cluster synchronization and extra TMEM passes, and it falls back to the unfused LN when the 4-CTA cluster layout is not chosen. It also deletes the unused multi-row LN kernel variants.

```diff
diff --git a/ubisoft-laforge-msmd_b200/csrc/denoiser.cu b/ubisoft-laforge-msmd_b200/csrc/denoiser.cu
--- a/ubisoft-laforge-msmd_b200/csrc/denoiser.cu
+++ b/ubisoft-laforge-msmd_b200/csrc/denoiser.cu
@@ -116,6 +116,18 @@
   return gemm_tc_launch(d, st);
 }
 
+int gemm_ln(int fmt, const bf16* A, int64_t lda, const void* W, int64_t ldw, const float* bias, const LnParams& l, int K,
+            cudaStream_t st) {
+  GemmDesc d;
+  d.mode = fmt ? 3 : 0; d.A = A; d.W = W; d.bias = bias; d.out = const_cast<bf16*>(l.y);
+  d.M = l.M; d.N = l.d; d.K = K; d.lda = lda; d.ldw = ldw; d.ldo = l.d;
+  d.ln_x = l.out; d.ln_g = l.g1; d.ln_b = l.b1;
+  bool fused = false;
+  int rc;
+  if ((rc = gemm_tc_launch(d, st, &fused))) return rc;
+  return fused ? MSMD_OK : ln_launch(l, st);
+}
+
 int up_split(msmd_model* m, __half** hi, __half** lo, const float* h, size_t n, bool want_lo) {
   std::vector<__half> a(n), b(want_lo ? n : 0);
   for (size_t i = 0; i < n; ++i) {
@@ -229,12 +241,11 @@
       if ((rc = ln_row0_launch(m->y0, m->x0c, w.g2, w.be2, m->x, nullptr, S, T, d, fmt, st))) return rc;
     }
     if ((rc = gemm(fmt, m->x, d, W1, d, w.b1, nullptr, 0, m->h, c.d_ff, 0, M, c.d_ff, d, 1, st))) return rc;
-    if ((rc = gemm(fmt, m->h, c.d_ff, W2, c.d_ff, w.b2, nullptr, 0, m->y, d, 0, M, d, c.d_ff, 0, st))) return rc;
     LnParams l3{};
     l3.resid = m->x;
     l3.y = m->y; l3.g1 = w.g3; l3.b1 = w.be3; l3.add = nullptr; l3.g2 = nullptr; l3.b2 = nullptr; l3.out = m->x;
     l3.x0 = nullptr; l3.skip_tok0 = 0; l3.M = M; l3.T = T; l3.d = d; l3.fp16 = fmt;
-    if ((rc = ln_launch(l3, st))) return rc;
+    if ((rc = gemm_ln(fmt, m->h, c.d_ff, W2, c.d_ff, w.b2, l3, c.d_ff, st))) return rc;
   }
   const void *Wd1 = fmt ? (const void*)m->Wd1_h : m->Wd1, *Wd2 = fmt ? (const void*)m->Wd2_h : m->Wd2;
   if ((rc = gemm(fmt, m->x, d, Wd1, d, m->bd1, nullptr, 0, m->dec1, d / 2, 0, M, d / 2, d, 1, st))) return rc;
diff --git a/ubisoft-laforge-msmd_b200/csrc/denoiser_kernels.cu b/ubisoft-laforge-msmd_b200/csrc/denoiser_kernels.cu
--- a/ubisoft-laforge-msmd_b200/csrc/denoiser_kernels.cu
+++ b/ubisoft-laforge-msmd_b200/csrc/denoiser_kernels.cu
@@ -382,95 +382,6 @@
   else { v[0] = a.x; v[1] = a.y; v[2] = b.x; v[3] = b.y; }
 }
 
-template <bool F16>
-__device__ __forceinline__ void ln_unpack8(const uint4& u, float* v, bool add) {
-  const float2 a = unpack_h<F16>(u.x), b = unpack_h<F16>(u.y), c = unpack_h<F16>(u.z), d = unpack_h<F16>(u.w);
-  if (add) { v[0] += a.x; v[1] += a.y; v[2] += b.x; v[3] += b.y; v[4] += c.x; v[5] += c.y; v[6] += d.x; v[7] += d.y; }
-  else { v[0] = a.x; v[1] = a.y; v[2] = b.x; v[3] = b.y; v[4] = c.x; v[5] = c.y; v[6] = d.x; v[7] = d.y; }
-}
-template <bool F16>
-__device__ __forceinline__ uint4 ln_pack8(const float* v) {
-  return make_uint4(pack_h<F16>(v[0], v[1]), pack_h<F16>(v[2], v[3]), pack_h<F16>(v[4], v[5]), pack_h<F16>(v[6], v[7]));
-}
-__device__ __forceinline__ void ln16(float (&v)[16], const float* __restrict__ sg, const float* __restrict__ sb, int lane) {
-  float s = 0.f;
-#pragma unroll
-  for (int i = 0; i < 16; ++i) s += v[i];
-  const float mean = warp_sum(s) * (1.0f / 512.0f);
-  float q = 0.f;
-#pragma unroll
-  for (int i = 0; i < 16; ++i) { v[i] -= mean; q = fmaf(v[i], v[i], q); }
-  const float rstd = rsqrtf(warp_sum(q) * (1.0f / 512.0f) + 1e-5f);
-#pragma unroll
-  for (int h = 0; h < 2; ++h) {
-    const float4 g0 = *reinterpret_cast<const float4*>(sg + h * 256 + lane * 8), g1 = *reinterpret_cast<const float4*>(sg + h * 256 + lane * 8 + 4);
-    const float4 b0 = *reinterpret_cast<const float4*>(sb + h * 256 + lane * 8), b1 = *reinterpret_cast<const float4*>(sb + h * 256 + lane * 8 + 4);
-    float* w = v + 8 * h;
-    w[0] = fmaf(w[0] * rstd, g0.x, b0.x); w[1] = fmaf(w[1] * rstd, g0.y, b0.y); w[2] = fmaf(w[2] * rstd, g0.z, b0.z); w[3] = fmaf(w[3] * rstd, g0.w, b0.w);
-    w[4] = fmaf(w[4] * rstd, g1.x, b1.x); w[5] = fmaf(w[5] * rstd, g1.y, b1.y); w[6] = fmaf(w[6] * rstd, g1.z, b1.z); w[7] = fmaf(w[7] * rstd, g1.w, b1.w);
-  }
-}
-
-template <int D, bool F16, int kLnRows>
-__global__ void __launch_bounds__(256) ln_kernel(LnParams p) {
-  static_assert(D == 512, "lane layout: two 8-element chunks per lane");
-  griddep_launch();
-  __shared__ __align__(16) float sgb[4][D];
-  for (int i = threadIdx.x; i < D; i += blockDim.x) {
-    sgb[0][i] = p.g1[i]; sgb[1][i] = p.b1[i];
-    sgb[2][i] = p.g2 ? p.g2[i] : 0.f; sgb[3][i] = p.b2 ? p.b2[i] : 0.f;
-  }
-  griddep_wait();
-  __syncthreads();
-  const int lane = threadIdx.x & 31;
-  const int row0 = (blockIdx.x * (blockDim.x >> 5) + (threadIdx.x >> 5)) * kLnRows;
-  const int c0 = lane * 8, c1 = 256 + lane * 8;
-  struct Raw { uint4 y0, y1, r0, r1, a0, a1; };
-  auto load = [&](int row, Raw& w) {
-    if (row >= p.M) return;
-    const bf16* y = p.y + (int64_t)row * D;
-    w.y0 = *reinterpret_cast<const uint4*>(y + c0); w.y1 = *reinterpret_cast<const uint4*>(y + c1);
-    if (p.resid != nullptr) {
-      const bf16* r = p.resid + (int64_t)row * D;
-      w.r0 = *reinterpret_cast<const uint4*>(r + c0); w.r1 = *reinterpret_cast<const uint4*>(r + c1);
-    }
-    const int s = row / p.T, tok = row - s * p.T;
-    if (p.add != nullptr && tok > 0) {
-      const bf16* a = p.add + ((int64_t)s * (p.T - 1) + (tok - 1)) * D;
-      w.a0 = __ldg(reinterpret_cast<const uint4*>(a + c0)); w.a1 = __ldg(reinterpret_cast<const uint4*>(a + c1));
-    }
-  };
-  Raw cur, nxt;
-  load(row0, cur);
-#pragma unroll
-  for (int i = 0; i < kLnRows; ++i) {
-    const int row = row0 + i;
-    if (i + 1 < kLnRows) load(row + 1, nxt);
-    if (row < p.M) {
-      const int s = row / p.T, tok = row - s * p.T;
-      float v[16];
-      ln_unpack8<F16>(cur.y0, v, false); ln_unpack8<F16>(cur.y1, v + 8, false);
-      if (p.resid != nullptr) {
-        ln_unpack8<F16>(cur.r0, v, true); ln_unpack8<F16>(cur.r1, v + 8, true);
-      }
-      if (!(tok == 0 && p.skip_tok0)) {
-        ln16(v, sgb[0], sgb[1], lane);
-        if (tok == 0 && p.x0 != nullptr) {
-          bf16* o = p.x0 + (int64_t)s * D;
-          *reinterpret_cast<uint4*>(o + c0) = ln_pack8<F16>(v); *reinterpret_cast<uint4*>(o + c1) = ln_pack8<F16>(v + 8);
-        } else {
-          if (p.add != nullptr && tok > 0) {
-            ln_unpack8<F16>(cur.a0, v, true); ln_unpack8<F16>(cur.a1, v + 8, true);
-            ln16(v, sgb[2], sgb[3], lane);
-          }
-          bf16* o = p.out + (int64_t)row * D;
-          *reinterpret_cast<uint4*>(o + c0) = ln_pack8<F16>(v); *reinterpret_cast<uint4*>(o + c1) = ln_pack8<F16>(v + 8);
-        }
-      }
-    }
-    cur = nxt;
-  }
-}
 template <int D, bool F16>
 __global__ void __launch_bounds__(256) ln_kernel_v1(LnParams p) {
   griddep_launch();
@@ -510,16 +421,7 @@
 int ln_launch(const LnParams& p, cudaStream_t st) {
   MSMD_REQUIRE(p.d == 512, "ln: only d_model = 512 is instantiated (got %d)", p.d);
   ProfileScope prof(p.add ? "ln1_ln2" : "ln3", st);
-  static const int rows = [] { const char* e = getenv("MSMD_LN_ROWS"); return e ? atoi(e) : 0; }();
-  if (rows == 0) {
-    MSMD_CHECK_CUDA(launch_pdl(p.fp16 ? ln_kernel_v1<512, true> : ln_kernel_v1<512, false>, dim3(cdiv(p.M, 8)), dim3(256), 0, st, p));
-  } else if (rows == 1 || p.M <= 148 * 3 * 8) {
-    MSMD_CHECK_CUDA(launch_pdl(p.fp16 ? ln_kernel<512, true, 1> : ln_kernel<512, false, 1>, dim3(cdiv(p.M, 8)), dim3(256), 0, st, p));
-  } else if (rows == 4 || p.M < 148 * 3 * 8 * 4) {
-    MSMD_CHECK_CUDA(launch_pdl(p.fp16 ? ln_kernel<512, true, 4> : ln_kernel<512, false, 4>, dim3(cdiv(p.M, 8 * 4)), dim3(256), 0, st, p));
-  } else {
-    MSMD_CHECK_CUDA(launch_pdl(p.fp16 ? ln_kernel<512, true, 6> : ln_kernel<512, false, 6>, dim3(cdiv(p.M, 8 * 6)), dim3(256), 0, st, p));
-  }
+  MSMD_CHECK_CUDA(launch_pdl(p.fp16 ? ln_kernel_v1<512, true> : ln_kernel_v1<512, false>, dim3(cdiv(p.M, 8)), dim3(256), 0, st, p));
   MSMD_CHECK_LAUNCH();
   return MSMD_OK;
 }
diff --git a/ubisoft-laforge-msmd_b200/csrc/gemm_tc.cu b/ubisoft-laforge-msmd_b200/csrc/gemm_tc.cu
--- a/ubisoft-laforge-msmd_b200/csrc/gemm_tc.cu
+++ b/ubisoft-laforge-msmd_b200/csrc/gemm_tc.cu
@@ -73,7 +73,9 @@
   return make_tmap(out, base, dt, 3, dims, str, box, CU_TENSOR_MAP_SWIZZLE_128B);
 }
 
-template <class Cfg, int MODE, bool GELU>
+constexpr int kLnUnfused = 1;
+
+template <class Cfg, int MODE, bool GELU, bool LN = false>
 static int launch_cfg2(const GemmDesc& d, cudaStream_t st) {
   GemmParams p;
   memset(&p, 0, sizeof(p));
@@ -96,7 +98,8 @@
   using AuxT = typename Cfg::AuxT;
   const auto dt16 = MODE == 3 ? CU_TENSOR_MAP_DATA_TYPE_FLOAT16 : CU_TENSOR_MAP_DATA_TYPE_BFLOAT16;
   const auto out_dt = sizeof(OutT) == 2 ? dt16 : CU_TENSOR_MAP_DATA_TYPE_FLOAT32;
-  if ((rc = make_tmap_23(&p.out_map, d.out, out_dt, sizeof(OutT), d.N, d.M, d.ldo, d.batch, d.sO, Cfg::OUT_COLS, 32)))
+  if ((rc = make_tmap_23(&p.out_map, LN ? d.ln_x : d.out, out_dt, sizeof(OutT), d.N, d.M, LN ? d.N : d.ldo, d.batch, d.sO,
+                         Cfg::OUT_COLS, 32)))
     return rc;
   if (Cfg::HAS_AUX) {
     const auto aux_dt = sizeof(AuxT) == 2 ? dt16 : CU_TENSOR_MAP_DATA_TYPE_FLOAT32;
@@ -110,6 +113,7 @@
   p.batch = d.batch < 1 ? 1 : d.batch;
   p.wz_mod = d.wz_mod;
   p.bias_zstride = d.bias_zstride;
+  p.ln_g = d.ln_g; p.ln_b = d.ln_b;
 #ifdef MSMD_GEMM_TRACE
   static const bool env_trace = getenv("MSMD_GEMM_TRACE") != nullptr;
 #else
@@ -125,16 +129,15 @@
   p.tiles_m = cdiv(d.M, Cfg::CTA2 ? 2 * Cfg::BM : Cfg::BM);
   p.tiles_n = cdiv(d.N, Cfg::BN);
   const int tiles = p.tiles_m * p.tiles_n * p.batch;
-  auto kern = gemm_tc_kernel<Cfg, MODE, GELU>;
+  auto kern = gemm_tc_kernel<Cfg, MODE, GELU, LN>;
   static bool attr_set = false;
   if (!attr_set) {
     MSMD_CHECK_CUDA(cudaFuncSetAttribute(kern, cudaFuncAttributeMaxDynamicSharedMemorySize, Cfg::SMEM_BYTES));
     attr_set = true;
   }
-  ProfileScope prof(MODE == 0 ? "gemm_bf16" : (MODE == 1 ? "gemm_tf32x3" : (MODE == 2 ? "gemm_fp16x3" : "gemm_fp16")), st);
   char shape_name[64];
-  snprintf(shape_name, sizeof(shape_name), "gemm_%dx%dx%d%s", d.M, d.N, d.K, Cfg::CTA2 ? "_pair" : "");
-  ProfileScope prof2(profiling_on() ? strdup(shape_name) : "", st);
+  snprintf(shape_name, sizeof(shape_name), "gemm_%dx%dx%d%s%s", d.M, d.N, d.K, Cfg::CTA2 ? "_pair" : "",
+           LN ? "_ln" : "");
   if constexpr (Cfg::CTA2) {
     const int sms = (d.max_ctas > 0 && d.max_ctas < kNumSMs) ? d.max_ctas : kNumSMs;
     int pairs = tiles < sms / 2 ? tiles : sms / 2;
@@ -167,6 +170,9 @@
         attr[0].val.clusterDim.x = 4;
       }
     }
+    if (LN && !p.cl4) return kLnUnfused;
+    ProfileScope prof(LN ? "gemm_ln3" : (MODE == 0 ? "gemm_bf16" : (MODE == 2 ? "gemm_fp16x3" : "gemm_fp16")), st);
+    ProfileScope prof2(profiling_on() ? strdup(shape_name) : "", st);
     cfg.gridDim = dim3(2 * pairs);
     attr[1].id = cudaLaunchAttributeProgrammaticStreamSerialization;
     attr[1].val.programmaticStreamSerializationAllowed = 1;
@@ -174,6 +180,8 @@
     cfg.numAttrs = pdl_enabled() ? 2 : 1;
     MSMD_CHECK_CUDA(cudaLaunchKernelEx(&cfg, kern, p));
   } else {
+    ProfileScope prof(MODE == 0 ? "gemm_bf16" : (MODE == 1 ? "gemm_tf32x3" : (MODE == 2 ? "gemm_fp16x3" : "gemm_fp16")), st);
+    ProfileScope prof2(profiling_on() ? strdup(shape_name) : "", st);
     const int sms = (d.max_ctas > 0 && d.max_ctas < kNumSMs) ? d.max_ctas : kNumSMs;
     const int grid = tiles < sms ? tiles : sms;
     MSMD_CHECK_CUDA(launch_pdl(kern, dim3(grid), dim3(Cfg::THREADS), Cfg::SMEM_BYTES, st, p));
@@ -211,7 +219,7 @@
 }
 
 template <int MODE, class H>
-static int dispatch16(const GemmDesc& d, cudaStream_t st) {
+static int dispatch16(const GemmDesc& d, cudaStream_t st, bool* ln_fused) {
   const bool aux = d.aux != nullptr;
   const bool narrow = d.N <= 128;
   static const int cta2_mode = [] { const char* e = getenv("MSMD_GEMM_CTA2"); return e ? atoi(e) : 1; }();
@@ -219,6 +227,17 @@
   const bool pair = d.cta2 == 1 || (d.cta2 < 0 && cta2_env && !aux && !d.out_f32 && d.batch <= 1 && d.N >= 256 &&
                                     d.M >= 2048);
   const bool epi8 = d.gelu_heavy != 0;
+  if (d.ln_x != nullptr) {
+    static const int ln_env = [] { const char* e = getenv("MSMD_GEMM_LN"); return e ? atoi(e) : 1; }();
+    *ln_fused = false;
+    if (ln_env && pair && !epi8 && !d.act && d.N == 512) {
+      const int rc = launch_cfg2<GemmCfg<MODE, 256, 4, false, H, H, true>, MODE, false, true>(d, st);
+      if (rc != kLnUnfused) {
+        *ln_fused = rc == MSMD_OK;
+        return rc;
+      }
+    }
+  }
   if (pair) {
     if (epi8) return launch_cfg<GemmCfg<MODE, 256, 8, false, H, H, true>, MODE>(d, st);
     return launch_cfg<GemmCfg<MODE, 256, 4, false, H, H, true>, MODE>(d, st);
@@ -246,12 +265,15 @@
   }
 }
 
-int gemm_tc_launch(const GemmDesc& d, cudaStream_t st) {
+int gemm_tc_launch(const GemmDesc& d, cudaStream_t st, bool* ln_fused) {
   MSMD_REQUIRE(d.M > 0 && d.N > 0 && d.K > 0, "gemm: empty problem %dx%dx%d", d.M, d.N, d.K);
   MSMD_REQUIRE(d.A && d.W && d.out, "gemm: null operand");
+  MSMD_REQUIRE(!d.ln_x || (ln_fused && (d.mode == 0 || d.mode == 3) && d.bias && d.ln_g && d.ln_b && !d.aux && !d.out_f32 &&
+                           d.batch <= 1),
+               "gemm: the LayerNorm epilogue needs a 16-bit GEMM with bias, gamma and beta");
   const bool aux = d.aux != nullptr;
-  if (d.mode == 0) return dispatch16<0, __nv_bfloat16>(d, st);
-  if (d.mode == 3) return dispatch16<3, __half>(d, st);
+  if (d.mode == 0) return dispatch16<0, __nv_bfloat16>(d, st, ln_fused);
+  if (d.mode == 3) return dispatch16<3, __half>(d, st, ln_fused);
   MSMD_REQUIRE(d.mode == 1 || d.mode == 2, "gemm: unknown mode %d", d.mode);
   MSMD_REQUIRE(d.out_f32 && (!aux || d.aux_f32), "gemm: the three-pass modes are fp32 out");
   if (d.mode == 2) {
diff --git a/ubisoft-laforge-msmd_b200/csrc/gemm_tc.cuh b/ubisoft-laforge-msmd_b200/csrc/gemm_tc.cuh
--- a/ubisoft-laforge-msmd_b200/csrc/gemm_tc.cuh
+++ b/ubisoft-laforge-msmd_b200/csrc/gemm_tc.cuh
@@ -21,6 +21,7 @@
   int bias_zstride;
   int tiles_m, tiles_n;
   unsigned long long* trace;
+  const float *ln_g, *ln_b;
 };
 
 template <int MODE, int BN_, int EPI_WARPS_, bool HAS_AUX_, typename OutT_, typename AuxT_, bool CTA2_ = false, int OUT_BUFS_ = 2>
@@ -112,7 +113,150 @@
 #endif
 }
 
-template <class Cfg, int MODE, bool GELU>
+template <class Cfg>
+__device__ __forceinline__ void gemm_ln_epilogue(const GemmParams& p, uint8_t* stage, uint64_t* stage_bar, uint32_t tmem_base,
+                                                 uint64_t* tfull_bar, uint64_t* tempty_bar, uint64_t* xch_bar, float2* xch,
+                                                 int tile0, int tstride, int num_tiles, int crank) {
+  using namespace tc;
+  using H = typename Cfg::OutT;
+  constexpr int D = 512, HALF = 256, NCH = HALF / 32;
+  static_assert(Cfg::OUT_BUFS == 2 && Cfg::OUT_COLS == 64, "two 64-column staging tiles per warp");
+  const int warp = threadIdx.x >> 5, lane = threadIdx.x & 31, q = warp & 3, swz = lane & 7;
+  const int half = crank >> 1, cta_rank = crank & 1;
+  const uint32_t peer = (uint32_t)(crank ^ 2);
+  const int n0 = half * HALF, rl = q * 32 + lane;
+  const float *bias = p.bias + n0, *g = p.ln_g + n0, *be = p.ln_b + n0;
+  int xe = 0, so = 0, it = 0;
+
+  auto exchange = [&](float mean, float m2, float& gmean, float& rstd) {
+    const int slot = xe & 1;
+    const uint32_t par = (xe >> 1) & 1;
+    ++xe;
+    if (threadIdx.x == 64) mbar_expect_tx(&xch_bar[slot], 128 * 8);
+    st_async_cluster_f2(&xch[slot * 128 + rl], mean, m2, &xch_bar[slot], peer);
+    mbar_wait(&xch_bar[slot], par);
+    const float2 o = xch[slot * 128 + rl];
+    const float ma = half ? o.x : mean, mb = half ? mean : o.x;
+    const float qa = half ? o.y : m2, qb = half ? m2 : o.y;
+    gmean = (ma + mb) * 0.5f;
+    const float dm = ma - mb;
+    rstd = rsqrtf(fmaf(128.0f * dm, dm, qa + qb) * (1.0f / D) + 1e-5f);
+  };
+  auto pass = [&](uint32_t t, auto&& f) {
+    uint32_t ra[32], rb[32];
+    tmem_ld32(t, ra);
+#pragma unroll
+    for (int c = 0; c < NCH; c += 2) {
+      tmem_ld_wait();
+      tmem_ld32(t + 32 * (c + 1), rb);
+      f(c, ra);
+      tmem_ld_wait();
+      if (c + 2 < NCH) tmem_ld32(t + 32 * (c + 2), ra);
+      f(c + 1, rb);
+    }
+  };
+  auto load_x = [&](int b, int col, int m0) {
+    if (lane == 0) {
+      mbar_expect_tx(&stage_bar[b], 4096);
+      tma_load_2d(stage + b * 4096, &p.out_map, &stage_bar[b], col, m0 + q * 32);
+    }
+  };
+
+  for (int t = tile0; t < num_tiles; t += tstride, ++it) {
+    const int a = it & 1;
+    const uint32_t aph = (it >> 1) & 1;
+    const int m0 = (t >> 1) * (2 * Cfg::BM) + cta_rank * Cfg::BM;
+    if (lane == 0) tma_store_wait_read<0>();
+    __syncwarp();
+    load_x(0, n0, m0);
+    load_x(1, n0 + 64, m0);
+    if (warp == 2 && lane == 0) trace_stamp(p.trace, 2, it, 0);
+    mbar_wait(&tfull_bar[a], aph);
+    tc_fence_after();
+    if (warp == 2 && lane == 0) trace_stamp(p.trace, 2, it, 1);
+    const uint32_t t_addr = tmem_base + ((uint32_t)(q * 32) << 16) + a * Cfg::ACC_COLS;
+
+    float sum = 0.f;
+    pass(t_addr, [&](int c, uint32_t (&r)[32]) {
+      const int b = (c >> 1) & 1;
+      if ((c & 1) == 0) mbar_wait(&stage_bar[b], (uint32_t)(c >> 2));
+      const uint8_t* xrow = stage + b * 4096 + lane * 128;
+#pragma unroll
+      for (int k = 0; k < 4; ++k) {
+        const uint4 w4 = *reinterpret_cast<const uint4*>(xrow + ((((c & 1) * 4 + k) ^ swz) << 4));
+        const uint32_t w[4] = {w4.x, w4.y, w4.z, w4.w};
+        const float4 b0 = __ldg(reinterpret_cast<const float4*>(bias + 32 * c + 8 * k));
+        const float4 b1 = __ldg(reinterpret_cast<const float4*>(bias + 32 * c + 8 * k + 4));
+        const float bb[8] = {b0.x, b0.y, b0.z, b0.w, b1.x, b1.y, b1.z, b1.w};
+#pragma unroll
+        for (int u = 0; u < 4; ++u) {
+          const int j = 8 * k + 2 * u;
+          const float2 y = unpack16x2<H>(pack16x2<H>(__uint_as_float(r[j]) + bb[2 * u], __uint_as_float(r[j + 1]) + bb[2 * u + 1]));
+          const float2 xv = unpack16x2<H>(w[u]);
+          const float v0 = y.x + xv.x, v1 = y.y + xv.y;
+          sum += v0; sum += v1;
+          r[j] = __float_as_uint(v0); r[j + 1] = __float_as_uint(v1);
+        }
+      }
+      tmem_st32(t_addr + 32 * c, r);
+      if ((c & 1) && c < 4) {
+        __syncwarp();
+        load_x(b, n0 + 128 + 64 * b, m0);
+      }
+    });
+    tmem_st_wait();
+    const float hmean = sum * (1.0f / HALF);
+    float m2 = 0.f;
+    pass(t_addr, [&](int c, uint32_t (&r)[32]) {
+#pragma unroll
+      for (int j = 0; j < 32; ++j) { const float dlt = __uint_as_float(r[j]) - hmean; m2 = fmaf(dlt, dlt, m2); }
+    });
+    float mean, rstd;
+    exchange(hmean, m2, mean, rstd);
+    pass(t_addr, [&](int c, uint32_t (&r)[32]) {
+      if ((c & 1) == 0) {
+        if (lane == 0) tma_store_wait_read<Cfg::OUT_BUFS - 1>();
+        __syncwarp();
+      }
+      uint8_t* obuf = stage + (so % Cfg::OUT_BUFS) * 4096;
+      uint8_t* orow = obuf + lane * 128;
+#pragma unroll
+      for (int k = 0; k < 4; ++k) {
+        const float4 g0 = __ldg(reinterpret_cast<const float4*>(g + 32 * c + 8 * k));
+        const float4 g1 = __ldg(reinterpret_cast<const float4*>(g + 32 * c + 8 * k + 4));
+        const float4 e0 = __ldg(reinterpret_cast<const float4*>(be + 32 * c + 8 * k));
+        const float4 e1 = __ldg(reinterpret_cast<const float4*>(be + 32 * c + 8 * k + 4));
+        const float gg[8] = {g0.x, g0.y, g0.z, g0.w, g1.x, g1.y, g1.z, g1.w};
+        const float ee[8] = {e0.x, e0.y, e0.z, e0.w, e1.x, e1.y, e1.z, e1.w};
+        float o[8];
+#pragma unroll
+        for (int u = 0; u < 8; ++u) o[u] = (__uint_as_float(r[8 * k + u]) - mean) * rstd * gg[u] + ee[u];
+        *reinterpret_cast<uint4*>(orow + ((((c & 1) * 4 + k) ^ swz) << 4)) =
+            make_uint4(pack16x2<H>(o[0], o[1]), pack16x2<H>(o[2], o[3]), pack16x2<H>(o[4], o[5]), pack16x2<H>(o[6], o[7]));
+      }
+      if (c & 1) {
+        fence_proxy_async_smem();
+        __syncwarp();
+        if (lane == 0) {
+          tma_store_2d(&p.out_map, obuf, n0 + 64 * (c >> 1), m0 + q * 32);
+          tma_store_commit();
+        }
+        ++so;
+      }
+    });
+    if (warp == 2 && lane == 0) trace_stamp(p.trace, 2, it, 2);
+    tc_fence_before();
+    __syncwarp();
+    if (lane == 0) {
+      if (cta_rank != 0) mbar_arrive_cluster(&tempty_bar[a], crank & ~1);
+      else mbar_arrive(&tempty_bar[a]);
+    }
+    if (warp == 2 && lane == 0) trace_stamp(p.trace, 2, it, 3);
+  }
+  if (lane == 0) tma_store_wait<0>();
+}
+
+template <class Cfg, int MODE, bool GELU, bool LN = false>
 __global__ void __launch_bounds__(Cfg::THREADS, 1) gemm_tc_kernel(const __grid_constant__ GemmParams p) {
   using namespace tc;
   using OutT = typename Cfg::OutT;
@@ -130,7 +274,12 @@
   uint64_t* aux_bar = bars + 2 * STAGES + 4;
   uint32_t* tmem_slot = reinterpret_cast<uint32_t*>(bars + 2 * STAGES + 4 + 2 * Cfg::EPI_WARPS);
   float* bias_tile = reinterpret_cast<float*>(reinterpret_cast<uint8_t*>(bars) + 256);
-  static_assert((2 * Cfg::STAGES + 4 + 2 * Cfg::EPI_WARPS) * 8 + 4 <= 256, "barrier block overflows its 256 bytes");
+  uint64_t* xch_bar = bars + 2 * STAGES + 4 + 2 * Cfg::EPI_WARPS + 1;
+  float2* xch = reinterpret_cast<float2*>(bias_tile);
+  static_assert((2 * Cfg::STAGES + 4 + 2 * Cfg::EPI_WARPS + (LN ? 3 : 0)) * 8 + 4 <= 256, "barrier block overflows its 256 bytes");
+  static_assert(!LN || (Cfg::CTA2 && !GELU && !Cfg::HAS_AUX && Cfg::BN == 256 && Cfg::EPI_WARPS == 4 &&
+                        (MODE == 0 || MODE == 3) && 2 * 128 * sizeof(float2) <= 2 * 256 * sizeof(float)),
+                "LayerNorm epilogue: 16-bit CTA-pair kernels with 256-column tiles and 4 epilogue warps");
   if (threadIdx.x == 0 && reinterpret_cast<uint8_t*>(bias_tile) + 2 * 256 * 4 > smem_raw + Cfg::SMEM_BYTES) __trap();
 
   griddep_launch();
@@ -154,6 +303,7 @@
     for (int s = 0; s < STAGES; ++s) { mbar_init(&full_bar[s], 1); mbar_init(&empty_bar[s], cl4 ? 2 : 1); }
     for (int a = 0; a < 2; ++a) { mbar_init(&tfull_bar[a], 1); mbar_init(&tempty_bar[a], Cfg::EPI_WARPS * (Cfg::CTA2 ? 2 : 1)); }
     for (int i = 0; i < 2 * Cfg::EPI_WARPS; ++i) mbar_init(&aux_bar[i], 1);
+    if (LN) { mbar_init(&xch_bar[0], 1); mbar_init(&xch_bar[1], 1); }
     fence_barrier_init();
   }
   if (warp == 1) {
@@ -280,6 +430,9 @@
       }
       __syncwarp();
     }
+  } else if constexpr (LN) {
+    gemm_ln_epilogue<Cfg>(p, epi_base + (warp - 2) * Cfg::EPI_WARP_BYTES, aux_bar + 2 * (warp - 2), tmem_base, tfull_bar,
+                          tempty_bar, xch_bar, xch, tile0, tstride, num_tiles, crank);
   } else {
     const int e = warp - 2;
     const int q = warp & 3;
@@ -532,9 +685,11 @@
   int gelu_heavy = 0;
   int cta2 = -1;
   int max_ctas = 0;
+  void* ln_x = nullptr;
+  const float *ln_g = nullptr, *ln_b = nullptr;
 };
 
-int gemm_tc_launch(const GemmDesc& d, cudaStream_t st);
+int gemm_tc_launch(const GemmDesc& d, cudaStream_t st, bool* ln_fused = nullptr);
 int split_f16(const float* x, __half* hi, __half* lo, int64_t n, cudaStream_t st, int* overflow = nullptr);
 
 }
diff --git a/ubisoft-laforge-msmd_b200/csrc/tc_common.cuh b/ubisoft-laforge-msmd_b200/csrc/tc_common.cuh
--- a/ubisoft-laforge-msmd_b200/csrc/tc_common.cuh
+++ b/ubisoft-laforge-msmd_b200/csrc/tc_common.cuh
@@ -126,6 +126,18 @@
       : "memory");
 }
 __device__ __forceinline__ void tmem_ld_wait() { asm volatile("tcgen05.wait::ld.sync.aligned;" ::: "memory"); }
+__device__ __forceinline__ void tmem_st32(uint32_t taddr, const uint32_t* v) {
+  asm volatile(
+      "tcgen05.st.sync.aligned.32x32b.x32.b32 [%0], "
+      "{%1, %2, %3, %4, %5, %6, %7, %8, %9, %10, %11, %12, %13, %14, %15, %16, "
+      "%17, %18, %19, %20, %21, %22, %23, %24, %25, %26, %27, %28, %29, %30, %31, %32};"
+      ::"r"(taddr), "r"(v[0]), "r"(v[1]), "r"(v[2]), "r"(v[3]), "r"(v[4]), "r"(v[5]), "r"(v[6]), "r"(v[7]), "r"(v[8]),
+        "r"(v[9]), "r"(v[10]), "r"(v[11]), "r"(v[12]), "r"(v[13]), "r"(v[14]), "r"(v[15]), "r"(v[16]), "r"(v[17]),
+        "r"(v[18]), "r"(v[19]), "r"(v[20]), "r"(v[21]), "r"(v[22]), "r"(v[23]), "r"(v[24]), "r"(v[25]), "r"(v[26]),
+        "r"(v[27]), "r"(v[28]), "r"(v[29]), "r"(v[30]), "r"(v[31])
+      : "memory");
+}
+__device__ __forceinline__ void tmem_st_wait() { asm volatile("tcgen05.wait::st.sync.aligned;" ::: "memory"); }
 
 __device__ __forceinline__ uint32_t cluster_ctarank() {
   uint32_t r;
@@ -183,6 +195,15 @@
       "{\n\t.reg .b32 ra;\n\tmapa.shared::cluster.u32 ra, %0, %1;\n\t"
       "mbarrier.arrive.shared::cluster.b64 _, [ra];\n\t}"
       ::"r"(smem_u32(bar)), "r"(rank)
+      : "memory");
+}
+__device__ __forceinline__ void st_async_cluster_f2(float2* dst, float a, float b, uint64_t* bar, uint32_t rank) {
+  asm volatile(
+      "{\n\t.reg .b32 rd, rb;\n\t"
+      "mapa.shared::cluster.u32 rd, %0, %4;\n\t"
+      "mapa.shared::cluster.u32 rb, %1, %4;\n\t"
+      "st.async.shared::cluster.mbarrier::complete_tx::bytes.v2.f32 [rd], {%2, %3}, [rb];\n\t}"
+      ::"r"(smem_u32(dst)), "r"(smem_u32(bar)), "f"(a), "f"(b), "r"(rank)
       : "memory");
 }
 
```

Measured after the change: 235.1, median of 6. 1.02x the previous value.
